# thunlp/OpenMatch

Measured on AMD Instinct MI355X. Metric: passages/sec encode (bert-base DPR bi-encoder, 128 tok -> 768-d) [+ queries/sec exact top-1000 over 8.8M x 768 in `search`], higher is better.
Workload: dtype f16; 1 GPU; bert-base DPR bi-encoder encode+search, MS MARCO 8.8M x 128-tok -> 768-d (BASELINE configs[1]); seq_len=128, global_batch=1024, index_rows=8841823, queries=6980, topk=1000, weights=random-init BertConfig() seed 0, parallelism=shard1

## Files before the change

### include/openmatch_hip.h

```cpp
#ifndef OPENMATCH_HIP_H
#define OPENMATCH_HIP_H

#include <stddef.h>
#include <stdint.h>

#ifdef __cplusplus
extern "C" {
#endif

#define OM_ABI_VERSION 6

#define OM_F32 0
#define OM_BF16 1
#define OM_F16 2

#define OM_ACT_NONE 0
#define OM_ACT_GELU_ERF 1
#define OM_ACT_RELU 2
#define OM_ACT_GELU_TANH 3
#define OM_ACT_SILU 5
#define OM_ACT_MUL_RESID 0x100
#define OM_ACT_PRE_GRAD 0x200

#define OM_ARCH_BERT 0
#define OM_ARCH_T5 1
#define OM_ARCH_MODERNBERT 2

#define OM_ARCH_CAUSAL 3

#define OM_ARCH_NOMICBERT 4

#define OM_POOL_NONE 0
#define OM_POOL_FIRST 1
#define OM_POOL_MEAN 2
#define OM_POOL_LAST 3

#define OM_SEARCH_F32 0
#define OM_SEARCH_F16_RESCORE 1

const char* om_last_error(void);
int om_abi_version(void);

int om_device_count(void);

#define OM_TIMING_GEMM_BF16 0
#define OM_TIMING_GEMM_F32 1
#define OM_TIMING_SCAN 2
void om_debug_gemm_trace(unsigned long long* buf);
void om_debug_gemm_gen(int gen);
#define OM_GEMM_FAMILY_V1 1
#define OM_GEMM_FAMILY_V2 2
#define OM_GEMM_FAMILY_V6 6
#define OM_GEMM_FAMILY_G7 7
#define OM_GEMM_FAMILY_G7_ONE_TILE 70
#define OM_GEMM_FAMILY_G7C16 71
#define OM_GEMM_FAMILY_G7R16 72
#define OM_GEMM_FAMILY_SKINNY 9
int om_debug_gemm_last(void);
int om_debug_gemm_plan(int in_dtype, const void* A, int64_t lda, const void* B, int64_t ldb, int out_dtype, void* C, int64_t ldc,
                       int64_t M, int64_t N, int64_t K, const float* bias, const void* resid, int64_t ldr, int act);
typedef struct OmDebugGemmEpilogue {
  const float* bias; const void* resid; int64_t ldr; int act;
  void* pre_act; int64_t ldp; float drop_p; uint64_t seed; const int* drop_rows;
  const float* ln_stats; const float* ln_colsum; const float* rln_stats; const float* rln_g; const float* rln_b; float* stats_out;
  const void* resid_lo; void* out_lo;
  const float* resid32; float* out32;
  const float* a_ln32; const float* a_ln_g; const float* a_ln_b; float* a_ln_stats_out; const float* rln32; const float* rln32_stats;
  int lo8; float ln_inv_h, ln_eps; int ln_rms; int reverse;
  const int* rows_dev;
} OmDebugGemmEpilogue;
int om_debug_gemm_ex(int in_dtype, const void* A, int64_t lda, const void* B, int64_t ldb, int out_dtype, void* C, int64_t ldc,
                     int64_t M, int64_t N, int64_t K, const OmDebugGemmEpilogue* ep, void* stream);
int om_debug_gemm_plan_ex(int in_dtype, const void* A, int64_t lda, const void* B, int64_t ldb, int out_dtype, void* C, int64_t ldc,
                          int64_t M, int64_t N, int64_t K, const OmDebugGemmEpilogue* ep);
int om_debug_gemm_splitk(int in_dtype, const void* A, int64_t lda, const void* B, int64_t ldb, float* C, int64_t ldc, int64_t M,
                         int64_t N, int64_t K, void* stream);
#define OM_OPT_ENCODER_FUSED_LN 0
#define OM_OPT_ENCODER_DEBUG 1
#define OM_OPT_ATTENTION_FAST 2
#define OM_OPT_SCAN_GEN7 3
#define OM_OPT_SCAN_GROWTH 4
#define OM_OPT_WGRAD_DEBUG 5
#define OM_OPT_GEMM_GROUP_M 6
#define OM_OPT_SCAN_QGROUP 7
#define OM_OPT_TRAIN_WGRAD_STREAM 8
#define OM_OPT_ATTENTION_DEBUG 9
#define OM_OPT_ENCODER_PINGPONG 10
#define OM_OPT_ENCODER_TWO_PLANE 11
#define OM_OPT_GEMM_VARIANT 12
#define OM_OPT_SEARCH_DEBUG 13
#define OM_OPT_TRAIN_WGRAD_BATCH 14
#define OM_OPT_GEMM_MAX_GRID 15
#define OM_OPT_GEMM_CONT 16
#define OM_OPT_TRAIN_TAPE_GRAD 17
#define OM_OPT_TRAIN_RES32 18
#define OM_OPT_GEMM_SKINNY_M 19
#define OM_OPT_GEMM_SKINNY_CFG 20
#define OM_OPT_FEW_ROWS_LN_FUSE 21
#define OM_OPT_ENCODER_SKIP_PAD 22
#define OM_OPT_ENCODER_CLS_TAIL 23
#define OM_OPT_ENCODER_LANES 24
#define OM_OPT_COUNT 25
int om_debug_option(int opt, int value);
int om_debug_option_value(int opt);
int om_debug_attention(const void* qkv, void* ctx, const int64_t* mask, int64_t B, int L, int H, int heads, void* stream);
int om_debug_attention_ex(int dtype, const void* qkv, void* ctx, const int64_t* mask, const float* pos_bias, int64_t B, int L, int H,
                          int heads, float scale, float drop_p, uint64_t seed, void* stream, int reverse, const int* kmax,
                          const int* cu, int w);
int om_debug_rope(int dtype, void* qkv, int64_t M, int L, int H, float theta, void* stream);
int om_debug_rope_rows(int dtype, void* qkv, int64_t rows, int L, int H, float theta, const int* row_map, void* stream);
int om_debug_swiglu_rows(int dtype, const void* in, void* out, int64_t M, int F, void* stream);
int om_debug_embed(int dtype, const int64_t* ids, const int64_t* type_ids, const float* word, const float* pos, const float* type,
                   const float* g, const float* b, void* out, int64_t M, int L, int H, int vocab, int type_vocab, float eps, void* stream);
int om_debug_attention_causal(int dtype, const void* qkv, void* ctx, const int64_t* mask, int64_t B, int L, int n_heads, int n_kv_heads,
                              float scale, void* stream);
int om_debug_rope_gqa(int dtype, void* qkv, int64_t M, int L, int n_heads, int n_kv_heads, const float* inv_freq, float scaling, void* stream);
int om_debug_attention_causal_packed(int dtype, const void* qkv, void* ctx, const int64_t* mask, const int* cu, int64_t B, int L, int n_heads,
                                     int n_kv_heads, float scale, void* stream);
int om_debug_rope_gqa_rows(int dtype, void* qkv, int64_t rows, int L, int n_heads, int n_kv_heads, const float* inv_freq, float scaling,
                           const int* row_map, void* stream);
int om_debug_attention_causal_hd(int dtype, const void* qkv, void* ctx, const int64_t* mask, int64_t B, int L, int n_heads, int n_kv_heads,
                                 int head_dim, float scale, void* stream);
int om_debug_attention_causal_hd_packed(int dtype, const void* qkv, void* ctx, const int64_t* mask, const int* cu, int64_t B, int L,
                                        int n_heads, int n_kv_heads, int head_dim, float scale, void* stream);
int om_debug_qknorm_rope(int dtype, void* qkv, int64_t M, int L, int n_heads, int n_kv_heads, int head_dim, const float* q_norm_g,
                         const float* k_norm_g, float eps, const float* inv_freq, float scaling, void* stream);
int om_debug_qknorm_rope_rows(int dtype, void* qkv, int64_t rows, int L, int n_heads, int n_kv_heads, int head_dim, const float* q_norm_g,
                              const float* k_norm_g, float eps, const float* inv_freq, float scaling, const int* row_map, void* stream);
int om_debug_attention_gqa_d256(int dtype, const void* qkv, void* ctx, const int64_t* mask, int64_t B, int L, int n_heads, int n_kv_heads,
                                float scale, int w, void* stream);
int om_debug_qknorm_rope_d256(int dtype, void* qkv, int64_t M, int L, int n_heads, int n_kv_heads, const float* q_norm_g, const float* k_norm_g,
                              float eps, const float* inv_freq, float scaling, void* stream);
int om_debug_attention_gqa_d256_packed(int dtype, const void* qkv, void* ctx, const int64_t* mask, const int* cu, int64_t B, int L, int n_heads,
                                       int n_kv_heads, float scale, int w, void* stream);
int om_debug_qknorm_rope_d256_rows(int dtype, void* qkv, int64_t rows, int L, int n_heads, int n_kv_heads, const float* q_norm_g,
                                   const float* k_norm_g, float eps, const float* inv_freq, float scaling, const int* row_map, void* stream);
int om_debug_rmsnorm_add(int dtype, const void* h, int64_t ldh, float* x, int64_t ldx, const float* g, int64_t M, int H, float eps, void* stream);
int om_debug_mask_extent(const int64_t* mask, int64_t B, int L, int* kmax, void* stream);
int om_debug_pack_rows(const int* kmax, int64_t B, int L, int64_t rows, int* cu, int* cls_rows, int* row_map, void* stream);
#define OM_ATTN_FAMILY_GENERIC 1
#define OM_ATTN_FAMILY_FWD16 2
#define OM_ATTN_FAMILY_FWD16_KMAX4 3
#define OM_ATTN_FAMILY_FWD16C 4
#define OM_ATTN_FAMILY_LONG 5
#define OM_ATTN_FAMILY_D32 6
#define OM_ATTN_FAMILY_BAND16 7
#define OM_ATTN_FAMILY_BAND32 8
int om_debug_attention_last(void);
int om_debug_attention_plan(int dtype, int64_t B, int L, int H, int heads, int has_bias, float drop_p, int has_kmax, int has_cu, int w);
#define OM_ATTN_BWD_FAMILY_BWD16 1
#define OM_ATTN_BWD_FAMILY_GENERIC 2
#define OM_ATTN_BWD_FAMILY_LONG 3
#define OM_ATTN_BWD_FAMILY_D32 4
int om_debug_attention_bwd_last(void);
int om_debug_attention_bwd_plan(int dtype, int64_t B, int L, int H, int heads, int has_bias, int has_drel, int has_cu, int packed);
int om_debug_attention_bwd_ex(int dtype, const void* qkv, const void* ctx, const void* dctx, void* dqkv, const int64_t* mask,
                              const float* pos_bias, float* drel, float* stats, int64_t B, int L, int H, int heads, float scale,
                              float drop_p, uint64_t seed, const int* cu, int packed, void* stream);
size_t om_debug_attention_bwd_stats_bytes(int64_t B, int heads);
#define OM_ENC_PATH_BERT_FUSED 1
#define OM_ENC_PATH_BERT_PENDING_LN 2
#define OM_ENC_PATH_BERT_FEW32 3
#define OM_ENC_PATH_BERT_PLAIN 4
#define OM_ENC_PATH_MODERNBERT 5
#define OM_ENC_PATH_T5_FUSED 6
#define OM_ENC_PATH_T5_PLAIN 7
struct OmEncoderConfig;
int om_debug_encoder_plan(const struct OmEncoderConfig* cfg, int gated_ffn, int has_rel_bias, int64_t B, int64_t L, int64_t packed_rows,
                          int want_hidden);
int om_debug_encoder_skip_pad(const struct OmEncoderConfig* cfg, int gated_ffn, int has_rel_bias, int64_t B, int64_t L, int want_hidden);
int om_debug_encoder_cls_tail(const struct OmEncoderConfig* cfg, int gated_ffn, int has_rel_bias, int64_t B, int64_t L, int64_t packed_rows,
                              int want_hidden);
int om_debug_encoder_lanes(const struct OmEncoderConfig* cfg, int gated_ffn, int has_rel_bias, int64_t B, int64_t L, int64_t packed_rows,
                           int want_hidden, int64_t* B0);
#define OM_ENCODER_LANE_RANGES 15
int om_debug_encoder_lane_ranges(const struct OmEncoderConfig* cfg, int gated_ffn, int has_rel_bias, int64_t B, int64_t L, int lane,
                                 int64_t* out, int cap);
int64_t om_debug_encoder_lane_forks(void);
int om_debug_gather_rows(const void* src0, void* dst0, const void* src1, void* dst1, const void* src2, void* dst2, const float* stats_src,
                         float* stats_dst, const int* rows, int64_t B, int64_t L, int64_t Mc, int H, void* stream);
int om_debug_attn_drop_keep(uint64_t seed, int64_t b, int h, int heads, int Lm, int q, int key, float p);
int om_debug_wave_sum_check(const float* in, float* out_shuffle, float* out_dpp, int64_t groups, void* stream);
#define OM_ROW_FWD_GENERIC 1
#define OM_ROW_FWD_X8 2
#define OM_ROW_LN_BWD 3
int om_debug_row_kernel_last(void);
int om_debug_layernorm(int dtype, const void* x, int64_t ldx, void* y, int64_t ldy, const float* g, const float* b, int64_t M, int H,
                       float eps, int rms, const void* x_lo, int lo8, void* stream);
int om_debug_layernorm_f32out(int dtype, const void* x, int64_t ldx, float* y, int64_t ldy, const float* g, const float* b, int64_t M,
                              int H, float eps, int rms, const void* x_lo, const int* rows, int lo8, void* stream);
int om_debug_layernorm_from_f32(int dtype, const float* x, int64_t ldx, void* y, int64_t ldy, const float* g, const float* b, int64_t M,
                                int H, float eps, int rms, void* stream);
int om_debug_layernorm_dual(int dtype, const float* x, int64_t ldx, void* y, float* y32, int64_t ldy, const float* g, const float* b,
                            int64_t M, int H, float eps, void* stream);
int om_debug_norm_bwd(int dtype, const void* dy, const void* x, const float* g, void* dx, float* dg, float* db, int64_t M, int H,
                      float eps, int rms, const void* add, void* stream);
int om_debug_ln_bwd_drop(int dtype, const void* dy, const void* x, const float* g, void* dx, void* dx_drop, float drop_p,
                         uint64_t drop_seed, float* dg, float* db, int64_t M, int H, float eps, const float* dy32, const float* x32,
                         float* partial, int* partial_blocks , const int* drop_rows, void* stream);
typedef struct OmLnSite { const float* partial; float* dg; float* db; int blocks; } OmLnSite;
int om_debug_ln_param_reduce(const OmLnSite* sites , int n, int H, void* stream);
int om_debug_embed_bwd(int dtype, const void* dy, const int64_t* ids, const int64_t* type_ids, const float* word, const float* pos,
                       const float* type, const float* g, float* dword, float* dpos, float* dtype_, float* dg, float* db, int64_t M,
                       int L, int H, int vocab, int type_vocab, float eps, const int* cu, void* stream);
int om_debug_pool(int dtype, const void* x, const int64_t* mask, float* out, int64_t B, int L, int H, int mode, const int* cu,
                  void* stream);
int om_debug_pool_bwd(int dtype, const float* dp, const int64_t* mask, void* dh, int64_t B, int L, int H, int mode, const int* cu,
                      void* stream);
int om_debug_l2norm(const float* x, float* y, int64_t M, int D, void* stream);
int om_debug_l2norm_bwd(const float* x, const float* dy, float* dx, int64_t M, int D, void* stream);
int om_debug_colsum(int dtype, const void* x, int64_t ld, int64_t M, int N, float* out, void* stream);
int om_debug_dropout(int dtype, const void* x, void* y, int64_t n, float p, uint64_t seed, const int* rows, int H, void* stream);
int om_debug_ln_fold(int dtype, const void* W, const float* gamma, const float* beta, const float* b, void* Wf, float* colsum,
                     float* bf, int N, int K, void* stream);
int om_debug_ln_stats_reduce(const float* slots, int nslots, int64_t M, float* out, void* stream);
int om_kernel_timing_enable(int enable);
int om_kernel_timing_read(int kernel_class, double* total_ms, int64_t* launches, double* flops);

int om_gemm_nt(int in_dtype, const void* A, int64_t lda, const void* B, int64_t ldb,
               int out_dtype, void* C, int64_t ldc, int64_t M, int64_t N, int64_t K,
               const float* bias, const void* resid, int64_t ldr, int act, void* stream);

int om_gemm_tn_acc(int in_dtype, const void* A, int64_t lda, const void* B, int64_t ldb,
                   float* C, int64_t ldc, float* bias, int64_t M, int64_t N, int64_t K, void* stream);

typedef struct OmTnProblem {
  const void* A; const void* B; float* C; float* bias;
  int64_t lda, ldb, ldc, N, K;
} OmTnProblem;
int om_gemm_tn_acc_batch(int in_dtype, const OmTnProblem* problems, int n, int64_t M, void* stream);

typedef struct OmLayerWeights {
  const void* qkv_w;
  const float* qkv_b;
  const void* o_w;
  const float* o_b;
  const float* ln1_g;
  const float* ln1_b;
  const void* ffn1_w;
  const float* ffn1_b;
  const void* ffn1g_w;
  const void* ffn2_w;
  const float* ffn2_b;
  const float* ln2_g;
  const float* ln2_b;
} OmLayerWeights;

typedef struct OmEncoderConfig {
  int arch;
  int dtype;
  int hidden;
  int n_layers;
  int n_heads;
  int head_dim;
  int ffn;
  int vocab;
  int max_pos;
  int type_vocab;
  int act;
  float ln_eps;
  int rel_buckets;
  int rel_max_dist;
  int pooling;
  int head_in;
  int head_out;
  int normalize;
  float rope_theta_global;
  float rope_theta_local;
  int half_window;
  uint64_t sliding_layers;
} OmEncoderConfig;

typedef struct OmEncoderWeights {
  const float* word_emb;
  const float* pos_emb;
  const float* type_emb;
  const float* emb_ln_g;
  const float* emb_ln_b;
  const OmLayerWeights* layers_host;
  const float* final_ln_g;
  const float* rel_bias;
  const float* head_w;
  const void* folded;
  const float* final_ln_b;
} OmEncoderWeights;

size_t om_encoder_fold_bytes(const OmEncoderConfig* cfg);
int om_encoder_fold_weights(const OmEncoderConfig* cfg, const OmEncoderWeights* w, void* folded, size_t bytes, void* stream);

size_t om_encoder_workspace_bytes(const OmEncoderConfig* cfg, int64_t B, int64_t L);

int om_t5_relative_bucket(int relative_position, int num_buckets, int max_distance);

int om_encoder_forward(const OmEncoderConfig* cfg, const OmEncoderWeights* w,
                       const int64_t* input_ids, const int64_t* attention_mask,
                       const int64_t* token_type_ids, int64_t B, int64_t L,
                       void* out_hidden, float* out_reps, void* workspace,
                       size_t workspace_bytes, void* stream);

int om_encoder_packed_supported(const OmEncoderConfig* cfg, int gated_ffn, int64_t B, int64_t L, int64_t packed_rows);
size_t om_encoder_workspace_bytes_packed(const OmEncoderConfig* cfg, int64_t B, int64_t L, int64_t packed_rows);
int om_encoder_forward_packed(const OmEncoderConfig* cfg, const OmEncoderWeights* w,
                              const int64_t* input_ids, const int64_t* attention_mask,
                              const int64_t* token_type_ids, int64_t B, int64_t L, int64_t packed_rows,
                              float* out_reps, void* workspace, size_t workspace_bytes, void* stream);

typedef struct OmCausalConfig {
  OmEncoderConfig base;
  int n_kv_heads;
  float rope_attention_scaling;
  float inv_freq[32];
} OmCausalConfig;
size_t om_causal_encoder_workspace_bytes(const OmCausalConfig* cfg, int64_t B, int64_t L);
int om_causal_encoder_forward(const OmCausalConfig* cfg, const OmEncoderWeights* w, const int64_t* input_ids,
                              const int64_t* attention_mask, int64_t B, int64_t L, void* out_hidden, float* out_reps,
                              void* workspace, size_t workspace_bytes, void* stream);
int om_causal_encoder_packed_supported(const OmCausalConfig* cfg, int64_t B, int64_t L, int64_t packed_rows);
size_t om_causal_encoder_workspace_bytes_packed(const OmCausalConfig* cfg, int64_t B, int64_t L, int64_t packed_rows);
int om_causal_encoder_forward_packed(const OmCausalConfig* cfg, const OmEncoderWeights* w, const int64_t* input_ids,
                                     const int64_t* attention_mask, int64_t B, int64_t L, int64_t packed_rows, float* out_reps,
                                     void* workspace, size_t workspace_bytes, void* stream);

typedef struct OmCausalConfig2 {
  OmCausalConfig base;
  int qk_norm;
  int reserved;
  float inv_freq[64];
} OmCausalConfig2;
typedef struct OmCausalQkNorm {
  const float* q_norm_g;
  const float* k_norm_g;
} OmCausalQkNorm;
size_t om_causal2_encoder_workspace_bytes(const OmCausalConfig2* cfg, int64_t B, int64_t L);
int om_causal2_encoder_forward(const OmCausalConfig2* cfg, const OmEncoderWeights* w, const OmCausalQkNorm* qk_norm_host,
                               const int64_t* input_ids, const int64_t* attention_mask, int64_t B, int64_t L, void* out_hidden,
                               float* out_reps, void* workspace, size_t workspace_bytes, void* stream);
int om_causal2_encoder_packed_supported(const OmCausalConfig2* cfg, int64_t B, int64_t L, int64_t packed_rows);
size_t om_causal2_encoder_workspace_bytes_packed(const OmCausalConfig2* cfg, int64_t B, int64_t L, int64_t packed_rows);
int om_causal2_encoder_forward_packed(const OmCausalConfig2* cfg, const OmEncoderWeights* w, const OmCausalQkNorm* qk_norm_host,
                                      const int64_t* input_ids, const int64_t* attention_mask, int64_t B, int64_t L, int64_t packed_rows,
                                      float* out_reps, void* workspace, size_t workspace_bytes, void* stream);

#define OM_ARCH_GEMMA3 5
typedef struct OmGemma3Config {
  OmCausalConfig base;
  float attn_scale;
  int half_window;
  uint64_t sliding_layers;
  float full_scaling;
  float sliding_scaling;
  float attn_logit_softcapping;
  int bidirectional;
  float full_inv_freq[128];
  float sliding_inv_freq[128];
} OmGemma3Config;
typedef struct OmGemma3Norms {
  const float* q_norm_g;
  const float* k_norm_g;
  const float* post_attention_norm_g;
  const float* post_feedforward_norm_g;
} OmGemma3Norms;
size_t om_gemma3_encoder_workspace_bytes(const OmGemma3Config* cfg, int64_t B, int64_t L);
int om_gemma3_encoder_forward(const OmGemma3Config* cfg, const OmEncoderWeights* w, const OmGemma3Norms* norms_host, const int64_t* input_ids,
                              const int64_t* attention_mask, int64_t B, int64_t L, void* out_hidden, float* out_reps, void* workspace,
                              size_t workspace_bytes, void* stream);
int om_gemma3_encoder_packed_supported(const OmGemma3Config* cfg, int64_t B, int64_t L, int64_t packed_rows);
size_t om_gemma3_encoder_workspace_bytes_packed(const OmGemma3Config* cfg, int64_t B, int64_t L, int64_t packed_rows);
int om_gemma3_encoder_forward_packed(const OmGemma3Config* cfg, const OmEncoderWeights* w, const OmGemma3Norms* norms_host,
                                     const int64_t* input_ids, const int64_t* attention_mask, int64_t B, int64_t L, int64_t packed_rows,
                                     float* out_reps, void* workspace, size_t workspace_bytes, void* stream);

typedef struct OmT5DecoderLayer {
  const void* sa_v_w;
  const void* sa_o_w;
  const float* sa_ln_g;
  const void* ca_q_w;
  const void* ca_kv_w;
  const void* ca_o_w;
  const float* ca_ln_g;
  const void* ffn1_w;
  const void* ffn1g_w;
  const void* ffn2_w;
  const float* ffn_ln_g;
} OmT5DecoderLayer;
typedef struct OmT5DecoderWeights {
  const float* start_emb;
  const float* final_ln_g;
  const OmT5DecoderLayer* layers_host;
  int n_layers;
} OmT5DecoderWeights;
size_t om_t5_decoder_workspace_bytes(const OmEncoderConfig* cfg, int64_t B, int64_t L);
int om_t5_decoder_step(const OmEncoderConfig* cfg, const OmT5DecoderWeights* w, const void* enc_hidden,
                       const int64_t* attention_mask, int64_t B, int64_t L, float* out_hidden,
                       void* workspace, size_t workspace_bytes, void* stream);

typedef struct OmT5DecoderLayerGrads {
  float* sa_v_w;  float* sa_o_w; float* sa_ln_g;
  float* ca_q_w;  float* ca_kv_w; float* ca_o_w; float* ca_ln_g;
  float* ffn1_w;  float* ffn1g_w; float* ffn2_w; float* ffn_ln_g;
} OmT5DecoderLayerGrads;
typedef struct OmT5DecoderGrads {
  float* start_emb;
  float* final_ln_g;
  const OmT5DecoderLayerGrads* layers_host;
} OmT5DecoderGrads;
size_t om_t5_decoder_tape_bytes(const OmEncoderConfig* cfg, int n_layers, int64_t B, int64_t L);
size_t om_t5_decoder_train_workspace_bytes(const OmEncoderConfig* cfg, int n_layers, int64_t B, int64_t L);
int om_t5_decoder_train_forward(const OmEncoderConfig* cfg, const OmT5DecoderWeights* w, const void* enc_hidden,
                                const int64_t* attention_mask, int64_t B, int64_t L, float dropout, uint64_t seed,
                                void* tape, size_t tape_bytes, float* out_hidden, void* workspace,
                                size_t workspace_bytes, void* stream);
int om_t5_decoder_train_backward(const OmEncoderConfig* cfg, const OmT5DecoderWeights* w, const void* enc_hidden,
                                 const int64_t* attention_mask, int64_t B, int64_t L, float dropout, uint64_t seed,
                                 const void* tape, const float* d_out, const OmT5DecoderGrads* grads,
                                 void* d_enc_hidden, void* workspace, size_t workspace_bytes, void* stream);

int om_linear_f32_backward(const float* dy, const float* x, const float* w, float* dw, float* dx, int B, int D, int K,
                           void* stream);

typedef struct OmLayerGrads {
  float* qkv_w;  float* qkv_b;  float* o_w;    float* o_b;   float* ln1_g; float* ln1_b;
  float* ffn1_w; float* ffn1_b; float* ffn2_w; float* ffn2_b; float* ln2_g; float* ln2_b;
  float* ffn1g_w;
} OmLayerGrads;

typedef struct OmEncoderGrads {
  float* word_emb; float* pos_emb; float* type_emb; float* emb_ln_g; float* emb_ln_b;
  const OmLayerGrads* layers_host;
  float* head_w;
  float* final_ln_g;
  float* rel_bias;
} OmEncoderGrads;

size_t om_encoder_tape_bytes(const OmEncoderConfig* cfg, int64_t B, int64_t L);
size_t om_encoder_train_workspace_bytes(const OmEncoderConfig* cfg, int64_t B, int64_t L);

int om_encoder_train_forward(const OmEncoderConfig* cfg, const OmEncoderWeights* w,
                             const int64_t* input_ids, const int64_t* attention_mask,
                             const int64_t* token_type_ids, int64_t B, int64_t L,
                             float hidden_dropout, float attn_dropout, uint64_t seed, void* tape,
                             size_t tape_bytes, float* out_reps, void* workspace,
                             size_t workspace_bytes, void* stream);

int om_encoder_train_backward(const OmEncoderConfig* cfg, const OmEncoderWeights* w,
                              const int64_t* input_ids, const int64_t* attention_mask,
                              const int64_t* token_type_ids, int64_t B, int64_t L,
                              float hidden_dropout, float attn_dropout, uint64_t seed,
                              const void* tape, const float* d_reps, const OmEncoderGrads* grads,
                              void* workspace, size_t workspace_bytes, void* stream);

int om_encoder_train_packed_supported(const OmEncoderConfig* cfg, int64_t B, int64_t L, int64_t packed_rows);
size_t om_encoder_tape_bytes_packed(const OmEncoderConfig* cfg, int64_t B, int64_t L, int64_t packed_rows);
size_t om_encoder_train_workspace_bytes_packed(const OmEncoderConfig* cfg, int64_t B, int64_t L, int64_t packed_rows);
int om_encoder_train_forward_packed(const OmEncoderConfig* cfg, const OmEncoderWeights* w,
                                    const int64_t* input_ids, const int64_t* attention_mask,
                                    const int64_t* token_type_ids, int64_t B, int64_t L, int64_t packed_rows,
                                    float hidden_dropout, float attn_dropout, uint64_t seed,
                                    void* tape, size_t tape_bytes, float* out_reps,
                                    void* workspace, size_t workspace_bytes, void* stream);
int om_encoder_train_backward_packed(const OmEncoderConfig* cfg, const OmEncoderWeights* w,
                                     const int64_t* input_ids, const int64_t* attention_mask,
                                     const int64_t* token_type_ids, int64_t B, int64_t L, int64_t packed_rows,
                                     float hidden_dropout, float attn_dropout, uint64_t seed,
                                     const void* tape, const float* d_reps, const OmEncoderGrads* grads,
                                     void* workspace, size_t workspace_bytes, void* stream);

int om_encoder_train_forward_hidden(const OmEncoderConfig* cfg, const OmEncoderWeights* w,
                                    const int64_t* input_ids, const int64_t* attention_mask,
                                    const int64_t* token_type_ids, int64_t B, int64_t L,
                                    float hidden_dropout, float attn_dropout, uint64_t seed, void* tape,
                                    size_t tape_bytes, void* out_hidden, void* workspace,
                                    size_t workspace_bytes, void* stream);
int om_encoder_train_backward_hidden(const OmEncoderConfig* cfg, const OmEncoderWeights* w,
                                     const int64_t* input_ids, const int64_t* attention_mask,
                                     const int64_t* token_type_ids, int64_t B, int64_t L,
                                     float hidden_dropout, float attn_dropout, uint64_t seed,
                                     const void* tape, const void* d_hidden, const OmEncoderGrads* grads,
                                     void* workspace, size_t workspace_bytes, void* stream);

int om_encoder_train_set_layer_events(void* const* events, int n);

#define OM_ADAM_CHUNK 16384
typedef struct OmAdamTensor {
  float* p; const float* g; float* m; float* v;
  void* shadow0; void* shadow1;
  int64_t n;
  float weight_decay;
  int shadow0_dtype, shadow1_dtype, reserved;
} OmAdamTensor;
int om_grad_sqnorm(const OmAdamTensor* tensors, const int32_t* chunks, int n_chunks, float* partial, float* out_sq, void* stream);
int om_adamw_step(const OmAdamTensor* tensors, const int32_t* chunks, int n_chunks, float lr, float beta1, float beta2, float eps,
                  int64_t step, const float* gnorm_sq, float max_norm, float grad_scale, int skip_nonfinite,
                  const float* scale_state ,
                  void* stream);
int om_loss_scale_update(const float* gnorm_sq, float* state4, int growth_interval, void* stream);


int om_index_to_f16(const float* rows_f32, int64_t N, int d, void* rows_f16, float* stats,
                    void* stream);

size_t om_sim_topk_workspace_bytes(int64_t n_queries, int d, int k);

int om_sim_topk(int mode, const float* queries, int64_t n_queries, const float* index_f32,
                const void* index_f16, const float* stats, int64_t N, int d, int k,
                int64_t id_offset, float* out_scores, int64_t* out_ids, void* workspace,
                size_t workspace_bytes, void* stream);

void om_sim_topk_info(int64_t out[8]);

#define OM_SCAN_FAMILY_GENERIC 1
#define OM_SCAN_FAMILY_WIDE 2
#define OM_SCAN_FAMILY_STREAM32 3
#define OM_SCAN_FAMILY_STREAM16 4
int om_debug_scan_plan(int half, int64_t nq, int d, int out[4]);
int om_debug_sim_stream(const void* rows16, int64_t nrows, uint32_t row_base, const void* queries16, int64_t nq, int d, const float* thr,
                        uint64_t* keys, unsigned* cnt, int grid, void* stream);

int om_topk_merge(const float* part_scores, const int64_t* part_ids, int W, int64_t n_queries,
                  int k_in, int k_out, float* out_scores, int64_t* out_ids, void* stream);

int om_contrastive_fwd_bwd(const float* q, const float* p, int Qg, int Pg, int d, int n_psg,
                           float loss_scale, int q_row0, int q_rows, int p_row0, int p_rows,
                           float* loss, float* scores, float* d_q, float* d_p, float* workspace,
                           void* stream);

int om_contrastive_fwd_bwd_ex(const float* q, const float* p, int Qg, int Pg, int d, const int64_t* target, int n_psg,
                              int reduction, const float* row_grad, float loss_scale, int q_row0, int q_rows,
                              int p_row0, int p_rows, float* loss, float* scores, float* d_q, float* d_p,
                              float* workspace, void* stream);

#define OM_COMM_ID_BYTES 128
int om_comm_unique_id(void* id128);
int om_comm_init(const void* id128, int world, int rank, void** comm);
int om_comm_destroy(void* comm);
int om_comm_count(void* comm, int* count);
int om_allgather_rows(void* comm, const void* send, void* recv, int64_t rows, int64_t row_bytes, void* stream);
int om_allreduce_grads(void* comm, float* buf, int64_t n, int average, void* stream);
int om_exchange_topk(void* comm, int world, const float* D, const int64_t* I, int64_t q_block, int k, float* recvD,
                     int64_t* recvI, void* stream);

#ifdef __cplusplus
}
#endif
#endif
```

### openmatch_amd/csrc/abi.cpp

```cpp
#include "common.h"

static thread_local std::string g_last_error;
void om_set_error(const std::string& msg) { g_last_error = msg; }

extern "C" const char* om_last_error(void) { return g_last_error.c_str(); }
extern "C" int om_abi_version(void) { return OM_ABI_VERSION; }
extern "C" int om_device_count(void) {
  int n = 0;
  hipError_t e = hipGetDeviceCount(&n);
  if (e != hipSuccess) {
    om_set_error(std::string("hipGetDeviceCount: ") + hipGetErrorString(e));
    return -1;
  }
  return n;
}

#include <mutex>
#include <vector>
namespace {
struct Span { hipEvent_t a, b; };
struct ClassStat { std::vector<Span> spans; double flops = 0; size_t used = 0; };
bool g_timing = false;
ClassStat g_stat[3];
std::mutex g_mu;
}
bool om_timing_on() { return g_timing; }
void om_timing_begin(int c, hipStream_t s) {
  std::lock_guard<std::mutex> lk(g_mu);
  ClassStat& st = g_stat[c];
  if (st.used == st.spans.size()) {
    Span sp;
    (void)hipEventCreate(&sp.a);
    (void)hipEventCreate(&sp.b);
    st.spans.push_back(sp);
  }
  (void)hipEventRecord(st.spans[st.used].a, s);
}
void om_timing_end(int c, hipStream_t s, double flops) {
  std::lock_guard<std::mutex> lk(g_mu);
  ClassStat& st = g_stat[c];
  (void)hipEventRecord(st.spans[st.used].b, s);
  st.used++;
  st.flops += flops;
}
extern "C" int om_kernel_timing_enable(int enable) { g_timing = enable != 0; return 0; }
extern "C" int om_kernel_timing_read(int c, double* total_ms, int64_t* launches, double* flops) {
  if (c < 0 || c > 2) { om_set_error("om_kernel_timing_read: bad class"); return 1; }
  std::lock_guard<std::mutex> lk(g_mu);
  ClassStat& st = g_stat[c];
  double ms = 0;
  for (size_t i = 0; i < st.used; ++i) {
    hipError_t e = hipEventSynchronize(st.spans[i].b);
    float t = 0;
    if (e == hipSuccess) e = hipEventElapsedTime(&t, st.spans[i].a, st.spans[i].b);
    if (e != hipSuccess) { om_set_error(std::string("om_kernel_timing_read: ") + hipGetErrorString(e)); return 1; }
    ms += t;
  }
  if (total_ms) *total_ms = ms;
  if (launches) *launches = (int64_t)st.used;
  if (flops) *flops = st.flops;
  st.used = 0; st.flops = 0;
  return 0;
}

#include <atomic>
#include <map>
#include <tuple>
namespace {
std::atomic<int> g_opt[OM_OPT_COUNT];
std::atomic<bool> g_opt_init{false};
std::mutex g_opt_mu;
void opt_init() {
  std::lock_guard<std::mutex> lk(g_opt_mu);
  if (g_opt_init.load()) return;
  const char* e = getenv("OM_ENCODER_FUSED_LN");
  g_opt[OM_OPT_ENCODER_FUSED_LN] = e ? atoi(e) : 1;
  g_opt[OM_OPT_ENCODER_DEBUG] = getenv("OM_ENCODER_DEBUG") ? 1 : 0;
  e = getenv("OM_ATTENTION_FAST");
  g_opt[OM_OPT_ATTENTION_FAST] = e ? atoi(e) : 1;
  e = getenv("OM_SCAN_GEN7");
  g_opt[OM_OPT_SCAN_GEN7] = e ? atoi(e) : 1;
  e = getenv("OM_SCAN_GROWTH");
  g_opt[OM_OPT_SCAN_GROWTH] = e ? atoi(e) : 60;
  g_opt[OM_OPT_WGRAD_DEBUG] = 0;
  g_opt[OM_OPT_ATTENTION_DEBUG] = 0;
  e = getenv("OM_ENCODER_PINGPONG");
  g_opt[OM_OPT_ENCODER_PINGPONG] = e ? atoi(e) : 1;
  e = getenv("OM_TRAIN_WGRAD_STREAM");
  g_opt[OM_OPT_TRAIN_WGRAD_STREAM] = e ? atoi(e) : 1;
  e = getenv("OM_SCAN_QGROUP");
  g_opt[OM_OPT_SCAN_QGROUP] = e ? atoi(e) : 8;
  e = getenv("OM_GEMM_GROUP_M");
  g_opt[OM_OPT_GEMM_GROUP_M] = e ? atoi(e) : 8;
  e = getenv("OM_ENCODER_TWO_PLANE");
  g_opt[OM_OPT_ENCODER_TWO_PLANE] = e ? atoi(e) : 3;
  e = getenv("OM_GEMM_VARIANT");
  g_opt[OM_OPT_GEMM_VARIANT] = e ? atoi(e) : 0;
  e = getenv("OM_SEARCH_DEBUG");
  g_opt[OM_OPT_SEARCH_DEBUG] = e ? (atoi(e) ? atoi(e) : 1) : 0;
  e = getenv("OM_TRAIN_WGRAD_BATCH");
  g_opt[OM_OPT_TRAIN_WGRAD_BATCH] = e ? atoi(e) : 4;
  e = getenv("OM_GEMM_MAX_GRID");
  g_opt[OM_OPT_GEMM_MAX_GRID] = e ? atoi(e) : 0;
  e = getenv("OM_TRAIN_TAPE_GRAD");
  g_opt[OM_OPT_TRAIN_TAPE_GRAD] = e ? atoi(e) : 1;
  e = getenv("OM_TRAIN_RES32");
  g_opt[OM_OPT_TRAIN_RES32] = e ? atoi(e) : 1;
  e = getenv("OM_GEMM_CONT");
  g_opt[OM_OPT_GEMM_CONT] = e ? atoi(e) : 495;
  e = getenv("OM_GEMM_SKINNY_M");
  g_opt[OM_OPT_GEMM_SKINNY_M] = e ? atoi(e) : 1024;
  e = getenv("OM_FEW_ROWS_LN_FUSE");
  g_opt[OM_OPT_FEW_ROWS_LN_FUSE] = e ? atoi(e) : 64;
  e = getenv("OM_ENCODER_SKIP_PAD");
  g_opt[OM_OPT_ENCODER_SKIP_PAD] = e ? atoi(e) : 1;
  e = getenv("OM_ENCODER_CLS_TAIL");
  g_opt[OM_OPT_ENCODER_CLS_TAIL] = e ? atoi(e) : 1;
  e = getenv("OM_ENCODER_LANES");
  g_opt[OM_OPT_ENCODER_LANES] = e ? atoi(e) : 65536;
  g_opt_init.store(true);
}
}
bool om_option_is_set(int opt) {
  if (opt == OM_OPT_SCAN_GROWTH) return getenv("OM_SCAN_GROWTH") != nullptr;
  return false;
}
int om_option(int opt) {
  if (!g_opt_init.load(std::memory_order_acquire)) opt_init();
  return g_opt[opt].load(std::memory_order_relaxed);
}
extern "C" int om_debug_option(int opt, int value) {
  if (opt < 0 || opt >= OM_OPT_COUNT) { om_set_error("om_debug_option: unknown option"); return 1; }
  if (!g_opt_init.load(std::memory_order_acquire)) opt_init();
  g_opt[opt].store(value);
  return 0;
}
extern "C" int om_debug_option_value(int opt) {
  if (opt < 0 || opt >= OM_OPT_COUNT) { om_set_error("om_debug_option_value: unknown option"); return -1; }
  return om_option(opt);
}

int om_t5_lut_device(int L, int buckets, int max_dist, const int** out) {
  static std::mutex mu;
  static std::map<std::tuple<int, int, int, int>, int*> cache;
  int dev = 0;
  OM_HIP(hipGetDevice(&dev));
  std::lock_guard<std::mutex> lk(mu);
  auto key = std::make_tuple(dev, L, buckets, max_dist);
  auto it = cache.find(key);
  if (it == cache.end()) {
    std::vector<int> lut(2 * L);
    for (int rel = -(L - 1); rel <= L - 1; ++rel) lut[rel + (L - 1)] = om_t5_relative_bucket(rel, buckets, max_dist);
    int* d = nullptr;
    OM_HIP(hipMalloc(&d, (size_t)(2 * L) * sizeof(int)));
    OM_HIP(hipMemcpy(d, lut.data(), (size_t)(2 * L - 1) * sizeof(int), hipMemcpyHostToDevice));
    it = cache.emplace(key, d).first;
  }
  *out = it->second;
  return 0;
}
```

### openmatch_amd/csrc/attention.hip

```cpp
#include <type_traits>

#include "attn_chunked.h"
#include "attn_plan.h"

static thread_local int g_attn_last = 0;
extern "C" int om_debug_attention_last(void) { return g_attn_last; }

template <typename T, int KT>
__global__ __launch_bounds__(64 * KT) void attention_kernel(
    const T* __restrict__ qkv, T* __restrict__ ctx, const int64_t* __restrict__ mask,
    const float* __restrict__ pos_bias, int L, int H, int heads, float scale, float drop_p,
    uint64_t seed) {
  typedef AttnGeom<T> G;
  typedef typename MmaOps<T>::frag_t frag_t;
  constexpr int LP = KT * 32 + 4;
  extern __shared__ __attribute__((aligned(16))) char smem[];
  char* sK = smem;
  T* sVt = (T*)(smem + KT * 32 * G::ROWB);
  float* sM = (float*)(smem + KT * 32 * G::ROWB + 64 * LP * (int)sizeof(T));

  const int h = blockIdx.x % heads;
  const int64_t b = blockIdx.x / heads;
  const int tid = threadIdx.x, nthr = blockDim.x;
  const int64_t ld = 3 * (int64_t)H;
  const T* base = qkv + b * L * ld + h * 64;

  for (int idx = tid; idx < KT * 32 * G::CPR; idx += nthr) {
    const int row = idx / G::CPR, c = idx % G::CPR;
    uint4 kv = make_uint4(0, 0, 0, 0), vv = make_uint4(0, 0, 0, 0);
    if (row < L) {
      kv = *(const uint4*)(base + (int64_t)row * ld + H + c * G::EPC);
      vv = *(const uint4*)(base + (int64_t)row * ld + 2 * H + c * G::EPC);
    }
    *(uint4*)(sK + row * G::ROWB + ((c ^ G::key(row)) << 4)) = kv;
    const T* ve = (const T*)&vv;
#pragma unroll
    for (int e = 0; e < G::EPC; ++e) sVt[(c * G::EPC + e) * LP + row] = ve[e];
  }
  for (int k = tid; k < KT * 32; k += nthr)
    sM[k] = k < L ? (mask[b * L + k] != 0 ? 0.f : kFinfoMin) : -INFINITY;
  __syncthreads();

  const int wave = tid >> 6, lane = tid & 63, half = lane >> 5, l31 = lane & 31;
  const int q0 = wave * 32;
  if (q0 >= L) return;
  const int qrow = (q0 + l31) < L ? (q0 + l31) : (L - 1);

  frag_t qf[G::NKK];
#pragma unroll
  for (int kk = 0; kk < G::NKK; ++kk)
    qf[kk] = *(const frag_t*)(base + (int64_t)qrow * ld + (kk * 2 + half) * G::EPC);

  f32x16_t s[KT];
#pragma unroll
  for (int t = 0; t < KT; ++t) {
#pragma unroll
    for (int r = 0; r < 16; ++r) s[t][r] = 0.f;
    const int row = t * 32 + l31;
    const char* krow = sK + row * G::ROWB;
    const int key = G::key(row);
#pragma unroll
    for (int kk = 0; kk < G::NKK; ++kk) {
      const frag_t a = *(const frag_t*)(krow + (((kk * 2 + half) ^ key) << 4));
      MmaOps<T>::mma(a, qf[kk], s[t]);
    }
  }

  float mx = -INFINITY;
#pragma unroll
  for (int t = 0; t < KT; ++t)
#pragma unroll
    for (int g = 0; g < 4; ++g) {
      const int k0 = t * 32 + 8 * g + 4 * half;
      const f32x4_t mb = *(const f32x4_t*)(sM + k0);
#pragma unroll
      for (int e = 0; e < 4; ++e) {
        float v = s[t][4 * g + e] * scale;
        if (pos_bias) {
          const int kc = (k0 + e) < L ? (k0 + e) : (L - 1);
          v += pos_bias[((int64_t)h * L + qrow) * L + kc];
        }
        v += mb[e];
        s[t][4 * g + e] = v;
        mx = fmaxf(mx, v);
      }
    }
  mx = fmaxf(mx, __shfl_xor(mx, 32, 64));
  float sum = 0.f;
#pragma unroll
  for (int t = 0; t < KT; ++t)
#pragma unroll
    for (int r = 0; r < 16; ++r) {
      const float e = G::exp_(s[t][r] - mx);
      s[t][r] = e;
      sum += e;
    }
  sum += __shfl_xor(sum, 32, 64);
  const float inv = 1.0f / sum;
#pragma unroll
  for (int t = 0; t < KT; ++t)
#pragma unroll
    for (int r = 0; r < 16; ++r) s[t][r] *= inv;
  if (drop_p > 0.f) {
    const AttnDrop dr(drop_p);
#pragma unroll
    for (int t = 0; t < KT; ++t)
#pragma unroll
      for (int g = 0; g < 4; ++g) {
        const uint64_t bits = attn_drop_bits(seed, b, h, heads, L, q0 + l31, (t * 32 + 8 * g + 4 * half) >> 2);
#pragma unroll
        for (int e = 0; e < 4; ++e) s[t][4 * g + e] = attn_drop_keep(bits, e, dr.thresh) ? s[t][4 * g + e] * dr.keep_scale : 0.f;
      }
  }

  f32x16_t o[2];
#pragma unroll
  for (int dt = 0; dt < 2; ++dt)
#pragma unroll
    for (int r = 0; r < 16; ++r) o[dt][r] = 0.f;
#pragma unroll
  for (int t = 0; t < KT; ++t) SlabMma<T>::run(s[t], sVt + l31 * LP + t * 32 + 4 * half, LP, o);

  __syncthreads();
  T* so = (T*)(sK + (size_t)q0 * G::ROWB);
#pragma unroll
  for (int dt = 0; dt < 2; ++dt)
#pragma unroll
    for (int r = 0; r < 16; ++r) {
      const int q = (r & 3) + 8 * (r >> 2) + 4 * half;
      ElemOps<T>::store(so + q * 64 + dt * 32 + l31, o[dt][r]);
    }
  T* out = ctx + (b * L + q0) * H + h * 64;
  constexpr int VPR = G::ROWB / 16;
#pragma unroll
  for (int it = 0; it < 32 * VPR / 64; ++it) {
    const int idx = it * 64 + lane, row = idx / VPR, c = idx % VPR;
    const uint4 v = *(const uint4*)((const char*)so + row * G::ROWB + c * 16);
    if (q0 + row < L) *(uint4*)((char*)(out + (int64_t)row * H) + c * 16) = v;
  }
}

template <typename T, int KT, bool BIAS, bool DROP, int DBG, int KTV>
__device__ __forceinline__ void attention_fwd16_body(
    const T* __restrict__ qkv, T* __restrict__ ctx, const int64_t* __restrict__ mask,
    const float* __restrict__ pos_bias, int L, int H, int heads, float scale, float drop_p, uint64_t seed, int rev,
    int64_t row0, int Lm) {
  typedef typename MmaOps<T>::frag_t frag_t;
  extern __shared__ __attribute__((aligned(16))) char smem[];
  char* const sK = smem;
  char* const sV = smem + KT * 32 * 128;
  float* const sM = (float*)(smem + 2 * KT * 32 * 128);
  const int h = blockIdx.x % heads;
  const int64_t b = rev ? (int64_t)(gridDim.x / heads) - 1 - blockIdx.x / heads : blockIdx.x / heads;
  const int tid = threadIdx.x, lane = tid & 63, half = lane >> 5, l31 = lane & 31;
  const int wave = __builtin_amdgcn_readfirstlane(tid >> 6);
  const int64_t ld2 = 6 * (int64_t)H;
  const char* const base = (const char*)(qkv + row0 * 3 * (int64_t)H + h * 64);
  if (!(DBG & 1))
#pragma unroll
  for (int i = 0; i < 4; ++i) {
    if (KTV < KT && i * KT + wave >= KTV * 4) continue;
    const int r = (i * KT + wave) * 8 + (lane >> 3);
    const int rr = r < L ? r : L - 1;
    const uint32_t off = (uint32_t)(rr * ld2) + (((lane & 7) ^ ((r >> 1) & 7)) << 4);
    const uint32_t offv = (uint32_t)(rr * ld2) + (((lane & 7) ^ (((r >> 1) & 1) << 2)) << 4);
    const uint32_t dst = (uint32_t)((i * KT + wave) * 1024);
    g7_dma(base + 2 * H, off, g7_lds_addr(sK) + dst);
    g7_dma(base + 4 * H, offv, g7_lds_addr(sV) + dst);
  }
  const float LOG2E = 1.4426950408889634f;
  for (int k = tid; k < KT * 32; k += 64 * KT)
    sM[k] = k < L ? (mask[b * Lm + k] != 0 ? 0.f : -1e30f) : -INFINITY;

  const int q0 = wave * 32;
  const int qrow = (q0 + l31) < L ? (q0 + l31) : (L - 1);
  frag_t qf[4];
#pragma unroll
  for (int kk = 0; kk < 4; ++kk) qf[kk] = *(const frag_t*)(base + (int64_t)qrow * ld2 + (kk * 2 + half) * 16);
  asm volatile("s_waitcnt vmcnt(0)" ::: "memory");
  __syncthreads();
  if (q0 >= L) return;

  constexpr int KTC = (DBG & 2) ? 0 : KTV;
  const int key = (l31 >> 1) & 7;
  f32x16_t s[KTV];
#pragma unroll
  for (int t = 0; t < KTC; ++t) {
#pragma unroll
    for (int r = 0; r < 16; ++r) s[t][r] = 0.f;
    const char* krow = sK + (t * 32 + l31) * 128;
#pragma unroll
    for (int kk = 0; kk < 4; ++kk) {
      const frag_t a = *(const frag_t*)(krow + (((kk * 2 + half) ^ key) << 4));
      MmaOps<T>::mma(a, qf[kk], s[t]);
    }
    __builtin_amdgcn_sched_barrier(0);
  }
  const float c2 = scale * LOG2E;
  float mx = -INFINITY;
#pragma unroll
  for (int t = 0; t < KTC; ++t)
#pragma unroll
    for (int g = 0; g < 4; ++g) {
      const int k0 = t * 32 + 8 * g + 4 * half;
      const f32x4_t mb = *(const f32x4_t*)(sM + k0);
      f32x4_t pb = {0.f, 0.f, 0.f, 0.f};
      if (BIAS) {
        const float* pr = pos_bias + ((int64_t)h * Lm + qrow) * Lm;
#pragma unroll
        for (int e = 0; e < 4; ++e) pb[e] = pr[(k0 + e) < Lm ? (k0 + e) : (Lm - 1)] * LOG2E;
      }
#pragma unroll
      for (int e = 0; e < 4; ++e) {
        const float v = fmaf(s[t][4 * g + e], c2, mb[e]) + pb[e];
        s[t][4 * g + e] = v;
        mx = fmaxf(mx, v);
      }
      __builtin_amdgcn_sched_barrier(0);
    }
  mx = fmaxf(mx, __shfl_xor(mx, 32, 64));
  float sum = 0.f;
#pragma unroll
  for (int t = 0; t < KTC; ++t)
#pragma unroll
    for (int r = 0; r < 16; ++r) {
      const float e = __builtin_amdgcn_exp2f(s[t][r] - mx);
      s[t][r] = e;
      sum += e;
    }
  sum += __shfl_xor(sum, 32, 64);
  float inv = 1.0f / sum;
  if (DROP) {
    const AttnDrop dr(drop_p);
#pragma unroll
    for (int t = 0; t < KTC; ++t)
  #pragma unroll
      for (int g = 0; g < 4; ++g) {
        const uint64_t bits = attn_drop_bits(seed, b, h, heads, Lm, q0 + l31, (t * 32 + 8 * g + 4 * half) >> 2);
#pragma unroll
        for (int e = 0; e < 4; ++e) s[t][4 * g + e] = attn_drop_keep(bits, e, dr.thresh) ? s[t][4 * g + e] : 0.f;
        __builtin_amdgcn_sched_barrier(0);
      }
    inv *= dr.keep_scale;
  }

  const int i16 = lane & 15;
  const char* const vt0 = sV + (4 * half + (i16 >> 2)) * 128 + 32 * ((lane >> 4) & 1) + 8 * (i16 & 3);
  const int vsw = (i16 >> 3) & 1;
  f32x16_t o[2];
#pragma unroll
  for (int dt = 0; dt < 2; ++dt)
#pragma unroll
    for (int r = 0; r < 16; ++r) o[dt][r] = 0.f;
#pragma unroll
  for (int t = 0; t < KTC; ++t) {
    uint4 pa[2];
#pragma unroll
    for (int u = 0; u < 2; ++u)
      pa[u] = make_uint4(Half16<T>::pack2(s[t][8 * u + 0], s[t][8 * u + 1]), Half16<T>::pack2(s[t][8 * u + 2], s[t][8 * u + 3]),
                         Half16<T>::pack2(s[t][8 * u + 4], s[t][8 * u + 5]), Half16<T>::pack2(s[t][8 * u + 6], s[t][8 * u + 7]));
#pragma unroll
    for (int u = 0; u < 2; ++u) {
#pragma unroll
      for (int dt = 0; dt < 2; ++dt) {
        const char* p = vt0 + (t * 32 + 16 * u) * 128 + ((dt ^ vsw) << 6);
        const frag_t vf = vfrag_of<frag_t>(vtrd(p), vtrd(p + 8 * 128));
        MmaOps<T>::mma(vf, __builtin_bit_cast(frag_t, pa[u]), o[dt]);
      }
    }
    __builtin_amdgcn_sched_barrier(0);
  }
  if (DBG & 2) {
#pragma unroll
    for (int kk = 0; kk < 4; ++kk) o[0][kk] = (float)qf[kk][0];
  }
  __syncthreads();
  char* const so = sK + q0 * 128;
#pragma unroll
  for (int dt = 0; dt < 2; ++dt)
#pragma unroll
    for (int gp = 0; gp < 2; ++gp) {
      uint32_t a0 = Half16<T>::pack2(o[dt][8 * gp + 0] * inv, o[dt][8 * gp + 1] * inv), a1 = Half16<T>::pack2(o[dt][8 * gp + 2] * inv, o[dt][8 * gp + 3] * inv);
      uint32_t b0 = Half16<T>::pack2(o[dt][8 * gp + 4] * inv, o[dt][8 * gp + 5] * inv), b1 = Half16<T>::pack2(o[dt][8 * gp + 6] * inv, o[dt][8 * gp + 7] * inv);
      auto r0 = __builtin_amdgcn_permlane32_swap(a0, b0, false, false);
      auto r1 = __builtin_amdgcn_permlane32_swap(a1, b1, false, false);
      *(uint4*)(so + l31 * 128 + (((4 * dt + 2 * gp + half) ^ (l31 & 7)) << 4)) = make_uint4(r0[0], r1[0], r0[1], r1[1]);
    }
  char* const out = (char*)(ctx + (row0 + q0) * (int64_t)H + h * 64);
#pragma unroll
  for (int it = 0; it < 4; ++it) {
    const int row = it * 8 + (lane >> 3), c = lane & 7;
    const uint4 v = *(const uint4*)(so + row * 128 + ((c ^ (row & 7)) << 4));
    if (!(DBG & 4) || v.x == 0x12345u) { if (q0 + row < L) *(uint4*)(out + (int64_t)row * H * 2 + c * 16) = v; }
  }
}

template <typename T, int KT, bool BIAS, bool DROP, int DBG = 0>
__global__ __launch_bounds__(64 * KT, KT <= 4 ? ((BIAS || DROP) ? 3 : 4) : 2) void attention_fwd16_kernel(
    const T* __restrict__ qkv, T* __restrict__ ctx, const int64_t* __restrict__ mask,
    const float* __restrict__ pos_bias, int L, int H, int heads, float scale, float drop_p, uint64_t seed, int rev,
    const int* __restrict__ kmax, const int* __restrict__ cu) {
#define OM_ATTN_BODY(V) attention_fwd16_body<T, KT, BIAS, DROP, DBG, V>(qkv, ctx, mask, pos_bias, Lb, H, heads, scale, drop_p, seed, rev, row0, L)
  const int64_t b = rev ? (int64_t)(gridDim.x / heads) - 1 - blockIdx.x / heads : blockIdx.x / heads;
  int64_t row0 = b * L;
  int Lb = L;
  if (cu) {
    const int c0 = __builtin_amdgcn_readfirstlane(cu[b]), c1 = __builtin_amdgcn_readfirstlane(cu[b + 1]);
    row0 = c0; Lb = c1 - c0;
    if (Lb <= 0) return;
  }
  if (KT == 4 && !BIAS && !DROP && (kmax || cu)) {
    const int kt = ((cu ? Lb : __builtin_amdgcn_readfirstlane(kmax[b])) + 31) >> 5;
    if (kt <= 1) { OM_ATTN_BODY(1); return; }
    if (kt == 2) { OM_ATTN_BODY(2); return; }
    if (kt == 3) { OM_ATTN_BODY(3); return; }
  }
  OM_ATTN_BODY(KT);
#undef OM_ATTN_BODY
}

template <typename T, int KT, bool BIAS, bool DROP>
static int launch_attn16(const void* qkv, void* ctx, const int64_t* mask, const float* pos_bias, int64_t B, int L, int H,
                         int heads, float scale, float drop_p, uint64_t seed, hipStream_t s, int rev, const int* kmax, const int* cu) {
  const int lds = 2 * KT * 32 * 128 + KT * 32 * 4;
  if (attn_lds_once<attention_fwd16_kernel<T, KT, BIAS, DROP>>(lds)) return 1;
#ifdef OM_PROBE_KERNELS
  const int dbg = (sizeof(T) == 2 && std::is_same<T, bf16_t>::value && KT == 4 && !BIAS && !DROP) ? om_option(OM_OPT_ATTENTION_DEBUG) : 0;
#else
  const int dbg = 0;
#endif
  if (dbg) {
#ifdef OM_PROBE_KERNELS
#define OM_ATTN_DBG(D)                                                                                                        \
  case D:                                                                                                                     \
    hipLaunchKernelGGL((attention_fwd16_kernel<bf16_t, 4, false, false, D>), dim3((unsigned)(heads * B)), dim3(256), lds, s,          \
                       (const bf16_t*)qkv, (bf16_t*)ctx, mask, pos_bias, L, H, heads, scale, drop_p, seed, rev, kmax, cu);    \
    break;
    switch (dbg) { OM_ATTN_DBG(1) OM_ATTN_DBG(2) OM_ATTN_DBG(3) OM_ATTN_DBG(4) OM_ATTN_DBG(5) OM_ATTN_DBG(6) OM_ATTN_DBG(7) default: break; }
#undef OM_ATTN_DBG
#endif
    OM_LAUNCH_CHECK();
    return 0;
  }
  hipLaunchKernelGGL((attention_fwd16_kernel<T, KT, BIAS, DROP>), dim3((unsigned)(heads * B)), dim3(64 * KT), lds, s, (const T*)qkv,
                     (T*)ctx, mask, pos_bias, L, H, heads, scale, drop_p, seed, rev, kmax, cu);
  OM_LAUNCH_CHECK();
  return 0;
}
template <typename T, bool BIAS, bool DROP>
__global__ __launch_bounds__(256, 2) void attention_fwd16c_kernel(
    const T* __restrict__ qkv, T* __restrict__ ctx, const int64_t* __restrict__ mask,
    const float* __restrict__ pos_bias, int Lm, int H, int heads, float scale, float drop_p, uint64_t seed, const int* __restrict__ cu) {
  const int h = blockIdx.x % heads;
  const int64_t b = blockIdx.x / heads;
  int64_t row0 = b * Lm;
  int L = Lm;
  if (cu) {
    const int c0 = __builtin_amdgcn_readfirstlane(cu[b]), c1 = __builtin_amdgcn_readfirstlane(cu[b + 1]);
    row0 = c0; L = c1 - c0;
  }
  const int qb = blockIdx.y * 128;
  if (qb >= L) return;
  attn_chunked16<T, AttnFull, BIAS, DROP>(attn_rows_fused(qkv, ctx, row0, H, h), AttnFull{}, mask + b * Lm, L, L, qb, scale, AttnFullArgs{pos_bias, drop_p, seed, b, h, heads, Lm});
}

template <typename T, bool BIAS, bool DROP>
static int launch_attn16c(const void* qkv, void* ctx, const int64_t* mask, const float* pos_bias, int64_t B, int L, int H,
                           int heads, float scale, float drop_p, uint64_t seed, hipStream_t s, const int* cu) {
  const int lds = 2 * 128 * 128 + 128 * 4;
  hipLaunchKernelGGL((attention_fwd16c_kernel<T, BIAS, DROP>), dim3((unsigned)(heads * B), (unsigned)((L + 127) / 128)), dim3(256), lds, s,
                     (const T*)qkv, (T*)ctx, mask, pos_bias, L, H, heads, scale, drop_p, seed, cu);
  OM_LAUNCH_CHECK();
  return 0;
}
template <typename T>
__global__ __launch_bounds__(256) void attention_long_kernel(
    const T* __restrict__ qkv, T* __restrict__ ctx, const int64_t* __restrict__ mask,
    const float* __restrict__ pos_bias, int Lm, int H, int heads, float scale, float drop_p, uint64_t seed, const int* __restrict__ cu) {
  const int h = blockIdx.x % heads;
  const int64_t b = blockIdx.x / heads;
  const int qb = blockIdx.y * 128;
  int64_t row0 = b * Lm;
  int L = Lm;
  if (cu) { row0 = cu[b]; L = cu[b + 1] - cu[b]; }
  if (qb >= L) return;
  attn_chunked_qreg<T, AttnFull>(attn_rows_fused(qkv, ctx, row0, H, h), AttnFull{}, mask + b * Lm, L, L, qb, scale, AttnFullArgs{pos_bias, drop_p, seed, b, h, heads, Lm});
}

template <typename T>
static int launch_attn_long(const void* qkv, void* ctx, const int64_t* mask, const float* pos_bias, int64_t B, int L, int H,
                            int heads, float scale, float drop_p, uint64_t seed, hipStream_t s, const int* cu) {
  const int lds = 128 * AttnGeom<T>::ROWB + 64 * 132 * (int)sizeof(T) + 128 * 4 + 128 * 4;
  if (attn_lds_once<attention_long_kernel<T>>(lds)) return 1;
  hipLaunchKernelGGL((attention_long_kernel<T>), dim3((unsigned)(heads * B), (unsigned)((L + 127) / 128)), dim3(256), lds, s,
                     (const T*)qkv, (T*)ctx, mask, pos_bias, L, H, heads, scale, drop_p, seed, cu);
  OM_LAUNCH_CHECK();
  return 0;
}

template <typename T, int KT>
static int launch_attn(const void* qkv, void* ctx, const int64_t* mask, const float* pos_bias,
                       int64_t B, int L, int H, int heads, float scale, float drop_p, uint64_t seed,
                       hipStream_t s) {
  constexpr int LP = KT * 32 + 4;
  const int lds = KT * 32 * AttnGeom<T>::ROWB + 64 * LP * (int)sizeof(T) + KT * 32 * 4;
  if (attn_lds_once<attention_kernel<T, KT>>(lds)) return 1;
  const int waves = (L + 31) / 32;
  hipLaunchKernelGGL((attention_kernel<T, KT>), dim3((unsigned)(heads * B)),
                     dim3(64 * waves), lds, s, (const T*)qkv, (T*)ctx, mask, pos_bias, L, H, heads,
                     scale, drop_p, seed);
  OM_LAUNCH_CHECK();
  return 0;
}

__global__ void mask_extent_kernel(const int64_t* __restrict__ mask, int64_t B, int L, int* __restrict__ kmax) {
  const int64_t b = (int64_t)blockIdx.x * (blockDim.x >> 6) + (threadIdx.x >> 6);
  if (b >= B) return;
  const int lane = threadIdx.x & 63;
  int last = 0;
  for (int k = lane; k < L; k += 64) if (mask[b * L + k] != 0) last = k + 1;
#pragma unroll
  for (int o = 32; o > 0; o >>= 1) last = max(last, __shfl_xor(last, o, 64));
  if (lane == 0) kmax[b] = last ? last : L;
}
__global__ __launch_bounds__(1024) void pack_rows_kernel(const int* __restrict__ kmax, int64_t B, int L, int64_t rows, int* __restrict__ cu,
                                                          int* __restrict__ cls_rows, int* __restrict__ row_map) {
  __shared__ int part[1024];
  const int tid = threadIdx.x;
  const int64_t per = (B + 1023) / 1024, lo = tid * per, hi = lo + per < B ? lo + per : B;
  int sum = 0;
  for (int64_t i = lo; i < hi; ++i) sum += kmax[i];
  part[tid] = sum;
  __syncthreads();
  for (int off = 1; off < 1024; off <<= 1) {
    const int v = tid >= off ? part[tid - off] : 0;
    __syncthreads();
    part[tid] += v;
    __syncthreads();
  }
  const int total = part[1023];
  const int cap = (int)rows;
  if (blockIdx.x == 0) {
    int run = part[tid] - sum;
    for (int64_t i = lo; i < hi; ++i) {
      cu[i] = run < cap ? run : cap;
      cls_rows[i] = run < cap ? run : cap - 1;
      run += kmax[i];
    }
    if (tid == 1023) { cu[B] = total < cap ? total : cap; cu[B + 1] = total; }
  }
  for (int64_t t = (int64_t)blockIdx.x * 1024 + tid; t < rows; t += (int64_t)gridDim.x * 1024) {
    int v = -1;
    if (t < total) {
      int a = 0, b = 1023;
      while (a < b) { const int m = (a + b) >> 1; if (part[m] > (int)t) b = m; else a = m + 1; }
      int64_t i = a * per;
      int run = a ? part[a - 1] : 0;
      for (int n = kmax[i]; run + n <= (int)t; n = kmax[++i]) run += n;
      v = (int)(i * L + ((int)t - run));
    }
    row_map[t] = v;
  }
}
int omk_pack_rows(const int* kmax, int64_t B, int L, int64_t rows, int* cu, int* cls_rows, int* row_map, hipStream_t s) {
  if (B <= 0) return 0;
  if (rows > 0x7fffffff || B * (int64_t)L > 0x7fffffff) OM_FAIL("packed rows: token counts below 2^31");
  const int64_t slices = (rows + 1023) / 1024;
  hipLaunchKernelGGL(pack_rows_kernel, dim3((unsigned)(slices < 1 ? 1 : slices > 1024 ? 1024 : slices)), dim3(1024), 0, s, kmax, B, L, rows, cu, cls_rows,
                     row_map);
  OM_LAUNCH_CHECK();
  return 0;
}

int omk_mask_extent(const int64_t* mask, int64_t B, int L, int* kmax, hipStream_t s) {
  if (B <= 0) return 0;
  hipLaunchKernelGGL(mask_extent_kernel, dim3((unsigned)((B + 3) / 4)), dim3(256), 0, s, mask, B, L, kmax);
  OM_LAUNCH_CHECK();
  return 0;
}

int omk_attention(int dtype, const void* qkv, void* ctx, const int64_t* mask, const float* pos_bias, int64_t B, int L, int H, int heads,
                  float scale, float drop_p, uint64_t seed, hipStream_t s, int reverse, const int* kmax, const int* cu, int w) {
  g_attn_last = 0;
  const AttnPlan p = attn_plan_fwd(dtype, B, L, H, heads, pos_bias != nullptr, drop_p, kmax != nullptr, cu != nullptr, w, attn_switches());
  if (p.error) OM_FAIL(p.error);
  g_attn_last = p.family | (p.kt << 8);
  switch (p.family) {
    case 0: return 0;
    case OM_ATTN_FAMILY_D32: return omk_attention_d32(p, dtype, qkv, ctx, mask, pos_bias, B, L, H, heads, scale, drop_p, seed, s, reverse, kmax, cu);
    case OM_ATTN_FAMILY_BAND16: case OM_ATTN_FAMILY_BAND32: return omk_attention_band(dtype, qkv, ctx, mask, B, L, H, heads, scale, w, kmax, s);
    case OM_ATTN_FAMILY_FWD16: case OM_ATTN_FAMILY_FWD16_KMAX4:
      return attn_with_type16(dtype, [&](auto t) {
        return attn_with_kt<1, 2, 4, 6, 8>(p.kt, [&](auto kt) {
          return attn_with_flags(p.bias, p.drop, [&](auto bias, auto drop) {
            return launch_attn16<decltype(t), kt(), bias(), drop()>(qkv, ctx, mask, pos_bias, B, L, H, heads, scale, drop_p, seed, s, reverse, kmax, cu);
          });
        });
      });
    case OM_ATTN_FAMILY_FWD16C:
      return attn_with_type16(dtype, [&](auto t) {
        return attn_with_flags(p.bias, p.drop, [&](auto bias, auto drop) {
          return launch_attn16c<decltype(t), bias(), drop()>(qkv, ctx, mask, pos_bias, B, L, H, heads, scale, drop_p, seed, s, cu);
        });
      });
    case OM_ATTN_FAMILY_LONG:
      return attn_with_type(dtype, [&](auto t) { return launch_attn_long<decltype(t)>(qkv, ctx, mask, pos_bias, B, L, H, heads, scale, drop_p, seed, s, cu); });
    default:
      if (dtype == OM_BF16)
        return attn_with_kt<1, 2, 4, 6, 8>(p.kt, [&](auto kt) { return launch_attn<bf16_t, kt()>(qkv, ctx, mask, pos_bias, B, L, H, heads, scale, drop_p, seed, s); });
      return attn_with_kt<1, 2, 4, 6, 8>(p.kt, [&](auto kt) { return launch_attn<float, kt()>(qkv, ctx, mask, pos_bias, B, L, H, heads, scale, drop_p, seed, s); });
  }
}

extern "C" int om_debug_attention_plan(int dtype, int64_t B, int L, int H, int heads, int has_bias, float drop_p, int has_kmax, int has_cu, int w) {
  const AttnPlan p = attn_plan_fwd(dtype, B, L, H, heads, has_bias != 0, drop_p, has_kmax != 0, has_cu != 0, w, attn_switches());
  if (p.error) { om_set_error(std::string(__func__) + ": " + p.error); return -1; }
  return p.family | (p.kt << 8);
}

extern "C" int om_debug_attention_ex(int dtype, const void* qkv, void* ctx, const int64_t* mask, const float* pos_bias, int64_t B, int L, int H,
                                     int heads, float scale, float drop_p, uint64_t seed, void* stream, int reverse, const int* kmax,
                                     const int* cu, int w) {
  g_attn_last = 0;
  if (!qkv || !ctx || !mask) OM_FAIL("null argument");
  if (dtype != OM_F32 && dtype != OM_BF16 && dtype != OM_F16) OM_FAIL("attention: dtype must be OM_F32, OM_BF16 or OM_F16");
  if (w > 0 && (pos_bias || drop_p > 0.f || cu || reverse)) OM_FAIL("banded attention: no position bias, dropout, packed rows or reverse walk");
  return omk_attention(dtype, qkv, ctx, mask, pos_bias, B, L, H, heads, scale, drop_p, seed, (hipStream_t)stream, reverse, kmax, cu, w);
}
extern "C" int om_debug_attention(const void* qkv, void* ctx, const int64_t* mask, int64_t B, int L, int H, int heads, void* stream) {
  return om_debug_attention_ex(OM_BF16, qkv, ctx, mask, nullptr, B, L, H, heads, 0.125f, 0.f, 0, stream, 0, nullptr, nullptr, 0);
}
extern "C" int om_debug_rope(int dtype, void* qkv, int64_t M, int L, int H, float theta, void* stream) {
  if (!qkv) OM_FAIL("null argument");
  if (dtype != OM_F32 && dtype != OM_BF16 && dtype != OM_F16) OM_FAIL("rotary positions: dtype must be OM_F32, OM_BF16 or OM_F16");
  return omk_rope(dtype, qkv, M, L, H, theta, (hipStream_t)stream);
}
extern "C" int om_debug_rope_rows(int dtype, void* qkv, int64_t rows, int L, int H, float theta, const int* row_map, void* stream) {
  if (!qkv || !row_map) OM_FAIL("null argument");
  if (dtype != OM_F32 && dtype != OM_BF16 && dtype != OM_F16) OM_FAIL("rotary positions: dtype must be OM_F32, OM_BF16 or OM_F16");
  return omk_rope(dtype, qkv, rows, L, H, theta, (hipStream_t)stream, row_map);
}
extern "C" int om_debug_mask_extent(const int64_t* mask, int64_t B, int L, int* kmax, void* stream) {
  if (!mask || !kmax) OM_FAIL("null argument");
  if (L < 1) OM_FAIL("mask extent: L must be at least 1");
  return omk_mask_extent(mask, B, L, kmax, (hipStream_t)stream);
}
extern "C" int om_debug_pack_rows(const int* kmax, int64_t B, int L, int64_t rows, int* cu, int* cls_rows, int* row_map, void* stream) {
  if (!kmax || !cu || !cls_rows || !row_map) OM_FAIL("null argument");
  if (rows < 1) OM_FAIL("packed rows: rows must be at least 1");
  return omk_pack_rows(kmax, B, L, rows, cu, cls_rows, row_map, (hipStream_t)stream);
}
extern "C" int om_debug_attn_drop_keep(uint64_t seed, int64_t b, int h, int heads, int Lm, int q, int key, float p) {
  return attn_drop_keep1(seed, b, h, heads, Lm, q, key, AttnDrop(p).thresh) ? 1 : 0;
}
```

### openmatch_amd/csrc/encoder.hip

```cpp
#include <math.h>

#include <stdlib.h>

#include <algorithm>
#include <atomic>
#include <map>
#include <mutex>
#include <utility>
#include <vector>

#include "encoder_plan.h"

namespace {
struct FoldSlot { size_t w, cs, bf; };
struct FoldLayout { size_t per_layer, total; FoldSlot qkv, ffn1; };
FoldLayout fold_layout(const OmEncoderConfig* c) {
  const size_t H = c->hidden, F = enc_ffn1_cols(c);
  size_t off = 0;
  auto take = [&](size_t bytes) { size_t o = off; off = align_up(off + bytes, 256); return o; };
  FoldLayout L;
  L.qkv.w = take(3 * H * H * 2); L.qkv.cs = take(3 * H * 4); L.qkv.bf = take(3 * H * 4);
  L.ffn1.w = take(F * H * 2); L.ffn1.cs = take(F * 4); L.ffn1.bf = take(F * 4);
  L.per_layer = off;
  L.total = off * (size_t)c->n_layers;
  return L;
}
bool fold_applies(const OmEncoderConfig* c) {
  return c->arch != OM_ARCH_MODERNBERT && (c->dtype == OM_BF16 || c->dtype == OM_F16) && c->n_layers > 0 && c->hidden % 256 == 0 && c->ffn % 256 == 0;
}
}

extern "C" size_t om_encoder_fold_bytes(const OmEncoderConfig* cfg) {
  if (!cfg || !fold_applies(cfg)) return 0;
  return fold_layout(cfg).total;
}

extern "C" int om_encoder_fold_weights(const OmEncoderConfig* c, const OmEncoderWeights* w, void* blob, size_t bytes, void* stream) {
  if (!c || !w || !blob) OM_FAIL("null argument");
  if (!fold_applies(c)) OM_FAIL("nothing to fold for this configuration (om_encoder_fold_bytes is 0)");
  const FoldLayout L = fold_layout(c);
  if (bytes < L.total || ((uintptr_t)blob & 255)) OM_FAIL("fold buffer too small or not 256-byte aligned");
  const OmLayerWeights* Ls = w->layers_host;
  if (!Ls) OM_FAIL("layers_host is null");
  hipStream_t s = (hipStream_t)stream;
  const int H = c->hidden, F = enc_ffn1_cols(c);
  const bool bert = enc_bert_family(c);
  for (int l = 0; l < c->n_layers; ++l) {
    char* base = (char*)blob + (size_t)l * L.per_layer;
    const OmLayerWeights& lw = Ls[l];
    if (l > 0) {
      const float* g = bert ? Ls[l - 1].ln2_g : lw.ln1_g;
      const float* beta = bert ? Ls[l - 1].ln2_b : nullptr;
      if (omk_ln_fold(c->dtype, lw.qkv_w, g, beta, bert ? lw.qkv_b : nullptr, base + L.qkv.w, (float*)(base + L.qkv.cs),
                      (float*)(base + L.qkv.bf), 3 * H, H, s)) return 1;
    }
    if (!lw.ffn1g_w) {
      const float* g = bert ? lw.ln1_g : lw.ln2_g;
      const float* beta = bert ? lw.ln1_b : nullptr;
      if (omk_ln_fold(c->dtype, lw.ffn1_w, g, beta, bert ? lw.ffn1_b : nullptr, base + L.ffn1.w, (float*)(base + L.ffn1.cs),
                      (float*)(base + L.ffn1.bf), F, H, s)) return 1;
    }
  }
  return 0;
}

static int folded_weights(const OmEncoderConfig* c, const OmEncoderWeights* w, int layer, bool ffn1, const void* W, const float* g,
                          const float* beta, const float* b, int N, int K, void* scratch_w, float* scratch_cs, float* scratch_bf,
                          hipStream_t s, const void** Wf, const float** cs, const float** bf) {
  if (w->folded) {
    const FoldLayout L = fold_layout(c);
    const char* base = (const char*)w->folded + (size_t)layer * L.per_layer;
    const FoldSlot& sl = ffn1 ? L.ffn1 : L.qkv;
    *Wf = base + sl.w; *cs = (const float*)(base + sl.cs); *bf = (const float*)(base + sl.bf);
    return 0;
  }
  if (omk_ln_fold(c->dtype, W, g, beta, b, scratch_w, scratch_cs, scratch_bf, N, K, s)) return 1;
  *Wf = scratch_w; *cs = scratch_cs; *bf = scratch_bf;
  return 0;
}

struct EncWs {
  char *x, *y, *x1, *qkv, *ctx, *ff, *ff2;
  float *pooled, *headout, *posbias;
  float* final32;
  int* lut;
  int* kmax;
  int *cu, *cls_rows, *row_map;
  char* wfold;
  float *colsum, *bfold, *stats1, *stats2, *slots;
  char *y_lo, *x1_lo;
  float *r32a, *r32b, *y32;
  size_t total;
};

static EncWs carve(const OmEncoderConfig* c, const EncPlan& p, int64_t B, int64_t L, int64_t packed_rows, char* base) {
  const bool half = c->dtype == OM_BF16 || c->dtype == OM_F16;
  const size_t es = half ? 2 : 4;
  const size_t Mreal = (size_t)p.M, M = (size_t)p.Mp, H = c->hidden, F = c->ffn, F1 = enc_ffn1_cols(c);
  const bool bertf = enc_bert_family(c);
  size_t off = 0;
  auto take = [&](size_t bytes) { size_t o = off; off = align_up(off + bytes, 256); return base + o; };
  EncWs w;
  w.x = take(M * H * es);
  w.y = take(M * H * es);
  w.x1 = take(M * H * es);
  w.qkv = take(M * 3 * H * es);
  w.ctx = take(M * H * es);
  w.ff = take(M * F1 * es);
  w.ff2 = take(c->arch == OM_ARCH_T5 || c->arch == OM_ARCH_MODERNBERT || c->arch == OM_ARCH_NOMICBERT ? M * F * es : 0);
  w.pooled = (float*)take((size_t)B * H * 4);
  w.headout = (float*)take((size_t)B * (c->head_out > 0 ? c->head_out : 1) * 4);
  const bool rel = c->arch == OM_ARCH_T5 || (c->arch == OM_ARCH_BERT && c->rel_buckets > 0);
  w.posbias = (float*)take(rel ? (size_t)c->n_heads * L * L * 4 : 0);
  w.lut = (int*)take(rel ? (size_t)(2 * L) * 4 : 0);
  w.kmax = (int*)take((size_t)B * 4);
  w.cu = (int*)take(packed_rows > 0 ? (size_t)(B + 2) * 4 : 0);
  w.cls_rows = (int*)take(packed_rows > 0 ? (size_t)B * 4 : 0);
  w.row_map = (int*)take(packed_rows > 0 ? (size_t)packed_rows * 4 : 0);
  w.final32 = (float*)take(half && c->pooling != OM_POOL_NONE ? (c->pooling == OM_POOL_FIRST ? (size_t)B : Mreal) * H * 4 : 0);
  const bool fuse = half && c->arch != OM_ARCH_MODERNBERT;
  const size_t wide = std::max((size_t)3 * H, F1);
  w.wfold = take(fuse ? wide * H * es : 0);
  w.colsum = (float*)take(fuse ? wide * 4 : 0);
  w.bfold = (float*)take(fuse ? wide * 4 : 0);
  w.stats1 = (float*)take(fuse ? (size_t)2 * c->n_layers * M * 8 : 0);
  w.stats2 = w.stats1 ? w.stats1 + (size_t)c->n_layers * M * 2 : nullptr;
  w.slots = (float*)take(fuse ? (size_t)2 * ((H + 255) / 256) * M * 8 : 0);
  const bool two = fuse && bertf;
  w.y_lo = take(two ? M * H * es : 0);
  w.x1_lo = take(two ? M * H * es : 0);
  w.r32a = (float*)take(p.alloc_few32 ? Mreal * H * 4 : 0);
  w.r32b = (float*)take(p.alloc_few32 ? Mreal * H * 4 : 0);
  w.y32 = (float*)take(p.alloc_few32 ? Mreal * H * 4 : 0);
  w.total = off;
  return w;
}

static size_t workspace_bytes(const OmEncoderConfig* c, int64_t B, int64_t L, int64_t packed_rows) {
  const EncPlan p = encoder_plan_checked(EncPlanIn{c, B, L, packed_rows, false, false, false, false}, encoder_switches());
  return carve(c, p, B, L, packed_rows, nullptr).total;
}

extern "C" size_t om_encoder_workspace_bytes(const OmEncoderConfig* cfg, int64_t B, int64_t L) {
  if (!cfg || B <= 0 || L <= 0) return 0;
  return workspace_bytes(cfg, B, L, 0);
}

extern "C" size_t om_encoder_workspace_bytes_packed(const OmEncoderConfig* cfg, int64_t B, int64_t L, int64_t packed_rows) {
  if (!cfg || B <= 0 || L <= 0 || packed_rows <= 0) return 0;
  return workspace_bytes(cfg, B, L, packed_rows);
}

extern "C" int om_encoder_packed_supported(const OmEncoderConfig* c, int gated_ffn, int64_t B, int64_t L, int64_t packed_rows) {
  return encoder_packed_ok(c, gated_ffn != 0, B, L, packed_rows, encoder_switches()) ? 1 : 0;
}

extern "C" int om_debug_encoder_plan(const OmEncoderConfig* c, int gated_ffn, int has_rel_bias, int64_t B, int64_t L, int64_t packed_rows,
                                     int want_hidden) {
  if (!c) {
    om_set_error("om_debug_encoder_plan: null argument");
    return -1;
  }
  const EncPlan p = encoder_plan(EncPlanIn{c, B, L, packed_rows, want_hidden != 0, gated_ffn != 0, has_rel_bias != 0, c->type_vocab > 0},
                                 encoder_switches());
  if (p.error) {
    om_set_error(std::string("om_debug_encoder_plan: ") + p.error);
    return -1;
  }
  return p.path | (int)p.few_rows << 8 | (int)p.two << 9 | p.lo8 << 10;
}

extern "C" int om_debug_encoder_skip_pad(const OmEncoderConfig* c, int gated_ffn, int has_rel_bias, int64_t B, int64_t L, int want_hidden) {
  if (!c) {
    om_set_error("om_debug_encoder_skip_pad: null argument");
    return -1;
  }
  const EncPlanIn in = {c, B, L, 0, want_hidden != 0, gated_ffn != 0, has_rel_bias != 0, c->type_vocab > 0};
  const EncSwitches sw = encoder_switches();
  return encoder_skip_pad(in, encoder_plan(in, sw), sw) ? 1 : 0;
}

extern "C" int om_debug_encoder_cls_tail(const OmEncoderConfig* c, int gated_ffn, int has_rel_bias, int64_t B, int64_t L, int64_t packed_rows,
                                         int want_hidden) {
  if (!c) {
    om_set_error("om_debug_encoder_cls_tail: null argument");
    return -1;
  }
  const EncPlanIn in = {c, B, L, packed_rows, want_hidden != 0, gated_ffn != 0, has_rel_bias != 0, c->type_vocab > 0};
  const EncSwitches sw = encoder_switches();
  return encoder_cls_tail(in, encoder_plan(in, sw), sw) ? 1 : 0;
}

extern "C" int om_t5_relative_bucket(int relative_position, int num_buckets, int max_distance) {
  int nb = num_buckets / 2;
  int bucket = relative_position > 0 ? nb : 0;
  const int n = relative_position < 0 ? -relative_position : relative_position;
  const int max_exact = nb / 2;
  if (n < max_exact) return bucket + n;
  const double v = log((double)n / max_exact) / log((double)max_distance / max_exact) * (nb - max_exact);
  int large = max_exact + (int)v;
  if (large > nb - 1) large = nb - 1;
  return bucket + large;
}

static int check_cfg(const OmEncoderConfig* c) {
  if (const char* why = encoder_cfg_error(c)) OM_FAIL(why);
  return 0;
}

struct EncCall {
  const OmEncoderConfig* c;
  const OmEncoderWeights* w;
  const int64_t* mask;
  int64_t B, L;
  const EncPlan& p;
  const EncWs& ws;
  const float* posbias;
  const int* cu;
  const int* row_map;
  void* out_hidden;
  hipStream_t s;
  const int* rows_dev;
  int64_t cls_mc;
  std::vector<int>* families;
  int64_t whole_mg, whole_mc;
};

struct EncStream {
  const void* x;
  const void* x_lo;
  int lo8;
  const float *g, *b;
  int rms;
  void* spare;
  char* hidden;
  const float* rows32;
  bool cls_compact;
};

#define GEMM(A_, lda_, W_, ldw_, C_, ldc_, N_, K_, bias_, res_, ldr_, act_)                        \
  do {                                                                                             \
    if (om_gemm_nt(dt, A_, lda_, W_, ldw_, dt, C_, ldc_, Mg, N_, K_, bias_, res_, ldr_, act_, s)) \
      return 1;                                                                                    \
  } while (0)
#define RUN(expr) do { if (expr) return 1; } while (0)
#define ENC_LOCALS                                                                                                   \
  const OmEncoderConfig* c = k.c; const EncWs& ws = k.ws; const OmLayerWeights* Ls = k.w->layers_host; hipStream_t s = k.s;     \
  const int dt = c->dtype, H = c->hidden, F = c->ffn, nh = c->n_heads;                                              \
  const int64_t B = k.B, L = k.L, M = k.p.M, Mg = k.p.Mg
#define NOMIC_LOCALS                                                                                                 \
  const bool nomic = c->arch == OM_ARCH_NOMICBERT;                                                                   \
  const int F1 = enc_ffn1_cols(c), act1 = nomic ? OM_ACT_NONE : c->act;                                             \
  const void* const ffa = nomic ? ws.ff2 : ws.ff
#define NOMIC_ROPE() do { if (nomic) RUN(omk_rope(dt, ws.qkv, M, (int)L, H, c->rope_theta_global, s, k.row_map)); } while (0)
#define NOMIC_SWIGLU(rows_) do { if (nomic) RUN(omk_swiglu_rows(dt, ws.ff, ws.ff2, rows_, F, s)); } while (0)

static int bert_fused(const EncCall& k, EncStream* out) {
  ENC_LOCALS;
  NOMIC_LOCALS;
  const float scale = 1.0f / sqrtf((float)c->head_dim);
  const float inv_h = 1.0f / (float)H;
  const bool two = k.p.two;
  const int lo8 = k.p.lo8;
  const int nslots = 2 * (H / 256);
  const bool pingpong = k.p.pingpong;
  int walk = 1;
  const bool probe = k.families != nullptr;
  auto gemm = [&](const void* A, int64_t lda, const void* W, int64_t ldw, void* C, int64_t ldc, int64_t rows, int64_t N, int64_t K,
                  const GemmEpilogue& ep) {
    const int64_t as = rows == Mg ? k.whole_mg : k.whole_mc;
    if (!probe) return omk_gemm(dt, A, lda, W, ldw, dt, C, ldc, rows, N, K, ep, s, as);
    k.families->push_back(omk_gemm_family(dt, A, lda, W, ldw, dt, C, ldc, rows, N, K, ep, as));
    return 0;
  };
#define LAUNCH(expr) do { if (!probe) RUN(expr); } while (0)
  const int64_t Mc = k.cls_mc;
  const size_t cplane = (size_t)Mc * H * 2;
  char* const cbase = ws.qkv;
  float* const cst2p = (float*)(cbase + 7 * cplane);
  float* const cst1 = cst2p + 2 * Mc;
  if (Mc > 0 && ((char*)(cst1 + 2 * Mc) > ws.qkv + (size_t)Mg * 3 * H * 2 || Mc > Mg || c->n_layers < 2 || lo8))
    OM_FAIL("[CLS] tail: the compact buffers do not fit the qkv area");
#define OM_WALK() (pingpong ? (walk ^= 1, walk ^ 1) : 0)
  for (int l = 0; l < c->n_layers; ++l) {
    const OmLayerWeights& lw = Ls[l];
    const bool last = l == c->n_layers - 1, tail = last && Mc > 0;
    float* st1 = tail ? cst1 : ws.stats1 + (size_t)l * Mg * 2;
    float* st2 = ws.stats2 + (size_t)l * Mg * 2;
    const float* st2p = l ? ws.stats2 + (size_t)(l - 1) * Mg * 2 : nullptr;
    const int64_t Mr = tail ? Mc : Mg;
    const int* const rdev = tail ? nullptr : k.rows_dev;
    const char *ctx = ws.ctx, *xin = ws.x1, *xin_lo = ws.x1_lo;
    char *y = ws.y, *y_lo = ws.y_lo, *xout = ws.x1, *xout_lo = ws.x1_lo;
    GemmEpilogue e = {};
    if (l == 0) {
      e.bias = lw.qkv_b; e.reverse = OM_WALK(); e.rows_dev = k.rows_dev;
      RUN(gemm(ws.x, H, lw.qkv_w, H, ws.qkv, 3 * H, Mg, 3 * H, H, e));
    } else {
      const OmLayerWeights& pw = Ls[l - 1];
      const void* wf; const float *cs, *bfp;
      RUN(folded_weights(c, k.w, l, false, lw.qkv_w, pw.ln2_g, pw.ln2_b, lw.qkv_b, 3 * H, H, ws.wfold, ws.colsum, ws.bfold, s, &wf, &cs, &bfp));
      e.bias = bfp; e.ln_stats = st2p; e.ln_colsum = cs; e.ln_inv_h = inv_h; e.ln_eps = c->ln_eps; e.reverse = OM_WALK(); e.rows_dev = k.rows_dev;
      RUN(gemm(ws.x1, H, wf, H, ws.qkv, 3 * H, Mg, 3 * H, H, e));
    }
    if (!probe) NOMIC_ROPE();
    const int attn_walk = OM_WALK();
    LAUNCH(omk_attention(dt, ws.qkv, ws.ctx, k.mask, k.posbias, B, (int)L, H, nh, scale, 0.f, 0, s, attn_walk, ws.kmax, k.cu));
    if (tail) {
      const GatherPlane planes[3] = {{ws.ctx, cbase}, {ws.x1, cbase + cplane}, {two ? ws.x1_lo : nullptr, cbase + 2 * cplane}};
      LAUNCH(omk_gather_rows(planes, st2p, cst2p, k.cu ? ws.cls_rows : nullptr, B, L, Mc, H, s));
      ctx = cbase; xin = cbase + cplane; xin_lo = cbase + 2 * cplane; st2p = cst2p;
      y = cbase + 3 * cplane; y_lo = cbase + 4 * cplane; xout = cbase + 5 * cplane; xout_lo = cbase + 6 * cplane;
    }
    e = GemmEpilogue{};
    e.bias = lw.o_b; e.ldr = H; e.stats_out = ws.slots; e.ln_inv_h = inv_h; e.ln_eps = c->ln_eps;
    if (two) { e.out_lo = y_lo; e.lo8 = lo8; }
    if (l == 0) {
      e.resid = ws.x;
    } else {
      const OmLayerWeights& pw = Ls[l - 1];
      e.resid = xin; e.rln_stats = st2p; e.rln_g = pw.ln2_g; e.rln_b = pw.ln2_b;
      if (two) e.resid_lo = xin_lo;
    }
    e.reverse = OM_WALK(); e.rows_dev = rdev;
    RUN(gemm(ctx, H, lw.o_w, H, y, H, Mr, H, H, e));
    LAUNCH(omk_ln_stats_reduce(ws.slots, nslots, Mr, st1, s));
    const void* wf1; const float *cs1, *bf1;
    RUN(folded_weights(c, k.w, l, true, lw.ffn1_w, lw.ln1_g, lw.ln1_b, lw.ffn1_b, F1, H, ws.wfold, ws.colsum, ws.bfold, s, &wf1, &cs1, &bf1));
    e = GemmEpilogue{};
    e.bias = bf1; e.act = act1; e.ln_stats = st1; e.ln_colsum = cs1; e.ln_inv_h = inv_h; e.ln_eps = c->ln_eps;
    e.reverse = OM_WALK(); e.rows_dev = rdev;
    RUN(gemm(y, H, wf1, H, ws.ff, F1, Mr, F1, H, e));
    if (!probe) NOMIC_SWIGLU(Mr);
    e = GemmEpilogue{};
    e.bias = lw.ffn2_b; e.resid = y; e.ldr = H; e.rln_stats = st1; e.rln_g = lw.ln1_g; e.rln_b = lw.ln1_b;
    e.stats_out = ws.slots; e.ln_inv_h = inv_h; e.ln_eps = c->ln_eps;
    if (two) { e.resid_lo = y_lo; e.out_lo = xout_lo; e.lo8 = lo8; }
    e.reverse = OM_WALK(); e.rows_dev = rdev;
    RUN(gemm(ffa, F, lw.ffn2_w, F, xout, H, Mr, H, F, e));
    if (!last) LAUNCH(omk_ln_stats_reduce(ws.slots, nslots, Mg, st2, s));
  }
#undef LAUNCH
#undef OM_WALK
  const OmLayerWeights& lastw = Ls[c->n_layers - 1];
  *out = EncStream{ws.x1, two ? ws.x1_lo : nullptr, lo8, lastw.ln2_g, lastw.ln2_b, 0, ws.x};
  if (Mc > 0) { out->x = cbase + 5 * cplane; out->x_lo = two ? cbase + 6 * cplane : nullptr; out->cls_compact = true; }
  return 0;
}

static int bert_pending_ln(const EncCall& k, EncStream* out) {
  ENC_LOCALS;
  NOMIC_LOCALS;
  const float scale = 1.0f / sqrtf((float)c->head_dim);
  float* const y_a = ws.y32;
  float* const y_b = ws.r32b;
  for (int l = 0; l < c->n_layers; ++l) {
    const OmLayerWeights& lw = Ls[l];
    float* const st1 = ws.stats1 + (size_t)l * M * 2;
    float* const st2p = l ? ws.stats2 + (size_t)(l - 1) * M * 2 : nullptr;
    GemmEpilogue e = {};
    e.bias = lw.qkv_b; e.ln_eps = c->ln_eps;
    if (l) { e.a_ln32 = y_b; e.a_ln_g = Ls[l - 1].ln2_g; e.a_ln_b = Ls[l - 1].ln2_b; e.a_ln_stats_out = st2p; }
    RUN(omk_gemm(dt, ws.x, H, lw.qkv_w, H, dt, ws.qkv, 3 * H, Mg, 3 * H, H, e, s));
    NOMIC_ROPE();
    RUN(omk_attention(dt, ws.qkv, ws.ctx, k.mask, k.posbias, B, (int)L, H, nh, scale, 0.f, 0, s, 0, ws.kmax));
    e = GemmEpilogue{};
    e.bias = lw.o_b; e.ldr = H; e.out32 = y_a; e.ln_eps = c->ln_eps;
    if (l) { e.rln32 = y_b; e.rln32_stats = st2p; e.rln_g = Ls[l - 1].ln2_g; e.rln_b = Ls[l - 1].ln2_b; }
    else e.resid32 = ws.r32a;
    RUN(omk_gemm(dt, ws.ctx, H, lw.o_w, H, dt, ws.y, H, Mg, H, H, e, s));
    e = GemmEpilogue{};
    e.bias = lw.ffn1_b; e.act = act1; e.ln_eps = c->ln_eps;
    e.a_ln32 = y_a; e.a_ln_g = lw.ln1_g; e.a_ln_b = lw.ln1_b; e.a_ln_stats_out = st1;
    RUN(omk_gemm(dt, ws.x1, H, lw.ffn1_w, H, dt, ws.ff, F1, Mg, F1, H, e, s));
    NOMIC_SWIGLU(Mg);
    e = GemmEpilogue{};
    e.bias = lw.ffn2_b; e.ldr = H; e.out32 = y_b; e.ln_eps = c->ln_eps;
    e.rln32 = y_a; e.rln32_stats = st1; e.rln_g = lw.ln1_g; e.rln_b = lw.ln1_b;
    RUN(omk_gemm(dt, ffa, F, lw.ffn2_w, F, dt, ws.y, H, Mg, H, F, e, s));
  }
  const OmLayerWeights& last = Ls[c->n_layers - 1];
  void* dst = k.out_hidden ? k.out_hidden : (void*)ws.x;
  RUN(omk_layernorm_dual(dt, y_b, H, dst, ws.r32a, H, last.ln2_g, last.ln2_b, M, H, c->ln_eps, s));
  *out = EncStream{};
  out->hidden = (char*)dst; out->rows32 = ws.r32a;
  return 0;
}

static int bert_few32(const EncCall& k, EncStream* out) {
  ENC_LOCALS;
  NOMIC_LOCALS;
  const float scale = 1.0f / sqrtf((float)c->head_dim);
  void* dst = ws.x;
  for (int l = 0; l < c->n_layers; ++l) {
    const OmLayerWeights& lw = Ls[l];
    GEMM(ws.x, H, lw.qkv_w, H, ws.qkv, 3 * H, 3 * H, H, lw.qkv_b, nullptr, 0, OM_ACT_NONE);
    NOMIC_ROPE();
    RUN(omk_attention(dt, ws.qkv, ws.ctx, k.mask, k.posbias, B, (int)L, H, nh, scale, 0.f, 0, s, 0, ws.kmax));
    GemmEpilogue e = {};
    e.bias = lw.o_b; e.resid32 = ws.r32a; e.ldr = H; e.out32 = ws.y32;
    RUN(omk_gemm(dt, ws.ctx, H, lw.o_w, H, dt, ws.y, H, Mg, H, H, e, s));
    RUN(omk_layernorm_dual(dt, ws.y32, H, ws.x1, ws.r32b, H, lw.ln1_g, lw.ln1_b, M, H, c->ln_eps, s));
    GEMM(ws.x1, H, lw.ffn1_w, H, ws.ff, F1, F1, H, lw.ffn1_b, nullptr, 0, act1);
    NOMIC_SWIGLU(Mg);
    e = GemmEpilogue{};
    e.bias = lw.ffn2_b; e.resid32 = ws.r32b; e.ldr = H; e.out32 = ws.y32;
    RUN(omk_gemm(dt, ffa, F, lw.ffn2_w, F, dt, ws.y, H, Mg, H, F, e, s));
    if (l == c->n_layers - 1 && k.out_hidden) dst = k.out_hidden;
    RUN(omk_layernorm_dual(dt, ws.y32, H, dst, ws.r32a, H, lw.ln2_g, lw.ln2_b, M, H, c->ln_eps, s));
  }
  *out = EncStream{};
  out->hidden = (char*)dst; out->rows32 = ws.r32a;
  return 0;
}

static int bert_plain(const EncCall& k, EncStream* out) {
  ENC_LOCALS;
  NOMIC_LOCALS;
  const float scale = 1.0f / sqrtf((float)c->head_dim);
  for (int l = 0; l < c->n_layers; ++l) {
    const OmLayerWeights& lw = Ls[l];
    if (l) RUN(omk_layernorm(dt, ws.y, H, ws.x, H, Ls[l - 1].ln2_g, Ls[l - 1].ln2_b, M, H, c->ln_eps, 0, s));
    GEMM(ws.x, H, lw.qkv_w, H, ws.qkv, 3 * H, 3 * H, H, lw.qkv_b, nullptr, 0, OM_ACT_NONE);
    NOMIC_ROPE();
    RUN(omk_attention(dt, ws.qkv, ws.ctx, k.mask, k.posbias, B, (int)L, H, nh, scale, 0.f, 0, s, 0, ws.kmax));
    GEMM(ws.ctx, H, lw.o_w, H, ws.y, H, H, H, lw.o_b, ws.x, H, OM_ACT_NONE);
    RUN(omk_layernorm(dt, ws.y, H, ws.x1, H, lw.ln1_g, lw.ln1_b, M, H, c->ln_eps, 0, s));
    GEMM(ws.x1, H, lw.ffn1_w, H, ws.ff, F1, F1, H, lw.ffn1_b, nullptr, 0, act1);
    NOMIC_SWIGLU(Mg);
    GEMM(ffa, F, lw.ffn2_w, F, ws.y, H, H, F, lw.ffn2_b, ws.x1, H, OM_ACT_NONE);
  }
  *out = EncStream{};
  if (c->n_layers > 0) *out = EncStream{ws.y, nullptr, 0, Ls[c->n_layers - 1].ln2_g, Ls[c->n_layers - 1].ln2_b, 0, ws.x};
  else out->hidden = ws.x;
  return 0;
}

static int modernbert(const EncCall& k, EncStream* out) {
  ENC_LOCALS;
  const float scale = 1.0f / sqrtf((float)c->head_dim);
  for (int l = 0; l < c->n_layers; ++l) {
    const OmLayerWeights& lw = Ls[l];
    if (!lw.ffn1g_w) OM_FAIL("ModernBERT layers need the gate half of Wi (ffn1g_w)");
    const void* a_in = ws.x;
    if (lw.ln1_g) {
      RUN(omk_layernorm(dt, ws.x, H, ws.y, H, lw.ln1_g, lw.ln1_b, M, H, c->ln_eps, 0, s));
      a_in = ws.y;
    }
    GEMM(a_in, H, lw.qkv_w, H, ws.qkv, 3 * H, 3 * H, H, lw.qkv_b, nullptr, 0, OM_ACT_NONE);
    const bool sliding = ((c->sliding_layers >> l) & 1) != 0;
    RUN(omk_rope(dt, ws.qkv, M, (int)L, H, sliding ? c->rope_theta_local : c->rope_theta_global, s));
    RUN(omk_attention(dt, ws.qkv, ws.ctx, k.mask, nullptr, B, (int)L, H, nh, scale, 0.f, 0, s, 0, ws.kmax, nullptr, sliding ? c->half_window : 0));
    GEMM(ws.ctx, H, lw.o_w, H, ws.x, H, H, H, lw.o_b, ws.x, H, OM_ACT_NONE);
    RUN(omk_layernorm(dt, ws.x, H, ws.y, H, lw.ln2_g, lw.ln2_b, M, H, c->ln_eps, 0, s));
    GEMM(ws.y, H, lw.ffn1g_w, H, ws.ff2, F, F, H, nullptr, nullptr, 0, OM_ACT_NONE);
    GEMM(ws.y, H, lw.ffn1_w, H, ws.ff, F, F, H, lw.ffn1_b, ws.ff2, F, c->act | OM_ACT_MUL_RESID);
    GEMM(ws.ff, F, lw.ffn2_w, F, ws.x, H, H, F, lw.ffn2_b, ws.x, H, OM_ACT_NONE);
  }
  *out = EncStream{ws.x, nullptr, 0, k.w->final_ln_g, k.w->final_ln_b, 0, ws.y};
  return 0;
}

static int t5_fused(const EncCall& k, EncStream* out) {
  ENC_LOCALS;
  const float inv_h = 1.0f / (float)H;
  const int nslots = 2 * (H / 256);
  auto folded = [&](int layer_, bool ffn1_, const void* A_, const void* W_, const float* g_, const float* stats_, void* C_, int N_, int act_,
                    const void* res_, int64_t ldr_) -> int {
    const void* wf; const float *cs, *bfp;
    if (folded_weights(c, k.w, layer_, ffn1_, W_, g_, nullptr, nullptr, N_, H, ws.wfold, ws.colsum, ws.bfold, s, &wf, &cs, &bfp)) return 1;
    (void)cs; (void)bfp;
    GemmEpilogue e = {};
    e.act = act_; e.resid = res_; e.ldr = ldr_;
    e.ln_stats = stats_; e.ln_rms = 1; e.ln_inv_h = inv_h; e.ln_eps = c->ln_eps; e.rows_dev = k.rows_dev;
    return omk_gemm(dt, A_, H, wf, H, dt, C_, N_, Mg, N_, H, e, s);
  };
  for (int l = 0; l < c->n_layers; ++l) {
    const OmLayerWeights& lw = Ls[l];
    float* st1 = ws.stats1 + (size_t)l * Mg * 2;
    float* st2 = ws.stats2 + (size_t)l * Mg * 2;
    if (l == 0) {
      RUN(omk_layernorm(dt, ws.x, H, ws.y, H, lw.ln1_g, nullptr, M, H, c->ln_eps, 1, s));
      GemmEpilogue e0 = {};
      e0.rows_dev = k.rows_dev;
      RUN(omk_gemm(dt, ws.y, H, lw.qkv_w, H, dt, ws.qkv, 3 * H, Mg, 3 * H, H, e0, s));
    } else {
      RUN(folded(l, false, ws.x, lw.qkv_w, lw.ln1_g, ws.stats2 + (size_t)(l - 1) * Mg * 2, ws.qkv, 3 * H, OM_ACT_NONE, nullptr, 0));
    }
    RUN(omk_attention(dt, ws.qkv, ws.ctx, k.mask, k.posbias, B, (int)L, H, nh, 1.0f, 0.f, 0, s, 0, ws.kmax, k.cu));
    GemmEpilogue e = {};
    e.resid = ws.x; e.ldr = H; e.stats_out = ws.slots; e.ln_inv_h = inv_h; e.ln_eps = c->ln_eps; e.rows_dev = k.rows_dev;
    RUN(omk_gemm(dt, ws.ctx, H, lw.o_w, H, dt, ws.x, H, Mg, H, H, e, s));
    RUN(omk_ln_stats_reduce(ws.slots, nslots, Mg, st1, s));
    RUN(folded(l, true, ws.x, lw.ffn1_w, lw.ln2_g, st1, ws.ff, F, c->act, nullptr, 0));
    e = GemmEpilogue{};
    e.resid = ws.x; e.ldr = H; e.stats_out = ws.slots; e.ln_inv_h = inv_h; e.ln_eps = c->ln_eps; e.rows_dev = k.rows_dev;
    RUN(omk_gemm(dt, ws.ff, F, lw.ffn2_w, F, dt, ws.x, H, Mg, H, F, e, s));
    RUN(omk_ln_stats_reduce(ws.slots, nslots, Mg, st2, s));
  }
  *out = EncStream{ws.x, nullptr, 0, k.w->final_ln_g, nullptr, 1, ws.y};
  return 0;
}

static int t5_plain(const EncCall& k, EncStream* out) {
  ENC_LOCALS;
  for (int l = 0; l < c->n_layers; ++l) {
    const OmLayerWeights& lw = Ls[l];
    RUN(omk_layernorm(dt, ws.x, H, ws.y, H, lw.ln1_g, nullptr, M, H, c->ln_eps, 1, s));
    GEMM(ws.y, H, lw.qkv_w, H, ws.qkv, 3 * H, 3 * H, H, nullptr, nullptr, 0, OM_ACT_NONE);
    RUN(omk_attention(dt, ws.qkv, ws.ctx, k.mask, k.posbias, B, (int)L, H, nh, 1.0f, 0.f, 0, s, 0, ws.kmax));
    GEMM(ws.ctx, H, lw.o_w, H, ws.x, H, H, H, nullptr, ws.x, H, OM_ACT_NONE);
    RUN(omk_layernorm(dt, ws.x, H, ws.y, H, lw.ln2_g, nullptr, M, H, c->ln_eps, 1, s));
    if (lw.ffn1g_w) {
      GEMM(ws.y, H, lw.ffn1g_w, H, ws.ff2, F, F, H, nullptr, nullptr, 0, OM_ACT_NONE);
      GEMM(ws.y, H, lw.ffn1_w, H, ws.ff, F, F, H, nullptr, ws.ff2, F, c->act | OM_ACT_MUL_RESID);
    } else {
      GEMM(ws.y, H, lw.ffn1_w, H, ws.ff, F, F, H, nullptr, nullptr, 0, c->act);
    }
    GEMM(ws.ff, F, lw.ffn2_w, F, ws.x, H, H, F, nullptr, ws.x, H, OM_ACT_NONE);
  }
  *out = EncStream{ws.x, nullptr, 0, k.w->final_ln_g, nullptr, 1, ws.y};
  return 0;
}

static int final_norm(const EncCall& k, const EncStream& n, char** hidden, const float** rows32, int64_t* n32) {
  const OmEncoderConfig* c = k.c; const EncWs& ws = k.ws; hipStream_t s = k.s;
  const int dt = c->dtype, H = c->hidden;
  const int64_t B = k.B, L = k.L, M = k.p.M;
  const bool pooled32 = dt != OM_F32 && c->pooling != OM_POOL_NONE;
  *hidden = n.hidden; *rows32 = ws.final32; *n32 = 0;
  if (!n.x) {
    if (n.rows32 && c->pooling != OM_POOL_NONE) { *rows32 = n.rows32; *n32 = M; }
    return 0;
  }
  if (k.out_hidden || !pooled32) {
    void* dst = k.out_hidden ? k.out_hidden : n.spare;
    RUN(omk_layernorm(dt, n.x, H, dst, H, n.g, n.b, M, H, c->ln_eps, n.rms, s, n.x_lo, n.lo8));
    *hidden = (char*)dst;
  }
  if (pooled32 && c->pooling == OM_POOL_FIRST) {
    const int* rows = k.cu && !n.cls_compact ? ws.cls_rows : nullptr;
    RUN(omk_layernorm_f32out(dt, n.x, rows || n.cls_compact ? H : L * H, ws.final32, H, n.g, n.b, B, H, c->ln_eps, n.rms, s, n.x_lo, rows, n.lo8));
    *n32 = B;
  } else if (pooled32) {
    RUN(omk_layernorm_f32out(dt, n.x, H, ws.final32, H, n.g, n.b, M, H, c->ln_eps, n.rms, s, n.x_lo, nullptr, n.lo8));
    *n32 = M;
  }
  return 0;
}

int omk_pooled_tail(const OmEncoderConfig* c, const OmEncoderWeights* w, const float* pooled, float* out_reps, int64_t B, const int* cu,
                    int64_t packed_rows, hipStream_t s) {
  int D = c->hidden;
  if (c->head_in > 0 && w->head_w) {
    D = c->head_out;
    RUN(om_gemm_nt(OM_F32, pooled, c->hidden, w->head_w, c->head_in, OM_F32, out_reps, D, B, D, c->head_in, nullptr, nullptr, 0, OM_ACT_NONE, s));
  }
  if (c->normalize) RUN(omk_l2norm(out_reps, out_reps, B, D, s));
  if (cu) RUN(omk_pack_overflow_poison(cu, B, packed_rows, out_reps, B * (int64_t)D, s));
  return 0;
}

static int skip_pad_buffer(hipStream_t s, size_t ints, int** out) {
  struct Buf { int* p = nullptr; size_t n = 0; bool captured = false; };
  static std::mutex mu;
  static std::map<std::pair<int, hipStream_t>, Buf> bufs;
  *out = nullptr;
  int dev = 0;
  OM_HIP(hipGetDevice(&dev));
  hipStreamCaptureStatus st = hipStreamCaptureStatusNone;
  if (hipStreamIsCapturing(s, &st) != hipSuccess) {
    (void)hipGetLastError();
    return 0;
  }
  const bool capturing = st != hipStreamCaptureStatusNone;
  std::lock_guard<std::mutex> lk(mu);
  Buf& b = bufs[std::make_pair(dev, s)];
  if (b.n < ints) {
    if (capturing) return 0;
    if (b.p && !b.captured) { OM_HIP(hipDeviceSynchronize()); OM_HIP(hipFree(b.p)); }
    b = Buf{};
    OM_HIP(hipMalloc(&b.p, ints * sizeof(int)));
    b.n = ints;
  }
  b.captured |= capturing;
  *out = b.p;
  return 0;
}

struct EncChain {
  const OmEncoderConfig* c;
  const OmEncoderWeights* w;
  const int64_t *input_ids, *attention_mask, *token_type_ids;
  void* out_hidden;
  float* out_reps;
  EncPlanIn in;
  EncPlan plan;
  EncSwitches sw;
  EncWs ws;
  hipStream_t s;
  int* side;
  int64_t whole_mg, whole_mc;
};

static EncWs lane_view(const OmEncoderConfig* c, const EncWs& w, const EncPlan& lane, int h, int64_t B0, int64_t L) {
  const size_t H = c->hidden, F = c->ffn, F1 = enc_ffn1_cols(c), es = 2;
  const size_t row0 = h ? (size_t)(B0 * L) : 0, seq0 = h ? (size_t)B0 : 0;
  EncWs v = {};
  v.x = w.x + row0 * H * es; v.y = w.y + row0 * H * es; v.x1 = w.x1 + row0 * H * es;
  v.qkv = w.qkv + row0 * 3 * H * es;
  v.ctx = w.ctx + row0 * H * es;
  v.ff = w.ff + row0 * F1 * es;
  v.ff2 = c->arch == OM_ARCH_NOMICBERT ? w.ff2 + row0 * F * es : w.ff2;
  v.y_lo = w.y_lo + row0 * H * es; v.x1_lo = w.x1_lo + row0 * H * es;
  v.pooled = w.pooled + seq0 * H;
  v.headout = w.headout + seq0 * (size_t)(c->head_out > 0 ? c->head_out : 1);
  v.kmax = w.kmax + seq0;
  v.final32 = w.final32 + (c->pooling == OM_POOL_FIRST ? seq0 : row0) * H;
  v.stats1 = w.stats1 + 4 * (size_t)c->n_layers * row0;
  v.stats2 = v.stats1 + (size_t)c->n_layers * (size_t)lane.Mg * 2;
  v.slots = w.slots + 4 * ((H + 255) / 256) * row0;
  v.total = w.total;
  return v;
}

static void lane_ranges(const OmEncoderConfig* c, const EncWs& v, const EncPlan& lane, int64_t Bh, const char* base, int64_t* out) {
  const size_t H = c->hidden, F = c->ffn, F1 = enc_ffn1_cols(c), es = 2, M = (size_t)lane.Mp, B = (size_t)Bh;
  const bool nomic = c->arch == OM_ARCH_NOMICBERT;
  const std::pair<const void*, size_t> f[OM_ENCODER_LANE_RANGES] = {
      {v.x, M * H * es}, {v.y, M * H * es}, {v.x1, M * H * es}, {v.qkv, M * 3 * H * es}, {v.ctx, M * H * es}, {v.ff, M * F1 * es},
      {v.ff2, nomic ? M * F * es : 0}, {v.pooled, B * H * 4}, {v.headout, B * (size_t)(c->head_out > 0 ? c->head_out : 1) * 4}, {v.kmax, B * 4},
      {v.final32, (c->pooling == OM_POOL_FIRST ? B : (size_t)lane.M) * H * 4}, {v.stats1, (size_t)2 * c->n_layers * M * 8},
      {v.slots, (size_t)2 * ((H + 255) / 256) * M * 8}, {v.y_lo, M * H * es}, {v.x1_lo, M * H * es}};
  for (int i = 0; i < OM_ENCODER_LANE_RANGES; ++i) {
    out[2 * i] = (int64_t)((const char*)f[i].first - base);
    out[2 * i + 1] = (int64_t)f[i].second;
  }
}

extern "C" int om_debug_encoder_lanes(const OmEncoderConfig* c, int gated_ffn, int has_rel_bias, int64_t B, int64_t L, int64_t packed_rows,
                                      int want_hidden, int64_t* B0) {
  if (!c) {
    om_set_error("om_debug_encoder_lanes: null argument");
    return -1;
  }
  const EncPlanIn in = {c, B, L, packed_rows, want_hidden != 0, gated_ffn != 0, has_rel_bias != 0, c->type_vocab > 0};
  const EncSwitches sw = encoder_switches();
  return encoder_lanes(in, encoder_plan(in, sw), sw, B0) ? 1 : 0;
}

extern "C" int om_debug_encoder_lane_ranges(const OmEncoderConfig* c, int gated_ffn, int has_rel_bias, int64_t B, int64_t L, int lane,
                                            int64_t* out, int cap) {
  if (!c || !out || cap < 2 * OM_ENCODER_LANE_RANGES || (lane != 0 && lane != 1)) {
    om_set_error("om_debug_encoder_lane_ranges: null argument, a lane other than 0 | 1, or room for fewer than 15 pairs");
    return -1;
  }
  EncPlanIn in = {c, B, L, 0, false, gated_ffn != 0, has_rel_bias != 0, c->type_vocab > 0};
  const EncSwitches sw = encoder_switches();
  const EncPlan whole = encoder_plan(in, sw);
  int64_t B0 = 0;
  if (!encoder_lanes(in, whole, sw, &B0)) {
    om_set_error("om_debug_encoder_lane_ranges: this call does not fork (om_debug_encoder_lanes)");
    return -1;
  }
  static char origin[1];
  const EncWs ws = carve(c, whole, B, L, 0, origin);
  in.B = lane ? B - B0 : B0;
  const EncPlan lp = encoder_plan_checked(in, sw);
  lane_ranges(c, lane_view(c, ws, lp, lane, B0, L), lp, in.B, origin, out);
  return OM_ENCODER_LANE_RANGES;
}

static std::atomic<int64_t> g_lane_forks{0};
extern "C" int64_t om_debug_encoder_lane_forks(void) { return g_lane_forks.load(); }

struct LaneStream { hipStream_t side = nullptr; hipEvent_t fork = nullptr, join = nullptr; };
static int lane_stream(hipStream_t s, LaneStream* out) {
  static std::mutex mu;
  static std::map<std::pair<int, hipStream_t>, LaneStream> lanes;
  int dev = 0;
  OM_HIP(hipGetDevice(&dev));
  std::lock_guard<std::mutex> lk(mu);
  LaneStream& l = lanes[std::make_pair(dev, s)];
  if (!l.side) {
    LaneStream n;
    OM_HIP(hipStreamCreateWithFlags(&n.side, hipStreamNonBlocking));
    OM_HIP(hipEventCreateWithFlags(&n.fork, hipEventDisableTiming));
    OM_HIP(hipEventCreateWithFlags(&n.join, hipEventDisableTiming));
    l = n;
  }
  *out = l;
  return 0;
}

static int encoder_chain(const EncChain& q, std::vector<int>* families);

static int encoder_fork(const EncChain& whole, int* forked) {
  *forked = 0;
  const OmEncoderConfig* c = whole.c;
  const int64_t B = whole.in.B, L = whole.in.L;
  int64_t B0 = 0;
  if (!whole.w->folded || om_timing_on() || !encoder_lanes(whole.in, whole.plan, whole.sw, &B0)) return 0;
  hipStreamCaptureStatus st = hipStreamCaptureStatusNone;
  if (hipStreamIsCapturing(whole.s, &st) != hipSuccess) {
    (void)hipGetLastError();
    return 0;
  }
  if (st != hipStreamCaptureStatusNone) return 0;
  LaneStream ls;
  RUN(lane_stream(whole.s, &ls));
  const bool skip = encoder_skip_pad(whole.in, whole.plan, whole.sw);
  int64_t whole_mc = 0;
  if (!encoder_cls_tail(whole.in, whole.plan, whole.sw, &whole_mc)) whole_mc = 0;
  const int64_t D =c->head_in > 0 && whole.w->head_w ? c->head_out : c->hidden;
  EncChain lane[2] = {whole, whole};
  for (int h = 0; h < 2; ++h) {
    EncChain& q = lane[h];
    const int64_t seq0 = h ? B0 : 0;
    q.in.B = h ? B - B0 : B0;
    q.plan = encoder_plan_checked(q.in, q.sw);
    q.ws = lane_view(c, whole.ws, q.plan, h, B0, L);
    q.input_ids += seq0 * L; q.attention_mask += seq0 * L;
    if (q.token_type_ids) q.token_type_ids += seq0 * L;
    q.out_reps += seq0 * D;
    if (h) q.s = ls.side;
    q.whole_mg = whole.plan.Mg; q.whole_mc = whole_mc;
    q.side = nullptr;
    if (skip) {
      RUN(skip_pad_buffer(q.s, (size_t)(q.plan.Mp + 2 * q.in.B + 2), &q.side));
      if (!q.side) return 0;
    }
  }
  if (lane[0].plan.Mp != B0 * L || lane[0].plan.Mp + lane[1].plan.Mp != whole.plan.Mp) return 0;
  EncChain ask = whole;
  ask.side = lane[0].side;
  std::vector<int> fam_whole, fam_lane[2];
  if (encoder_chain(ask, &fam_whole) || encoder_chain(lane[0], &fam_lane[0]) || encoder_chain(lane[1], &fam_lane[1])) return 0;
  if (fam_lane[0] != fam_whole || fam_lane[1] != fam_whole || std::find_if(fam_whole.begin(), fam_whole.end(), [](int f) { return f <= 0; }) != fam_whole.end())
    return 0;

  OM_HIP(hipEventRecord(ls.fork, whole.s));
  OM_HIP(hipStreamWaitEvent(ls.side, ls.fork, 0));
  *forked = 1;
  g_lane_forks.fetch_add(1);
  int rc = encoder_chain(lane[0], nullptr);
  if (!rc) rc = encoder_chain(lane[1], nullptr);
  hipError_t e = hipEventRecord(ls.join, ls.side);
  if (e == hipSuccess) e = hipStreamWaitEvent(whole.s, ls.join, 0);
  if (e != hipSuccess) {
    (void)hipStreamSynchronize(ls.side);
    if (!rc) OM_FAIL(std::string("encoder lanes: join failed: ") + hipGetErrorString(e));
  }
  return rc;
}

static int encoder_forward_impl(const OmEncoderConfig* c, const OmEncoderWeights* w,
                                const int64_t* input_ids, const int64_t* attention_mask,
                                const int64_t* token_type_ids, int64_t B, int64_t L,
                                void* out_hidden, float* out_reps, void* workspace,
                                size_t workspace_bytes, void* stream, int64_t packed_rows) {
  if (!c || !w || !input_ids || !attention_mask) OM_FAIL("null argument");
  if (check_cfg(c)) return 1;
  if (B <= 0) return 0;
  const OmLayerWeights* Ls = w->layers_host;
  if (!Ls) OM_FAIL("layers_host is null");
  const EncPlanIn plan_in = {c, B, L, packed_rows, out_hidden != nullptr, c->n_layers > 0 && Ls[0].ffn1g_w != nullptr, w->rel_bias != nullptr,
                             w->type_emb != nullptr};
  const EncSwitches sw = encoder_switches();
  const EncPlan plan = encoder_plan_checked(plan_in, sw);
  if (om_option(OM_OPT_ENCODER_DEBUG) && plan.path && enc_bert_family(c))
    fprintf(stderr, "om_encoder_forward: M=%ld fused_ln=%d packed=%d few_rows=%d pending_ln=%d L=%ld head_dim=%d rel_bias=%d\n", (long)plan.M,
            (int)(plan.path == OM_ENC_PATH_BERT_FUSED), (int)(packed_rows > 0), (int)plan.few_rows, (int)(plan.path == OM_ENC_PATH_BERT_PENDING_LN), (long)L,
            c->head_dim, (int)plan.rel_bias);
  if (om_option(OM_OPT_ENCODER_DEBUG) && plan.path && c->arch == OM_ARCH_T5)
    fprintf(stderr, "om_encoder_forward (t5): M=%ld fused_norm=%d packed=%d\n", (long)plan.M, (int)(plan.path == OM_ENC_PATH_T5_FUSED), (int)(packed_rows > 0));
  if (plan.error) OM_FAIL(plan.error);
  if (c->arch == OM_ARCH_T5 && !w->final_ln_g) OM_FAIL("T5 needs rel_bias and final_ln_g");
  if (c->arch == OM_ARCH_MODERNBERT && (!w->emb_ln_g || !w->final_ln_g)) OM_FAIL("ModernBERT needs emb_ln_g and final_ln_g");
  if (c->arch == OM_ARCH_NOMICBERT && (!w->type_emb || w->pos_emb || w->rel_bias)) OM_FAIL("NomicBERT needs type_emb and takes no pos_emb or rel_bias");
  if (!workspace || ((uintptr_t)workspace & 255)) OM_FAIL("workspace must be 256-byte aligned");
  EncChain whole = {c, w, input_ids, attention_mask, token_type_ids, out_hidden, out_reps, plan_in, plan, sw,
                    carve(c, plan, B, L, packed_rows, (char*)workspace), (hipStream_t)stream, nullptr, 0, 0};
  if (whole.ws.total > workspace_bytes) OM_FAIL("workspace too small");
  if (c->pooling != OM_POOL_NONE && !out_reps) OM_FAIL("out_reps required when pooling is set");
  int forked = 0;
  RUN(encoder_fork(whole, &forked));
  if (forked) return 0;
  if (encoder_skip_pad(plan_in, plan, sw)) RUN(skip_pad_buffer(whole.s, (size_t)(plan.Mp + 2 * B + 2), &whole.side));
  return encoder_chain(whole, nullptr);
}

static int encoder_chain(const EncChain& q, std::vector<int>* families) {
  const OmEncoderConfig* c = q.c; const OmEncoderWeights* w = q.w;
  const int64_t *input_ids = q.input_ids, *attention_mask = q.attention_mask, *token_type_ids = q.token_type_ids;
  void* const out_hidden = q.out_hidden; float* const out_reps = q.out_reps;
  const EncPlanIn& plan_in = q.in; const EncPlan& plan = q.plan; const EncSwitches sw = q.sw;
  const int64_t B = q.in.B, L = q.in.L, packed_rows = q.in.packed_rows;
  const bool bert = enc_bert_family(c);
  EncWs ws = q.ws;
  hipStream_t s = q.s;
  const int dt = c->dtype, H = c->hidden;
  const int64_t M = plan.M;
  int64_t pack_bound = packed_rows;
  const bool skip = q.side != nullptr;
  if (skip) {
    pack_bound = plan.Mp;
    ws.cu = q.side; ws.cls_rows = q.side + (B + 2); ws.row_map = ws.cls_rows + B;
  }
  const bool packed = pack_bound > 0;
  int64_t cls_mc = 0;
  if (!encoder_cls_tail(plan_in, plan, sw, &cls_mc)) cls_mc = 0;
  const int* const row_map = packed ? ws.row_map : nullptr;
  if (families) {
    if (plan.path != OM_ENC_PATH_BERT_FUSED) OM_FAIL("encoder lanes: the fused BERT path only");
    const EncCall k = {c, w, attention_mask, B, L, plan, ws, nullptr, packed ? ws.cu : nullptr, row_map, out_hidden, s, skip ? ws.cu + B : nullptr,
                       cls_mc, families, q.whole_mg, q.whole_mc};
    EncStream unused = {};
    RUN(bert_fused(k, &unused));
    if (c->head_in > 0 && w->head_w)
      families->push_back(omk_gemm_family(OM_F32, ws.pooled, c->hidden, w->head_w, c->head_in, OM_F32, out_reps, c->head_out, B, c->head_out,
                                          c->head_in, GemmEpilogue{}));
    return 0;
  }

  RUN(omk_mask_extent(attention_mask, B, (int)L, ws.kmax, s));
  if (packed) RUN(omk_pack_rows(ws.kmax, B, (int)L, pack_bound, ws.cu, ws.cls_rows, ws.row_map, s));
  if (plan.rel_bias) {
    const int* lut = nullptr;
    RUN(om_t5_lut_device((int)L, c->rel_buckets, c->rel_max_dist, &lut));
    RUN(omk_t5_bias(w->rel_bias, lut, ws.posbias, (int)L, c->n_heads, s));
  }
  const bool few32 = plan.path == OM_ENC_PATH_BERT_FEW32 || plan.path == OM_ENC_PATH_BERT_PENDING_LN;
  if (bert)
    RUN(omk_embed(dt, input_ids, token_type_ids, w->word_emb, w->pos_emb, w->type_emb, w->emb_ln_g, w->emb_ln_b, ws.x, M, (int)L, H,
                  c->vocab, c->type_vocab, c->ln_eps, 1, s, row_map, few32 ? ws.r32a : nullptr));
  else if (c->arch == OM_ARCH_MODERNBERT)
    RUN(omk_embed(dt, input_ids, nullptr, w->word_emb, nullptr, nullptr, w->emb_ln_g, w->emb_ln_b, ws.x, M, (int)L, H, c->vocab, 1, c->ln_eps, 1, s));
  else
    RUN(omk_embed(dt, input_ids, nullptr, w->word_emb, nullptr, nullptr, nullptr, nullptr, ws.x, M, (int)L, H, c->vocab, 1, c->ln_eps, 0, s, row_map));

  const EncCall k = {c, w, attention_mask, B, L, plan, ws, plan.rel_bias ? ws.posbias : nullptr, packed ? ws.cu : nullptr, row_map, out_hidden, s,
                     skip ? ws.cu + B : nullptr, cls_mc, nullptr, q.whole_mg, q.whole_mc};
  EncStream stream_out = {};
  switch (plan.path) {
    case OM_ENC_PATH_BERT_FUSED: RUN(bert_fused(k, &stream_out)); break;
    case OM_ENC_PATH_BERT_PENDING_LN: RUN(bert_pending_ln(k, &stream_out)); break;
    case OM_ENC_PATH_BERT_FEW32: RUN(bert_few32(k, &stream_out)); break;
    case OM_ENC_PATH_BERT_PLAIN: RUN(bert_plain(k, &stream_out)); break;
    case OM_ENC_PATH_MODERNBERT: RUN(modernbert(k, &stream_out)); break;
    case OM_ENC_PATH_T5_FUSED: RUN(t5_fused(k, &stream_out)); break;
    case OM_ENC_PATH_T5_PLAIN: RUN(t5_plain(k, &stream_out)); break;
    default: OM_FAIL("no path planned");
  }
  char* final_hidden;
  const float* f32_rows;
  int64_t final32_rows;
  RUN(final_norm(k, stream_out, &final_hidden, &f32_rows, &final32_rows));

  if (c->pooling != OM_POOL_NONE) {
    float* pooled = c->head_in > 0 && w->head_w ? ws.pooled : out_reps;
    if (final32_rows == B && c->pooling == OM_POOL_FIRST && (f32_rows == ws.final32 || L == 1))
      OM_HIP(hipMemcpyAsync(pooled, f32_rows, (size_t)B * H * 4, hipMemcpyDeviceToDevice, s));
    else if (final32_rows == M)
      RUN(omk_pool(OM_F32, f32_rows, attention_mask, pooled, B, (int)L, H, c->pooling, s, k.cu));
    else
      RUN(omk_pool(dt, final_hidden, attention_mask, pooled, B, (int)L, H, c->pooling, s));
    RUN(omk_pooled_tail(c, w, pooled, out_reps, B, k.cu, pack_bound, s));
  }
  return 0;
}
#undef NOMIC_SWIGLU
#undef NOMIC_ROPE
#undef NOMIC_LOCALS
#undef ENC_LOCALS
#undef GEMM
#undef RUN

extern "C" int om_encoder_forward(const OmEncoderConfig* c, const OmEncoderWeights* w,
                                  const int64_t* input_ids, const int64_t* attention_mask,
                                  const int64_t* token_type_ids, int64_t B, int64_t L,
                                  void* out_hidden, float* out_reps, void* workspace,
                                  size_t workspace_bytes, void* stream) {
  return encoder_forward_impl(c, w, input_ids, attention_mask, token_type_ids, B, L, out_hidden, out_reps, workspace, workspace_bytes, stream, 0);
}

extern "C" int om_encoder_forward_packed(const OmEncoderConfig* c, const OmEncoderWeights* w,
                                         const int64_t* input_ids, const int64_t* attention_mask,
                                         const int64_t* token_type_ids, int64_t B, int64_t L, int64_t packed_rows,
                                         float* out_reps, void* workspace, size_t workspace_bytes, void* stream) {
  if (packed_rows <= 0) OM_FAIL("packed_rows must be positive");
  return encoder_forward_impl(c, w, input_ids, attention_mask, token_type_ids, B, L, nullptr, out_reps, workspace, workspace_bytes, stream, packed_rows);
}
```

### openmatch_amd/csrc/encoder_plan.h

```cpp
#pragma once
#include <algorithm>

#include "kernels.h"

bool omk_gemm_skinny_ok(int in_dtype, int out_dtype, int64_t M, int64_t N, int64_t K, const GemmEpilogue& ep, int max_m);

struct EncSwitches {
  int fused_ln;
  int two_plane;
  int pingpong;
  int skinny_m;
  int few_ln_fuse;
  int attention_fast;
  int skip_pad;
  int cls_tail;
  int lanes;
};

static EncSwitches encoder_switches() {
  return EncSwitches{om_option(OM_OPT_ENCODER_FUSED_LN), om_option(OM_OPT_ENCODER_TWO_PLANE), om_option(OM_OPT_ENCODER_PINGPONG),
                     om_option(OM_OPT_GEMM_SKINNY_M), om_option(OM_OPT_FEW_ROWS_LN_FUSE), om_option(OM_OPT_ATTENTION_FAST),
                     om_option(OM_OPT_ENCODER_SKIP_PAD), om_option(OM_OPT_ENCODER_CLS_TAIL), om_option(OM_OPT_ENCODER_LANES)};
}

struct EncPlanIn {
  const OmEncoderConfig* c;
  int64_t B, L, packed_rows;
  bool want_hidden;
  bool gated_ffn, has_rel_bias, has_type_emb;
};

struct EncPlan {
  int path;
  const char* error;
  int64_t M;
  int64_t Mp;
  int64_t Mg;
  bool few_rows;
  bool two;
  int lo8;
  bool pingpong;
  bool rel_bias;
  bool alloc_few32;
};

static const char* encoder_cfg_error(const OmEncoderConfig* c) {
  if (c->dtype != OM_F32 && c->dtype != OM_BF16 && c->dtype != OM_F16) return "dtype must be OM_F32, OM_BF16 or OM_F16";
  if (c->dtype == OM_F16 && c->arch == OM_ARCH_BERT && c->act != OM_ACT_GELU_ERF) return "float16 mode: erf-GELU BERT-family encoders only";
  if (c->dtype == OM_F16 && c->arch == OM_ARCH_T5 && c->act != OM_ACT_RELU && c->act != OM_ACT_GELU_TANH)
    return "float16 mode: T5 feed-forwards with ReLU or tanh-GELU only";
  if (c->arch != OM_ARCH_BERT && c->arch != OM_ARCH_T5 && c->arch != OM_ARCH_MODERNBERT && c->arch != OM_ARCH_NOMICBERT) return "unknown arch";
  if (c->arch == OM_ARCH_NOMICBERT) {
    if (c->head_dim != 64 || c->n_heads * 64 != c->hidden) return "NomicBERT: only head_dim 64 with n_heads*64 == hidden is supported";
    if (c->act != OM_ACT_SILU) return "NomicBERT: hidden_act must be \"silu\"";
    if (!(c->rope_theta_global > 0.f)) return "NomicBERT: a positive rope theta";
    if (c->rel_buckets != 0) return "NomicBERT: no relative position bias (rel_buckets must be 0)";
    if (c->hidden % 64 || c->ffn % 64 || c->ffn < 64) return "NomicBERT: hidden and ffn must be multiples of 64";
  }
  if (c->arch == OM_ARCH_MODERNBERT) {
    if (c->head_dim != 64 || c->n_heads * 64 != c->hidden) return "ModernBERT: only head_dim 64 with n_heads*64 == hidden is supported";
    if (c->act != OM_ACT_GELU_ERF) return "ModernBERT: hidden_activation must be \"gelu\" (erf)";
    if (c->n_layers > 64) return "ModernBERT: at most 64 layers";
    if (!(c->rope_theta_global > 0.f) || !(c->rope_theta_local > 0.f) || c->half_window < 0)
      return "ModernBERT: positive rope thetas and a non-negative half window";
  }
  if (c->arch == OM_ARCH_T5 && (c->head_dim != 64 || c->n_heads * 64 != c->hidden))
    return "T5 encoders: only d_kv 64 with n_heads*64 == d_model is supported";
  if ((c->head_dim != 32 && c->head_dim != 64) || c->n_heads * c->head_dim != c->hidden)
    return "head_dim must be 32 or 64 with n_heads*head_dim == hidden";
  if (c->arch == OM_ARCH_BERT && c->rel_buckets != 0 && (c->rel_buckets < 4 || c->rel_buckets % 2 || c->rel_max_dist <= c->rel_buckets / 4))
    return "relative position bias: an even number of buckets >= 4 and a maximum distance beyond the exact buckets";
  const int es = c->dtype == OM_F32 ? 4 : 2;
  if ((c->hidden * es) % 128 || (c->ffn * es) % 128) return "hidden/ffn rows must be multiples of 128 bytes";
  if (c->head_in > 0 && ((c->head_in * 4) % 128 || c->head_in != c->hidden)) return "head_in must equal hidden";
  return nullptr;
}

static inline bool enc_bert_family(const OmEncoderConfig* c) { return c->arch == OM_ARCH_BERT || c->arch == OM_ARCH_NOMICBERT; }
static inline int enc_ffn1_cols(const OmEncoderConfig* c) { return c->arch == OM_ARCH_NOMICBERT ? 2 * c->ffn : c->ffn; }

static bool enc_ln_fusable(int dt, int64_t rows, int H, int F, int F1) {
  return omk_gemm_ln_fusable(dt, rows, H, H) && omk_gemm_ln_fusable(dt, rows, F1, H) && omk_gemm_ln_fusable(dt, rows, 3 * H, H) &&
         omk_gemm_ln_fusable(dt, rows, H, F);
}

static bool enc_pending_ln_ok(int dt, int64_t M, int H, int F, int F1, int act, int max_m) {
  static const float one = 1.f;
  GemmEpilogue a = {}, r = {};
  a.a_ln32 = &one; a.a_ln_g = &one; a.a_ln_b = &one;
  r.rln32 = &one; r.rln32_stats = &one; r.rln_g = &one; r.rln_b = &one; r.out32 = const_cast<float*>(&one);
  GemmEpilogue f = a;
  f.act = act;
  return omk_gemm_skinny_ok(dt, dt, M, 3 * (int64_t)H, H, a, max_m) && omk_gemm_skinny_ok(dt, dt, M, F1, H, f, max_m) &&
         omk_gemm_skinny_ok(dt, dt, M, H, H, r, max_m) && omk_gemm_skinny_ok(dt, dt, M, H, F, r, max_m);
}

static EncPlan encoder_plan_checked(const EncPlanIn& in, const EncSwitches sw) {
  const OmEncoderConfig* c = in.c;
  EncPlan p = {};
  auto run = [&](int path) { p.path = path; return p; };
  auto refuse = [&](const char* why) { p.error = why; return p; };
  const int dt = c->dtype, H = c->hidden, F = c->ffn, F1 = enc_ffn1_cols(c);
  const bool half = dt == OM_BF16 || dt == OM_F16, packed = in.packed_rows > 0, bert = enc_bert_family(c), nomic = c->arch == OM_ARCH_NOMICBERT;
  p.M = packed ? in.packed_rows : in.B * in.L;
  p.Mp = half && p.M >= 512 ? (p.M + 255) / 256 * 256 : p.M;
  p.alloc_few32 = half && bert && !packed && p.M <= (int64_t)std::max(0, sw.skinny_m);
  if (in.B <= 0) return p;
  if (in.L < 1 || in.L > 1024) return refuse("sequence length must be in [1,1024]");
  if (packed) {
    if (dt == OM_F32 || in.want_hidden || c->pooling == OM_POOL_NONE || c->n_layers < 1)
      return refuse("packed rows: 16-bit inference that returns representations only");
    if (in.packed_rows % 256 || in.packed_rows < 512 || in.packed_rows > in.B * in.L + 255)
      return refuse("packed_rows: a multiple of 256 in [512, B * L + 255]");
  }
  p.few_rows = !packed && half && p.M <= (int64_t)sw.skinny_m && !(dt == OM_BF16 && bert && p.M >= 512 && (sw.two_plane & 1) != 0);
  p.Mg = p.few_rows ? p.M : p.Mp;
  const bool fusable = sw.fused_ln != 0 && !p.few_rows && c->n_layers > 0 && H % 8 == 0 && enc_ln_fusable(dt, p.Mg, H, F, F1);
  if (c->arch == OM_ARCH_MODERNBERT) {
    if (packed) return refuse("packed rows: not for ModernBERT (om_encoder_packed_supported is 0)");
    return run(OM_ENC_PATH_MODERNBERT);
  }
  if (!bert) {
    if (!in.has_rel_bias) return refuse("T5 needs rel_bias and final_ln_g");
    p.rel_bias = true;
    p.path = fusable && !in.gated_ffn ? OM_ENC_PATH_T5_FUSED : OM_ENC_PATH_T5_PLAIN;
    if (packed && p.path != OM_ENC_PATH_T5_FUSED) return refuse("packed rows need the fused 16-bit path (T5: widths of 256, no gated feed-forward)");
    return p;
  }
  if (in.L > c->max_pos) return refuse(nomic ? "NomicBERT: sequence longer than max_pos (max_position_embeddings)" : "sequence longer than the position table");
  if (in.has_rel_bias != (c->rel_buckets > 0)) return refuse("relative position bias: rel_bias and rel_buckets must be set together");
  if (in.has_type_emb && c->type_vocab <= 0) return refuse("token types: a type_emb table needs type_vocab > 0");
  p.rel_bias = in.has_rel_bias;
  const bool plane = (sw.two_plane & (dt == OM_BF16 ? 1 : 2)) != 0;
  if (fusable && (c->act == OM_ACT_GELU_ERF || nomic)) {
    p.two = plane;
    p.lo8 = plane && dt == OM_F16 && (sw.two_plane & 4) ? 1 : 0;
    p.pingpong = sw.pingpong != 0;
    return run(OM_ENC_PATH_BERT_FUSED);
  }
  const bool few32 = p.few_rows && c->n_layers > 0 && plane;
  p.path = !few32 ? OM_ENC_PATH_BERT_PLAIN
           : p.M <= (int64_t)sw.few_ln_fuse && enc_pending_ln_ok(dt, p.Mg, H, F, F1, nomic ? OM_ACT_NONE : c->act, sw.skinny_m) ? OM_ENC_PATH_BERT_PENDING_LN
                                                                                                       : OM_ENC_PATH_BERT_FEW32;
  if (packed) return refuse("packed rows need the fused 16-bit path (hidden, ffn multiples of 256; erf-GELU)");
  return p;
}

static EncPlan encoder_plan(const EncPlanIn& in, const EncSwitches sw) {
  if (const char* why = encoder_cfg_error(in.c)) {
    EncPlan p = {};
    p.error = why;
    return p;
  }
  return encoder_plan_checked(in, sw);
}

static bool encoder_packed_ok(const OmEncoderConfig* c, bool gated_ffn, int64_t B, int64_t L, int64_t packed_rows, const EncSwitches sw) {
  if (!c || B <= 0 || packed_rows <= 0) return false;
  if ((c->dtype != OM_BF16 && c->dtype != OM_F16) || (!enc_bert_family(c) && c->arch != OM_ARCH_T5)) return false;
  if (B * L <= (int64_t)sw.skinny_m) return false;
  if (c->dtype == OM_BF16 && !sw.attention_fast) return false;
  if (c->arch == OM_ARCH_T5 && c->dtype == OM_F16 && c->act != OM_ACT_RELU) return false;
  OmEncoderConfig q = *c;
  q.pooling = OM_POOL_FIRST;
  q.max_pos = 1024;
  const bool rel = c->arch == OM_ARCH_T5 || c->rel_buckets > 0;
  const EncPlan p = encoder_plan_checked(EncPlanIn{&q, B, L, packed_rows, false, gated_ffn, rel, false}, sw);
  return p.path && !p.error;
}

static bool encoder_skip_pad(const EncPlanIn& in, const EncPlan& p, const EncSwitches sw) {
  if (!sw.skip_pad || in.packed_rows != 0 || in.want_hidden || in.c->pooling == OM_POOL_NONE) return false;
  if (p.error || (p.path != OM_ENC_PATH_BERT_FUSED && p.path != OM_ENC_PATH_T5_FUSED)) return false;
  return encoder_packed_ok(in.c, in.gated_ffn, in.B, in.L, p.Mp, sw);
}

static bool encoder_cls_tail(const EncPlanIn& in, const EncPlan& p, const EncSwitches sw, int64_t* Mc = nullptr) {
  if (!sw.cls_tail || p.error || p.path != OM_ENC_PATH_BERT_FUSED || p.lo8) return false;
  if (in.c->pooling != OM_POOL_FIRST || in.want_hidden || in.c->n_layers < 2 || in.B < 512) return false;
  const int64_t mc = (in.B + 255) / 256 * 256;
  if (4 * mc > p.Mp) return false;
  if (Mc) *Mc = mc;
  return true;
}

static const int64_t ENC_LANE_ROWS_END = 131072;
static bool encoder_lanes(const EncPlanIn& in, const EncPlan& p, const EncSwitches sw, int64_t* B0 = nullptr) {
  if (sw.lanes <= 0 || in.packed_rows != 0 || in.want_hidden || in.has_rel_bias || in.c->pooling == OM_POOL_NONE) return false;
  if (p.error || p.path != OM_ENC_PATH_BERT_FUSED || p.rel_bias || in.B < 2 || in.L < 1) return false;
  int64_t step = 256;
  for (int64_t l = in.L; step > 1 && l % 2 == 0; l /= 2) step /= 2;
  const int64_t b0 = in.B / 2 / step * step;
  if (b0 <= 0 || b0 * in.L < (int64_t)sw.lanes || (in.B - b0) * in.L < (int64_t)sw.lanes) return false;
  if ((in.B - b0) * in.L >= ENC_LANE_ROWS_END) return false;
  const bool skip = encoder_skip_pad(in, p, sw), tail = encoder_cls_tail(in, p, sw);
  for (const int64_t bh : {b0, in.B - b0}) {
    EncPlanIn li = in;
    li.B = bh;
    const EncPlan lp = encoder_plan_checked(li, sw);
    if (lp.error || lp.path != p.path || lp.two != p.two || lp.lo8 != p.lo8 || lp.pingpong != p.pingpong) return false;
    if (encoder_skip_pad(li, lp, sw) != skip || encoder_cls_tail(li, lp, sw) != tail) return false;
  }
  if (B0) *B0 = b0;
  return true;
}
```

### openmatch_amd/csrc/kernels.h

```cpp
#pragma once
#include "common.h"

int omk_ln_fold(int dtype , const void* W, const float* gamma, const float* beta, const float* b, void* Wf,
                float* colsum, float* bf, int N, int K, hipStream_t s);
int omk_layernorm(int dtype, const void* x, int64_t ldx, void* y, int64_t ldy, const float* g,
                  const float* b, int64_t M, int H, float eps, int rms, hipStream_t s,
                  const void* x_lo = nullptr ,
                  int lo8 = 0 );
int omk_layernorm_dual(int dtype, const float* x, int64_t ldx, void* y, float* y32, int64_t ldy, const float* g, const float* b,
                       int64_t M, int H, float eps, hipStream_t s);
int omk_layernorm_f32out(int dtype, const void* x, int64_t ldx, float* y, int64_t ldy, const float* g, const float* b,
                         int64_t M, int H, float eps, int rms, hipStream_t s, const void* x_lo = nullptr,
                         const int* rows = nullptr ,
                         int lo8 = 0 );
int omk_layernorm_from_f32(int dtype, const float* x, int64_t ldx, void* y, int64_t ldy, const float* g, const float* b, int64_t M, int H,
                           float eps, int rms, hipStream_t s);
int omk_embed(int dtype, const int64_t* ids, const int64_t* type_ids, const float* word,
              const float* pos, const float* type, const float* g, const float* b, void* out,
              int64_t M, int L, int H, int vocab, int type_vocab, float eps, int bert,
              hipStream_t s, const int* row_map = nullptr ,
              float* out32 = nullptr );
int omk_pool(int dtype, const void* x, const int64_t* mask, float* out, int64_t B, int L, int H,
             int mode, hipStream_t s, const int* cu = nullptr );
int omk_l2norm(const float* x, float* y, int64_t M, int D, hipStream_t s);
int omk_swiglu_rows(int dtype, const void* in, void* out, int64_t M, int F, hipStream_t s);
void omk_row_note(int word);
int omk_t5_bias(const float* table, const int* lut, float* out, int L, int heads, hipStream_t s);

int omk_attention(int dtype, const void* qkv, void* ctx, const int64_t* mask,
                  const float* pos_bias, int64_t B, int L, int H, int heads, float scale,
                  float drop_p, uint64_t seed, hipStream_t s, int reverse = 0 ,
                  const int* kmax = nullptr ,
                  const int* cu = nullptr ,
                  int w = 0 );
struct AttnPlan;
int omk_attention_d32(const AttnPlan& p, int dtype, const void* qkv, void* ctx, const int64_t* mask, const float* pos_bias, int64_t B, int L,
                      int H, int heads, float scale, float drop_p, uint64_t seed, hipStream_t s, int reverse, const int* kmax, const int* cu);
int omk_rope(int dtype, void* qkv, int64_t M, int L, int H, float theta, hipStream_t s,
             const int* row_map = nullptr );
int omk_attention_band(int dtype, const void* qkv, void* ctx, const int64_t* mask, int64_t B, int L, int H, int heads, float scale,
                       int w, const int* kmax, hipStream_t s);
int omk_rope_gqa(int dtype, void* qkv, int64_t M, int L, int heads, int kv_heads, const float* inv_freq_host, float scaling, hipStream_t s,
                 const int* row_map = nullptr );
int omk_attention_causal(int dtype, const void* qkv, void* ctx, const int64_t* mask, int64_t B, int L, int heads, int kv_heads, float scale,
                         const int* kmax, hipStream_t s);
int omk_attention_causal_packed(int dtype, const void* qkv, void* ctx, const int64_t* mask, int64_t B, int L, int heads, int kv_heads, float scale,
                                const int* cu, hipStream_t s);
int omk_attention_causal_d128(int dtype, const void* qkv, void* ctx, const int64_t* mask, int64_t B, int L, int heads, int kv_heads, float scale,
                              const int* kmax, hipStream_t s);
int omk_attention_causal_d128_packed(int dtype, const void* qkv, void* ctx, const int64_t* mask, int64_t B, int L, int heads, int kv_heads,
                                     float scale, const int* cu, hipStream_t s);
int omk_qknorm_rope(int dtype, void* qkv, int64_t M, int L, int heads, int kv_heads, int head_dim, const float* q_norm_g, const float* k_norm_g,
                    float eps, const float* inv_freq_host, float scaling, hipStream_t s, const int* row_map = nullptr,
                    int gemma = 0 );
int omk_attention_gqa_d256(int dtype, const void* qkv, void* ctx, const int64_t* mask, int64_t B, int L, int heads, int kv_heads, float scale, int w,
                           const int* kmax, hipStream_t s);
int omk_attention_gqa_d256_packed(int dtype, const void* qkv, void* ctx, const int64_t* mask, int64_t B, int L, int heads, int kv_heads, float scale,
                                  int w, const int* cu, hipStream_t s);
int omk_rmsnorm_add(int dtype, const void* h, int64_t ldh, float* x, int64_t ldx, const float* g, int64_t M, int H, float eps, hipStream_t s);
int omk_rope_table(const float* inv_freq, int n, float scaling, const float2** out);
int omk_causal_debug_kmax(int64_t B, int** out);
int omk_pack_rows(const int* kmax, int64_t B, int L, int64_t rows, int* cu, int* cls_rows, int* row_map, hipStream_t s);
int omk_pack_overflow_poison(const int* cu, int64_t B, int64_t rows, float* out, int64_t n, hipStream_t s);
int omk_mask_extent(const int64_t* mask, int64_t B, int L, int* kmax, hipStream_t s);
int omk_pooled_tail(const OmEncoderConfig* c, const OmEncoderWeights* w, const float* pooled, float* out_reps, int64_t B, const int* cu,
                    int64_t packed_rows, hipStream_t s);

#define OM_ACT_GELU_ERF_GRAD 4
struct GemmEpilogue {
  const float* bias;
  const void* resid;
  int64_t ldr;
  int act;
  void* pre_act;
  int64_t ldp;
  float drop_p;
  uint64_t seed;
  const int* drop_rows;
  unsigned long long* trace;
  const float* ln_stats;
  const float* ln_colsum;
  const float* rln_stats;
  const float* rln_g;
  const float* rln_b;
  float* stats_out;
  const void* resid_lo;
  void* out_lo;
  const float* resid32;
  float* out32;
  const float* a_ln32;
  const float* a_ln_g;
  const float* a_ln_b;
  float* a_ln_stats_out;
  const float* rln32;
  const float* rln32_stats;
  int lo8;
  float ln_inv_h, ln_eps;
  int ln_rms;
  int reverse;
  const int* rows_dev;
};
__host__ __device__ inline size_t omk_lo8_offset(int64_t m, int64_t n, int64_t N) {
  const int64_t tile = (m >> 8) * (N >> 8) + (n >> 8);
  const int wave = (int)(((m >> 7) & 1) * 2 + ((n >> 7) & 1));
  const int r = (int)(m & 127), c = (int)(n & 127);
  const int P = 2 * (r >> 5) + (c >> 6);
  const int G = 2 * ((r >> 4) & 1) + ((c >> 5) & 1);
  const int lane = ((c >> 2) & 3) * 16 + (r & 15);
  return ((size_t)((tile * 4 + wave) * 8 + P)) * 2048 + (size_t)((G >> 1) * 1024 + lane * 16 + (G & 1) * 8 + ((c >> 4) & 1) * 4 + (c & 3));
}
int omk_ln_stats_reduce(const float* slots, int nslots, int64_t M, float* out, hipStream_t s);
struct GatherPlane { const void* src; void* dst; };
int omk_gather_rows(const GatherPlane (&planes)[3], const float* stats_src, float* stats_dst, const int* rows, int64_t B, int64_t L, int64_t Mc,
                    int H, hipStream_t s);
struct GemmPlan { int family; const char* error; int act ; bool resid, train ; int lnf ; };
inline int gemm_lnf(const GemmEpilogue& ep, bool f16) {
  return ep.ln_stats ? 1 : ((ep.rln_stats || ep.stats_out) ? (ep.out_lo ? (ep.lo8 && f16 ? 4 : 3) : 2) : 0);
}
inline bool gemm_whole_tiles(int64_t M, int64_t N, int64_t K) { return M % 256 == 0 && N % 256 == 0 && (K * 2) % 128 == 0; }
bool omk_gemm_ln_fusable(int dtype, int64_t M, int64_t N, int64_t K);
unsigned long long* omk_debug_trace();
bool omk_gemm_tn_ok(int dtype, int64_t M, int64_t N, int64_t K, int64_t lda, int64_t ldb);
int omk_gemm_tn(int dtype, const void* A, int64_t lda, const void* B, int64_t ldb, float* C, int64_t ldc, float* bias,
                int64_t M, int64_t N, int64_t K, hipStream_t s);
bool omk_gemm_tn_batch_ok(int dtype, int64_t M, int64_t N, int64_t K, int64_t lda, int64_t ldb);
int omk_gemm_tn_batch(int dtype, const OmTnProblem* probs, int n, int64_t M, hipStream_t s);
bool omk_gemm_wide6_b16_has(int in_dtype, int out_dtype, int act, bool train, bool resid);
int omk_gemm_wide6_b16(int in_dtype, const void* A, int64_t lda, const void* B, int64_t ldb, int out_dtype,
                       void* C, int64_t ldc, int64_t M, int64_t N, int64_t K, const GemmEpilogue& ep, hipStream_t s);
bool omk_gemm_wide6_f32_has(int in_dtype, int out_dtype, int act, bool train, bool resid);
int omk_gemm_wide6_f32(int in_dtype, const void* A, int64_t lda, const void* B, int64_t ldb, int out_dtype,
                       void* C, int64_t ldc, int64_t M, int64_t N, int64_t K, const GemmEpilogue& ep, hipStream_t s);
int omk_gemm(int in_dtype, const void* A, int64_t lda, const void* B, int64_t ldb, int out_dtype,
             void* C, int64_t ldc, int64_t M, int64_t N, int64_t K, const GemmEpilogue& ep,
             hipStream_t s, int64_t plan_m = 0);
int omk_gemm_family(int in_dtype, const void* A, int64_t lda, const void* B, int64_t ldb, int out_dtype, const void* C, int64_t ldc, int64_t M,
                    int64_t N, int64_t K, const GemmEpilogue& ep, int64_t plan_m = 0);
void omk_gemm_note(int family);

int omk_gemm_splitk(int in_dtype, const void* A, int64_t lda, const void* B, int64_t ldb, float* C,
                    int64_t ldc, int64_t M, int64_t N, int64_t K, hipStream_t s);

__host__ __device__ inline uint64_t om_hash64(uint64_t seed, uint64_t idx) {
  uint64_t x = idx * 0x9E3779B97F4A7C15ull + seed;
  x ^= x >> 32; x *= 0xD6E8FEB86659FD93ull;
  x ^= x >> 32; x *= 0xD6E8FEB86659FD93ull;
  x ^= x >> 32;
  return x;
}
struct DropCfg {
  uint32_t thresh;
  float keep_scale;
  __host__ __device__ explicit DropCfg(float p) {
    thresh = p > 0.f ? (uint32_t)(p * 65536.0f + 0.5f) : 0u;
    if (thresh > 65535u) thresh = 65535u;
    keep_scale = 65536.0f / (float)(65536u - thresh);
  }
};
__host__ __device__ inline uint64_t dropout_bits(uint64_t seed, uint64_t group) { return om_hash64(seed, group); }
__host__ __device__ inline bool dropout_field(uint64_t bits, int e, uint32_t thresh) {
  return ((uint32_t)(bits >> (16 * e)) & 0xffffu) >= thresh;
}
__host__ __device__ inline bool dropout_keep(uint64_t seed, uint64_t idx, uint32_t thresh) {
  return dropout_field(dropout_bits(seed, idx >> 2), (int)(idx & 3), thresh);
}
```

### openmatch_amd/native.py

```python
import ctypes as C
import os

import torch

_HERE = os.path.dirname(os.path.abspath(__file__))
LIB_PATH = os.path.join(_HERE, "csrc", "libopenmatch_hip.so")

OM_F32, OM_BF16, OM_F16 = 0, 1, 2
ACT_NONE, ACT_GELU_ERF, ACT_RELU, ACT_GELU_TANH = 0, 1, 2, 3
ACT_SILU = 5
ACT_MUL_RESID = 0x100
ACT_GELU_ERF_GRAD, ACT_PRE_GRAD = 4, 0x200
ARCH_BERT, ARCH_T5, ARCH_MODERNBERT, ARCH_CAUSAL, ARCH_NOMICBERT, ARCH_GEMMA3 = 0, 1, 2, 3, 4, 5
POOL_NONE, POOL_FIRST, POOL_MEAN, POOL_LAST = 0, 1, 2, 3
OPT_TRAIN_WGRAD_BATCH, OPT_GEMM_MAX_GRID, OPT_GEMM_CONT = 14, 15, 16
OPT_GEMM_GROUP_M, OPT_GEMM_VARIANT, OPT_GEMM_SKINNY_M = 6, 12, 19
GEMM_FAMILY = {"v1": 1, "v2": 2, "v6": 6, "g7": 7, "g7_one_tile": 70, "7c16": 71, "7r16": 72, "skinny": 9}
ATTN_FAMILY = {"generic": 1, "fwd16": 2, "fwd16_kmax4": 3, "fwd16c": 4, "long": 5, "d32": 6, "band16": 7, "band32": 8}
ATTN_BWD_FAMILY = {"bwd16": 1, "generic": 2, "long": 3, "d32": 4}
ENC_PATH = {"bert_fused": 1, "bert_pending_ln": 2, "bert_few32": 3, "bert_plain": 4, "modernbert": 5, "t5_fused": 6, "t5_plain": 7}
SCAN_FAMILY = {"dense": 0, "generic": 1, "wide": 2, "stream32": 3, "stream16": 4}
SCAN_FAMILY_NAME = {v: k for k, v in SCAN_FAMILY.items()}
OPT_SCAN_GEN7 = 3
OPT_ATTENTION_FAST = 2
SEARCH_F32, SEARCH_F16_RESCORE = 0, 1
ABI_VERSION = 6

c_void_p, c_int, c_int64, c_float, c_size_t = C.c_void_p, C.c_int, C.c_int64, C.c_float, C.c_size_t


class OmLayerWeights(C.Structure):
    _fields_ = [(n, c_void_p) for n in (
        "qkv_w", "qkv_b", "o_w", "o_b", "ln1_g", "ln1_b", "ffn1_w", "ffn1_b", "ffn1g_w",
        "ffn2_w", "ffn2_b", "ln2_g", "ln2_b")]


class OmEncoderConfig(C.Structure):
    _fields_ = [("arch", c_int), ("dtype", c_int), ("hidden", c_int), ("n_layers", c_int),
                ("n_heads", c_int), ("head_dim", c_int), ("ffn", c_int), ("vocab", c_int),
                ("max_pos", c_int), ("type_vocab", c_int), ("act", c_int), ("ln_eps", c_float),
                ("rel_buckets", c_int), ("rel_max_dist", c_int), ("pooling", c_int),
                ("head_in", c_int), ("head_out", c_int), ("normalize", c_int),
                ("rope_theta_global", c_float), ("rope_theta_local", c_float), ("half_window", c_int),
                ("sliding_layers", C.c_uint64)]


class OmCausalConfig(C.Structure):
    _fields_ = [("base", OmEncoderConfig), ("n_kv_heads", c_int), ("rope_attention_scaling", c_float), ("inv_freq", c_float * 32)]


class OmCausalConfig2(C.Structure):
    _fields_ = [("base", OmCausalConfig), ("qk_norm", c_int), ("reserved", c_int), ("inv_freq", c_float * 64)]


class OmCausalQkNorm(C.Structure):
    _fields_ = [("q_norm_g", c_void_p), ("k_norm_g", c_void_p)]


class OmGemma3Config(C.Structure):
    _fields_ = [("base", OmCausalConfig), ("attn_scale", c_float), ("half_window", c_int), ("sliding_layers", C.c_uint64),
                ("full_scaling", c_float), ("sliding_scaling", c_float), ("attn_logit_softcapping", c_float), ("bidirectional", c_int),
                ("full_inv_freq", c_float * 128), ("sliding_inv_freq", c_float * 128)]


class OmGemma3Norms(C.Structure):
    _fields_ = [(n, c_void_p) for n in ("q_norm_g", "k_norm_g", "post_attention_norm_g", "post_feedforward_norm_g")]


class OmEncoderWeights(C.Structure):
    _fields_ = [("word_emb", c_void_p), ("pos_emb", c_void_p), ("type_emb", c_void_p),
                ("emb_ln_g", c_void_p), ("emb_ln_b", c_void_p),
                ("layers_host", C.POINTER(OmLayerWeights)), ("final_ln_g", c_void_p),
                ("rel_bias", c_void_p), ("head_w", c_void_p), ("folded", c_void_p), ("final_ln_b", c_void_p)]


class OmTnProblem(C.Structure):
    _fields_ = [("A", c_void_p), ("B", c_void_p), ("C", c_void_p), ("bias", c_void_p),
                ("lda", c_int64), ("ldb", c_int64), ("ldc", c_int64), ("N", c_int64), ("K", c_int64)]


class OmT5DecoderLayer(C.Structure):
    _fields_ = [(n, c_void_p) for n in (
        "sa_v_w", "sa_o_w", "sa_ln_g", "ca_q_w", "ca_kv_w", "ca_o_w", "ca_ln_g", "ffn1_w", "ffn1g_w", "ffn2_w", "ffn_ln_g")]


class OmT5DecoderWeights(C.Structure):
    _fields_ = [("start_emb", c_void_p), ("final_ln_g", c_void_p),
                ("layers_host", C.POINTER(OmT5DecoderLayer)), ("n_layers", c_int)]


class OmT5DecoderLayerGrads(C.Structure):
    _fields_ = [(n, c_void_p) for n in (
        "sa_v_w", "sa_o_w", "sa_ln_g", "ca_q_w", "ca_kv_w", "ca_o_w", "ca_ln_g", "ffn1_w", "ffn1g_w", "ffn2_w", "ffn_ln_g")]


class OmT5DecoderGrads(C.Structure):
    _fields_ = [("start_emb", c_void_p), ("final_ln_g", c_void_p), ("layers_host", C.POINTER(OmT5DecoderLayerGrads))]


class OmAdamTensor(C.Structure):
    _fields_ = [("p", c_void_p), ("g", c_void_p), ("m", c_void_p), ("v", c_void_p), ("shadow0", c_void_p), ("shadow1", c_void_p),
                ("n", c_int64), ("weight_decay", c_float), ("shadow0_dtype", c_int), ("shadow1_dtype", c_int), ("reserved", c_int)]


class OmDebugGemmEpilogue(C.Structure):
    _fields_ = [("bias", c_void_p), ("resid", c_void_p), ("ldr", c_int64), ("act", c_int),
                ("pre_act", c_void_p), ("ldp", c_int64), ("drop_p", c_float), ("seed", C.c_uint64), ("drop_rows", c_void_p),
                ("ln_stats", c_void_p), ("ln_colsum", c_void_p), ("rln_stats", c_void_p), ("rln_g", c_void_p), ("rln_b", c_void_p),
                ("stats_out", c_void_p), ("resid_lo", c_void_p), ("out_lo", c_void_p), ("resid32", c_void_p), ("out32", c_void_p),
                ("a_ln32", c_void_p), ("a_ln_g", c_void_p), ("a_ln_b", c_void_p), ("a_ln_stats_out", c_void_p), ("rln32", c_void_p),
                ("rln32_stats", c_void_p), ("lo8", c_int), ("ln_inv_h", c_float), ("ln_eps", c_float), ("ln_rms", c_int),
                ("reverse", c_int), ("rows_dev", c_void_p)]


class OmLnSite(C.Structure):
    _fields_ = [("partial", c_void_p), ("dg", c_void_p), ("db", c_void_p), ("blocks", c_int)]


ROW_KERNEL = {"fwd_generic": 1, "fwd_x8": 2, "ln_bwd": 3}
OPT_TRAIN_WGRAD_STREAM = 8
ADAM_CHUNK = 16384


class OmLayerGrads(C.Structure):
    _fields_ = [(n, c_void_p) for n in (
        "qkv_w", "qkv_b", "o_w", "o_b", "ln1_g", "ln1_b", "ffn1_w", "ffn1_b", "ffn2_w", "ffn2_b",
        "ln2_g", "ln2_b", "ffn1g_w")]


class OmEncoderGrads(C.Structure):
    _fields_ = [("word_emb", c_void_p), ("pos_emb", c_void_p), ("type_emb", c_void_p),
                ("emb_ln_g", c_void_p), ("emb_ln_b", c_void_p),
                ("layers_host", C.POINTER(OmLayerGrads)), ("head_w", c_void_p),
                ("final_ln_g", c_void_p), ("rel_bias", c_void_p)]


_SIGNATURES = {
    "om_last_error": (C.c_char_p, []),
    "om_abi_version": (c_int, []),
    "om_device_count": (c_int, []),
    "om_debug_gemm_trace": (None, [c_void_p]),
    "om_debug_gemm_gen": (None, [c_int]),
    "om_debug_option": (c_int, [c_int, c_int]),
    "om_debug_option_value": (c_int, [c_int]),
    "om_debug_gemm_last": (c_int, []),
    "om_debug_gemm_plan": (c_int, [c_int, c_void_p, c_int64, c_void_p, c_int64, c_int, c_void_p, c_int64,
                                   c_int64, c_int64, c_int64, c_void_p, c_void_p, c_int64, c_int]),
    "om_debug_gemm_ex": (c_int, [c_int, c_void_p, c_int64, c_void_p, c_int64, c_int, c_void_p, c_int64,
                                 c_int64, c_int64, c_int64, C.POINTER(OmDebugGemmEpilogue), c_void_p]),
    "om_debug_gemm_plan_ex": (c_int, [c_int, c_void_p, c_int64, c_void_p, c_int64, c_int, c_void_p, c_int64,
                                      c_int64, c_int64, c_int64, C.POINTER(OmDebugGemmEpilogue)]),
    "om_debug_gemm_splitk": (c_int, [c_int, c_void_p, c_int64, c_void_p, c_int64, c_void_p, c_int64, c_int64, c_int64, c_int64, c_void_p]),
    "om_debug_attention": (c_int, [c_void_p, c_void_p, c_void_p, c_int64, c_int, c_int, c_int, c_void_p]),
    "om_debug_attention_ex": (c_int, [c_int, c_void_p, c_void_p, c_void_p, c_void_p, c_int64, c_int, c_int, c_int, c_float, c_float,
                                      C.c_uint64, c_void_p, c_int, c_void_p, c_void_p, c_int]),
    "om_debug_rope": (c_int, [c_int, c_void_p, c_int64, c_int, c_int, c_float, c_void_p]),
    "om_debug_rope_rows": (c_int, [c_int, c_void_p, c_int64, c_int, c_int, c_float, c_void_p, c_void_p]),
    "om_debug_swiglu_rows": (c_int, [c_int, c_void_p, c_void_p, c_int64, c_int, c_void_p]),
    "om_debug_embed": (c_int, [c_int, c_void_p, c_void_p, c_void_p, c_void_p, c_void_p, c_void_p, c_void_p, c_void_p, c_int64, c_int, c_int,
                               c_int, c_int, c_float, c_void_p]),
    "om_debug_attention_causal": (c_int, [c_int, c_void_p, c_void_p, c_void_p, c_int64, c_int, c_int, c_int, c_float, c_void_p]),
    "om_debug_rope_gqa": (c_int, [c_int, c_void_p, c_int64, c_int, c_int, c_int, C.POINTER(c_float), c_float, c_void_p]),
    "om_debug_attention_causal_packed": (c_int, [c_int, c_void_p, c_void_p, c_void_p, c_void_p, c_int64, c_int, c_int, c_int, c_float, c_void_p]),
    "om_debug_rope_gqa_rows": (c_int, [c_int, c_void_p, c_int64, c_int, c_int, c_int, C.POINTER(c_float), c_float, c_void_p, c_void_p]),
    "om_debug_attention_causal_hd": (c_int, [c_int, c_void_p, c_void_p, c_void_p, c_int64, c_int, c_int, c_int, c_int, c_float, c_void_p]),
    "om_debug_attention_causal_hd_packed": (c_int, [c_int, c_void_p, c_void_p, c_void_p, c_void_p, c_int64, c_int, c_int, c_int, c_int, c_float,
                                                    c_void_p]),
    "om_debug_qknorm_rope": (c_int, [c_int, c_void_p, c_int64, c_int, c_int, c_int, c_int, c_void_p, c_void_p, c_float, C.POINTER(c_float),
                                     c_float, c_void_p]),
    "om_debug_qknorm_rope_rows": (c_int, [c_int, c_void_p, c_int64, c_int, c_int, c_int, c_int, c_void_p, c_void_p, c_float, C.POINTER(c_float),
                                          c_float, c_void_p, c_void_p]),
    "om_debug_attention_gqa_d256": (c_int, [c_int, c_void_p, c_void_p, c_void_p, c_int64, c_int, c_int, c_int, c_float, c_int, c_void_p]),
    "om_debug_qknorm_rope_d256": (c_int, [c_int, c_void_p, c_int64, c_int, c_int, c_int, c_void_p, c_void_p, c_float, C.POINTER(c_float), c_float,
                                          c_void_p]),
    "om_debug_attention_gqa_d256_packed": (c_int, [c_int, c_void_p, c_void_p, c_void_p, c_void_p, c_int64, c_int, c_int, c_int, c_float, c_int,
                                                   c_void_p]),
    "om_debug_qknorm_rope_d256_rows": (c_int, [c_int, c_void_p, c_int64, c_int, c_int, c_int, c_void_p, c_void_p, c_float, C.POINTER(c_float),
                                               c_float, c_void_p, c_void_p]),
    "om_debug_rmsnorm_add": (c_int, [c_int, c_void_p, c_int64, c_void_p, c_int64, c_void_p, c_int64, c_int, c_float, c_void_p]),
    "om_debug_mask_extent": (c_int, [c_void_p, c_int64, c_int, c_void_p, c_void_p]),
    "om_debug_pack_rows": (c_int, [c_void_p, c_int64, c_int, c_int64, c_void_p, c_void_p, c_void_p, c_void_p]),
    "om_debug_attention_last": (c_int, []),
    "om_debug_attention_plan": (c_int, [c_int, c_int64, c_int, c_int, c_int, c_int, c_float, c_int, c_int, c_int]),
    "om_debug_attention_bwd_last": (c_int, []),
    "om_debug_attention_bwd_plan": (c_int, [c_int, c_int64, c_int, c_int, c_int, c_int, c_int, c_int, c_int]),
    "om_debug_attention_bwd_ex": (c_int, [c_int, c_void_p, c_void_p, c_void_p, c_void_p, c_void_p, c_void_p, c_void_p, c_void_p, c_int64, c_int,
                                          c_int, c_int, c_float, c_float, C.c_uint64, c_void_p, c_int, c_void_p]),
    "om_debug_attention_bwd_stats_bytes": (c_size_t, [c_int64, c_int]),
    "om_debug_encoder_plan": (c_int, [C.POINTER(OmEncoderConfig), c_int, c_int, c_int64, c_int64, c_int64, c_int]),
    "om_debug_encoder_skip_pad": (c_int, [C.POINTER(OmEncoderConfig), c_int, c_int, c_int64, c_int64, c_int]),
    "om_debug_encoder_cls_tail": (c_int, [C.POINTER(OmEncoderConfig), c_int, c_int, c_int64, c_int64, c_int64, c_int]),
    "om_debug_encoder_lanes": (c_int, [C.POINTER(OmEncoderConfig), c_int, c_int, c_int64, c_int64, c_int64, c_int, C.POINTER(c_int64)]),
    "om_debug_encoder_lane_ranges": (c_int, [C.POINTER(OmEncoderConfig), c_int, c_int, c_int64, c_int64, c_int, C.POINTER(c_int64), c_int]),
    "om_debug_encoder_lane_forks": (c_int64, []),
    "om_debug_gather_rows": (c_int, [c_void_p, c_void_p, c_void_p, c_void_p, c_void_p, c_void_p, c_void_p, c_void_p, c_void_p, c_int64, c_int64,
                                     c_int64, c_int, c_void_p]),
    "om_debug_attn_drop_keep": (c_int, [C.c_uint64, c_int64, c_int, c_int, c_int, c_int, c_int, c_float]),
    "om_debug_wave_sum_check": (c_int, [c_void_p, c_void_p, c_void_p, c_int64, c_void_p]),
    "om_debug_row_kernel_last": (c_int, []),
    "om_debug_layernorm": (c_int, [c_int, c_void_p, c_int64, c_void_p, c_int64, c_void_p, c_void_p, c_int64, c_int, c_float, c_int, c_void_p,
                                   c_int, c_void_p]),
    "om_debug_layernorm_f32out": (c_int, [c_int, c_void_p, c_int64, c_void_p, c_int64, c_void_p, c_void_p, c_int64, c_int, c_float, c_int,
                                          c_void_p, c_void_p, c_int, c_void_p]),
    "om_debug_layernorm_from_f32": (c_int, [c_int, c_void_p, c_int64, c_void_p, c_int64, c_void_p, c_void_p, c_int64, c_int, c_float, c_int,
                                            c_void_p]),
    "om_debug_layernorm_dual": (c_int, [c_int, c_void_p, c_int64, c_void_p, c_void_p, c_int64, c_void_p, c_void_p, c_int64, c_int, c_float,
                                        c_void_p]),
    "om_debug_norm_bwd": (c_int, [c_int, c_void_p, c_void_p, c_void_p, c_void_p, c_void_p, c_void_p, c_int64, c_int, c_float, c_int, c_void_p,
                                  c_void_p]),
    "om_debug_ln_bwd_drop": (c_int, [c_int, c_void_p, c_void_p, c_void_p, c_void_p, c_void_p, c_float, C.c_uint64, c_void_p, c_void_p, c_int64,
                                     c_int, c_float, c_void_p, c_void_p, c_void_p, C.POINTER(c_int), c_void_p, c_void_p]),
    "om_debug_ln_param_reduce": (c_int, [C.POINTER(OmLnSite), c_int, c_int, c_void_p]),
    "om_debug_embed_bwd": (c_int, [c_int, c_void_p, c_void_p, c_void_p, c_void_p, c_void_p, c_void_p, c_void_p, c_void_p, c_void_p, c_void_p,
                                   c_void_p, c_void_p, c_int64, c_int, c_int, c_int, c_int, c_float, c_void_p, c_void_p]),
    "om_debug_pool": (c_int, [c_int, c_void_p, c_void_p, c_void_p, c_int64, c_int, c_int, c_int, c_void_p, c_void_p]),
    "om_debug_pool_bwd": (c_int, [c_int, c_void_p, c_void_p, c_void_p, c_int64, c_int, c_int, c_int, c_void_p, c_void_p]),
    "om_debug_l2norm": (c_int, [c_void_p, c_void_p, c_int64, c_int, c_void_p]),
    "om_debug_l2norm_bwd": (c_int, [c_void_p, c_void_p, c_void_p, c_int64, c_int, c_void_p]),
    "om_debug_colsum": (c_int, [c_int, c_void_p, c_int64, c_int64, c_int, c_void_p, c_void_p]),
    "om_debug_dropout": (c_int, [c_int, c_void_p, c_void_p, c_int64, c_float, C.c_uint64, c_void_p, c_int, c_void_p]),
    "om_debug_ln_fold": (c_int, [c_int, c_void_p, c_void_p, c_void_p, c_void_p, c_void_p, c_void_p, c_void_p, c_int, c_int, c_void_p]),
    "om_debug_ln_stats_reduce": (c_int, [c_void_p, c_int, c_int64, c_void_p, c_void_p]),
    "om_encoder_fold_bytes": (c_size_t, [C.POINTER(OmEncoderConfig)]),
    "om_encoder_fold_weights": (c_int, [C.POINTER(OmEncoderConfig), C.POINTER(OmEncoderWeights), c_void_p, c_size_t, c_void_p]),
    "om_kernel_timing_enable": (c_int, [c_int]),
    "om_kernel_timing_read": (c_int, [c_int, C.POINTER(C.c_double), C.POINTER(c_int64), C.POINTER(C.c_double)]),
    "om_gemm_nt": (c_int, [c_int, c_void_p, c_int64, c_void_p, c_int64, c_int, c_void_p, c_int64,
                           c_int64, c_int64, c_int64, c_void_p, c_void_p, c_int64, c_int, c_void_p]),
    "om_gemm_tn_acc": (c_int, [c_int, c_void_p, c_int64, c_void_p, c_int64, c_void_p, c_int64, c_void_p,
                               c_int64, c_int64, c_int64, c_void_p]),
    "om_gemm_tn_acc_batch": (c_int, [c_int, C.POINTER(OmTnProblem), c_int, c_int64, c_void_p]),
    "om_encoder_workspace_bytes": (c_size_t, [C.POINTER(OmEncoderConfig), c_int64, c_int64]),
    "om_t5_decoder_workspace_bytes": (c_size_t, [C.POINTER(OmEncoderConfig), c_int64, c_int64]),
    "om_t5_decoder_step": (c_int, [C.POINTER(OmEncoderConfig), C.POINTER(OmT5DecoderWeights), c_void_p, c_void_p,
                                   c_int64, c_int64, c_void_p, c_void_p, c_size_t, c_void_p]),
    "om_t5_relative_bucket": (c_int, [c_int, c_int, c_int]),
    "om_encoder_forward": (c_int, [C.POINTER(OmEncoderConfig), C.POINTER(OmEncoderWeights), c_void_p,
                                   c_void_p, c_void_p, c_int64, c_int64, c_void_p, c_void_p,
                                   c_void_p, c_size_t, c_void_p]),
    "om_causal_encoder_workspace_bytes": (c_size_t, [C.POINTER(OmCausalConfig), c_int64, c_int64]),
    "om_causal_encoder_forward": (c_int, [C.POINTER(OmCausalConfig), C.POINTER(OmEncoderWeights), c_void_p, c_void_p, c_int64, c_int64,
                                          c_void_p, c_void_p, c_void_p, c_size_t, c_void_p]),
    "om_causal_encoder_packed_supported": (c_int, [C.POINTER(OmCausalConfig), c_int64, c_int64, c_int64]),
    "om_causal_encoder_workspace_bytes_packed": (c_size_t, [C.POINTER(OmCausalConfig), c_int64, c_int64, c_int64]),
    "om_causal_encoder_forward_packed": (c_int, [C.POINTER(OmCausalConfig), C.POINTER(OmEncoderWeights), c_void_p, c_void_p, c_int64, c_int64,
                                                 c_int64, c_void_p, c_void_p, c_size_t, c_void_p]),
    "om_causal2_encoder_workspace_bytes": (c_size_t, [C.POINTER(OmCausalConfig2), c_int64, c_int64]),
    "om_causal2_encoder_forward": (c_int, [C.POINTER(OmCausalConfig2), C.POINTER(OmEncoderWeights), C.POINTER(OmCausalQkNorm), c_void_p, c_void_p,
                                           c_int64, c_int64, c_void_p, c_void_p, c_void_p, c_size_t, c_void_p]),
    "om_causal2_encoder_packed_supported": (c_int, [C.POINTER(OmCausalConfig2), c_int64, c_int64, c_int64]),
    "om_causal2_encoder_workspace_bytes_packed": (c_size_t, [C.POINTER(OmCausalConfig2), c_int64, c_int64, c_int64]),
    "om_causal2_encoder_forward_packed": (c_int, [C.POINTER(OmCausalConfig2), C.POINTER(OmEncoderWeights), C.POINTER(OmCausalQkNorm), c_void_p,
                                                  c_void_p, c_int64, c_int64, c_int64, c_void_p, c_void_p, c_size_t, c_void_p]),
    "om_gemma3_encoder_workspace_bytes": (c_size_t, [C.POINTER(OmGemma3Config), c_int64, c_int64]),
    "om_gemma3_encoder_forward": (c_int, [C.POINTER(OmGemma3Config), C.POINTER(OmEncoderWeights), C.POINTER(OmGemma3Norms), c_void_p, c_void_p,
                                          c_int64, c_int64, c_void_p, c_void_p, c_void_p, c_size_t, c_void_p]),
    "om_gemma3_encoder_packed_supported": (c_int, [C.POINTER(OmGemma3Config), c_int64, c_int64, c_int64]),
    "om_gemma3_encoder_workspace_bytes_packed": (c_size_t, [C.POINTER(OmGemma3Config), c_int64, c_int64, c_int64]),
    "om_gemma3_encoder_forward_packed": (c_int, [C.POINTER(OmGemma3Config), C.POINTER(OmEncoderWeights), C.POINTER(OmGemma3Norms), c_void_p,
                                                 c_void_p, c_int64, c_int64, c_int64, c_void_p, c_void_p, c_size_t, c_void_p]),
    "om_encoder_packed_supported": (c_int, [C.POINTER(OmEncoderConfig), c_int, c_int64, c_int64, c_int64]),
    "om_encoder_workspace_bytes_packed": (c_size_t, [C.POINTER(OmEncoderConfig), c_int64, c_int64, c_int64]),
    "om_encoder_forward_packed": (c_int, [C.POINTER(OmEncoderConfig), C.POINTER(OmEncoderWeights), c_void_p,
                                          c_void_p, c_void_p, c_int64, c_int64, c_int64, c_void_p,
                                          c_void_p, c_size_t, c_void_p]),
    "om_encoder_tape_bytes": (c_size_t, [C.POINTER(OmEncoderConfig), c_int64, c_int64]),
    "om_encoder_train_workspace_bytes": (c_size_t, [C.POINTER(OmEncoderConfig), c_int64, c_int64]),
    "om_encoder_train_forward": (c_int, [C.POINTER(OmEncoderConfig), C.POINTER(OmEncoderWeights), c_void_p,
                                         c_void_p, c_void_p, c_int64, c_int64, c_float, c_float, C.c_uint64,
                                         c_void_p, c_size_t, c_void_p, c_void_p, c_size_t, c_void_p]),
    "om_encoder_train_backward": (c_int, [C.POINTER(OmEncoderConfig), C.POINTER(OmEncoderWeights), c_void_p,
                                          c_void_p, c_void_p, c_int64, c_int64, c_float, c_float, C.c_uint64,
                                          c_void_p, c_void_p, C.POINTER(OmEncoderGrads), c_void_p, c_size_t,
                                          c_void_p]),
    "om_encoder_train_packed_supported": (c_int, [C.POINTER(OmEncoderConfig), c_int64, c_int64, c_int64]),
    "om_encoder_tape_bytes_packed": (c_size_t, [C.POINTER(OmEncoderConfig), c_int64, c_int64, c_int64]),
    "om_encoder_train_workspace_bytes_packed": (c_size_t, [C.POINTER(OmEncoderConfig), c_int64, c_int64, c_int64]),
    "om_encoder_train_forward_packed": (c_int, [C.POINTER(OmEncoderConfig), C.POINTER(OmEncoderWeights), c_void_p,
                                                c_void_p, c_void_p, c_int64, c_int64, c_int64, c_float, c_float, C.c_uint64,
                                                c_void_p, c_size_t, c_void_p, c_void_p, c_size_t, c_void_p]),
    "om_encoder_train_backward_packed": (c_int, [C.POINTER(OmEncoderConfig), C.POINTER(OmEncoderWeights), c_void_p,
                                                 c_void_p, c_void_p, c_int64, c_int64, c_int64, c_float, c_float, C.c_uint64,
                                                 c_void_p, c_void_p, C.POINTER(OmEncoderGrads), c_void_p, c_size_t,
                                                 c_void_p]),
    "om_encoder_train_forward_hidden": (c_int, [C.POINTER(OmEncoderConfig), C.POINTER(OmEncoderWeights), c_void_p,
                                                c_void_p, c_void_p, c_int64, c_int64, c_float, c_float, C.c_uint64,
                                                c_void_p, c_size_t, c_void_p, c_void_p, c_size_t, c_void_p]),
    "om_encoder_train_backward_hidden": (c_int, [C.POINTER(OmEncoderConfig), C.POINTER(OmEncoderWeights), c_void_p,
                                                 c_void_p, c_void_p, c_int64, c_int64, c_float, c_float, C.c_uint64,
                                                 c_void_p, c_void_p, C.POINTER(OmEncoderGrads), c_void_p, c_size_t,
                                                 c_void_p]),
    "om_t5_decoder_tape_bytes": (c_size_t, [C.POINTER(OmEncoderConfig), c_int, c_int64, c_int64]),
    "om_t5_decoder_train_workspace_bytes": (c_size_t, [C.POINTER(OmEncoderConfig), c_int, c_int64, c_int64]),
    "om_t5_decoder_train_forward": (c_int, [C.POINTER(OmEncoderConfig), C.POINTER(OmT5DecoderWeights), c_void_p, c_void_p,
                                            c_int64, c_int64, c_float, C.c_uint64, c_void_p, c_size_t, c_void_p,
                                            c_void_p, c_size_t, c_void_p]),
    "om_t5_decoder_train_backward": (c_int, [C.POINTER(OmEncoderConfig), C.POINTER(OmT5DecoderWeights), c_void_p, c_void_p,
                                             c_int64, c_int64, c_float, C.c_uint64, c_void_p, c_void_p,
                                             C.POINTER(OmT5DecoderGrads), c_void_p, c_void_p, c_size_t, c_void_p]),
    "om_linear_f32_backward": (c_int, [c_void_p, c_void_p, c_void_p, c_void_p, c_void_p, c_int, c_int, c_int, c_void_p]),
    "om_index_to_f16": (c_int, [c_void_p, c_int64, c_int, c_void_p, c_void_p, c_void_p]),
    "om_sim_topk_workspace_bytes": (c_size_t, [c_int64, c_int, c_int]),
    "om_sim_topk": (c_int, [c_int, c_void_p, c_int64, c_void_p, c_void_p, c_void_p, c_int64, c_int,
                            c_int, c_int64, c_void_p, c_void_p, c_void_p, c_size_t, c_void_p]),
    "om_sim_topk_info": (None, [C.POINTER(c_int64)]),
    "om_debug_scan_plan": (c_int, [c_int, c_int64, c_int, C.POINTER(c_int)]),
    "om_debug_sim_stream": (c_int, [c_void_p, c_int64, C.c_uint32, c_void_p, c_int64, c_int, c_void_p, c_void_p, c_void_p, c_int, c_void_p]),
    "om_topk_merge": (c_int, [c_void_p, c_void_p, c_int, c_int64, c_int, c_int, c_void_p, c_void_p,
                              c_void_p]),
    "om_contrastive_fwd_bwd": (c_int, [c_void_p, c_void_p, c_int, c_int, c_int, c_int, c_float,
                                       c_int, c_int, c_int, c_int, c_void_p, c_void_p, c_void_p,
                                       c_void_p, c_void_p, c_void_p]),
    "om_encoder_train_set_layer_events": (c_int, [c_void_p, c_int]),
    "om_comm_unique_id": (c_int, [c_void_p]),
    "om_comm_init": (c_int, [c_void_p, c_int, c_int, C.POINTER(c_void_p)]),
    "om_comm_destroy": (c_int, [c_void_p]),
    "om_comm_count": (c_int, [c_void_p, C.POINTER(c_int)]),
    "om_allgather_rows": (c_int, [c_void_p, c_void_p, c_void_p, c_int64, c_int64, c_void_p]),
    "om_allreduce_grads": (c_int, [c_void_p, c_void_p, c_int64, c_int, c_void_p]),
    "om_exchange_topk": (c_int, [c_void_p, c_int, c_void_p, c_void_p, c_int64, c_int, c_void_p, c_void_p, c_void_p]),
    "om_grad_sqnorm": (c_int, [c_void_p, c_void_p, c_int, c_void_p, c_void_p, c_void_p]),
    "om_adamw_step": (c_int, [c_void_p, c_void_p, c_int, c_float, c_float, c_float, c_float, c_int64, c_void_p, c_float, c_float,
                              c_int, c_void_p, c_void_p]),
    "om_loss_scale_update": (c_int, [c_void_p, c_void_p, c_int, c_void_p]),
    "om_contrastive_fwd_bwd_ex": (c_int, [c_void_p, c_void_p, c_int, c_int, c_int, c_void_p, c_int, c_int, c_void_p,
                                          c_float, c_int, c_int, c_int, c_int, c_void_p, c_void_p, c_void_p,
                                          c_void_p, c_void_p, c_void_p]),
}

_lib = None


class NativeError(RuntimeError):
    pass


def lib():
    global _lib
    if _lib is None:
        if not os.path.exists(LIB_PATH):
            raise NativeError(
                f"{LIB_PATH} is missing: build the HIP library first "
                "(python -m openmatch_amd._build, or __graft_entry__.build()). "
                "openmatch_amd has no CPU / eager fallback.")
        handle = C.CDLL(LIB_PATH)
        for name, (res, args) in _SIGNATURES.items():
            try:
                fn = getattr(handle, name)
            except AttributeError as e:
                raise NativeError(f"{LIB_PATH} does not export {name}; rebuild it") from e
            fn.restype, fn.argtypes = res, args
        if handle.om_abi_version() != ABI_VERSION:
            raise NativeError("libopenmatch_hip.so ABI version mismatch; rebuild it")
        _lib = handle
    return _lib


def exported_symbols():
    return list(_SIGNATURES)


def check(rc):
    if rc != 0:
        raise NativeError(lib().om_last_error().decode("utf-8", "replace"))


def require_device(*tensors):
    for t in tensors:
        if t is None:
            continue
        if not t.is_cuda:
            raise NativeError(
                "openmatch_amd runs on MI355X only: got a CPU tensor. Move the model and the batch "
                "to the GPU (model.to('cuda')); there is no CPU / eager fallback.")
        if not t.is_contiguous():
            raise NativeError("non-contiguous tensor passed to the HIP boundary")


def ptr(t):
    return c_void_p(t.data_ptr()) if t is not None else c_void_p(0)


def stream_ptr(device=None):
    return c_void_p(torch.cuda.current_stream(device).cuda_stream)


class Workspace:
    _pool = {}

    @classmethod
    def get(cls, device, nbytes, tag="default"):
        key = (str(device), tag)
        buf = cls._pool.get(key)
        if buf is None or buf.numel() - ((-buf.data_ptr()) % 256) < nbytes:
            buf = torch.empty(int(nbytes) + 256, dtype=torch.uint8, device=device)
            cls._pool[key] = buf
        off = (-buf.data_ptr()) % 256
        return buf, buf.data_ptr() + off
```

Measured before the change: 74830 passages/s.

## Compute last-layer attention only for the [CLS] query row

In the last BERT layer, where only the [CLS] output is pooled, the QKV projection is split. K and V are computed for all rows, while Q is computed only for the gathered [CLS] rows. A new attention kernel then runs a single wave per (batch, head) using that one query. This removes the Q third of the last QKV GEMM and most of the last-layer attention work. The cost is extra plan checks, a compact buffer carved from the FFN workspace, and a fallback path whenever the GEMM families do not match.

Result: no change. 75050 passages/s (median of 6 runs) (+0.3%).

```diff
diff --git a/include/openmatch_hip.h b/include/openmatch_hip.h
--- a/include/openmatch_hip.h
+++ b/include/openmatch_hip.h
@@ -100,7 +100,8 @@
 #define OM_OPT_ENCODER_SKIP_PAD 22
 #define OM_OPT_ENCODER_CLS_TAIL 23
 #define OM_OPT_ENCODER_LANES 24
-#define OM_OPT_COUNT 25
+#define OM_OPT_ENCODER_CLS_QUERY 25
+#define OM_OPT_COUNT 26
 int om_debug_option(int opt, int value);
 int om_debug_option_value(int opt);
 int om_debug_attention(const void* qkv, void* ctx, const int64_t* mask, int64_t B, int L, int H, int heads, void* stream);
@@ -171,6 +172,11 @@
 int om_debug_encoder_skip_pad(const struct OmEncoderConfig* cfg, int gated_ffn, int has_rel_bias, int64_t B, int64_t L, int want_hidden);
 int om_debug_encoder_cls_tail(const struct OmEncoderConfig* cfg, int gated_ffn, int has_rel_bias, int64_t B, int64_t L, int64_t packed_rows,
                               int want_hidden);
+int om_debug_encoder_cls_query(const struct OmEncoderConfig* cfg, int gated_ffn, int has_rel_bias, int64_t B, int64_t L, int64_t packed_rows,
+                               int want_hidden);
+int64_t om_debug_encoder_cls_query_chains(void);
+int om_debug_attention_cls(int dtype, const void* qkv, const void* q, void* ctx, const int64_t* mask, int64_t B, int64_t Mc, int L, int H,
+                           int heads, float scale, void* stream, int reverse, const int* kmax, const int* cu);
 int om_debug_encoder_lanes(const struct OmEncoderConfig* cfg, int gated_ffn, int has_rel_bias, int64_t B, int64_t L, int64_t packed_rows,
                            int want_hidden, int64_t* B0);
 #define OM_ENCODER_LANE_RANGES 15
diff --git a/openmatch_amd/csrc/abi.cpp b/openmatch_amd/csrc/abi.cpp
--- a/openmatch_amd/csrc/abi.cpp
+++ b/openmatch_amd/csrc/abi.cpp
@@ -118,6 +118,8 @@
   g_opt[OM_OPT_ENCODER_CLS_TAIL] = e ? atoi(e) : 1;
   e = getenv("OM_ENCODER_LANES");
   g_opt[OM_OPT_ENCODER_LANES] = e ? atoi(e) : 65536;
+  e = getenv("OM_ENCODER_CLS_QUERY");
+  g_opt[OM_OPT_ENCODER_CLS_QUERY] = e ? atoi(e) : 1;
   g_opt_init.store(true);
 }
 }
diff --git a/openmatch_amd/csrc/attention.hip b/openmatch_amd/csrc/attention.hip
--- a/openmatch_amd/csrc/attention.hip
+++ b/openmatch_amd/csrc/attention.hip
@@ -140,18 +140,19 @@
   }
 }
 
-template <typename T, int KT, bool BIAS, bool DROP, int DBG, int KTV>
+template <typename T, int KT, bool BIAS, bool DROP, int DBG, int KTV, bool CLS = false>
 __device__ __forceinline__ void attention_fwd16_body(
     const T* __restrict__ qkv, T* __restrict__ ctx, const int64_t* __restrict__ mask,
     const float* __restrict__ pos_bias, int L, int H, int heads, float scale, float drop_p, uint64_t seed, int rev,
-    int64_t row0, int Lm) {
+    int64_t row0, int Lm,
+    const T* __restrict__ qc = nullptr, T* __restrict__ cc = nullptr, int64_t bcls = 0) {
   typedef typename MmaOps<T>::frag_t frag_t;
   extern __shared__ __attribute__((aligned(16))) char smem[];
   char* const sK = smem;
   char* const sV = smem + KT * 32 * 128;
   float* const sM = (float*)(smem + 2 * KT * 32 * 128);
   const int h = blockIdx.x % heads;
-  const int64_t b = rev ? (int64_t)(gridDim.x / heads) - 1 - blockIdx.x / heads : blockIdx.x / heads;
+  const int64_t b = CLS ? bcls : rev ? (int64_t)(gridDim.x / heads) - 1 - blockIdx.x / heads : blockIdx.x / heads;
   const int tid = threadIdx.x, lane = tid & 63, half = lane >> 5, l31 = lane & 31;
   const int wave = __builtin_amdgcn_readfirstlane(tid >> 6);
   const int64_t ld2 = 6 * (int64_t)H;
@@ -176,10 +177,11 @@
   const int qrow = (q0 + l31) < L ? (q0 + l31) : (L - 1);
   frag_t qf[4];
 #pragma unroll
-  for (int kk = 0; kk < 4; ++kk) qf[kk] = *(const frag_t*)(base + (int64_t)qrow * ld2 + (kk * 2 + half) * 16);
+  for (int kk = 0; kk < 4; ++kk)
+    qf[kk] = CLS ? *(const frag_t*)((const char*)(qc + h * 64) + (kk * 2 + half) * 16) : *(const frag_t*)(base + (int64_t)qrow * ld2 + (kk * 2 + half) * 16);
   asm volatile("s_waitcnt vmcnt(0)" ::: "memory");
   __syncthreads();
-  if (q0 >= L) return;
+  if (CLS ? wave != 0 : q0 >= L) return;
 
   constexpr int KTC = (DBG & 2) ? 0 : KTV;
   const int key = (l31 >> 1) & 7;
@@ -286,6 +288,10 @@
       auto r1 = __builtin_amdgcn_permlane32_swap(a1, b1, false, false);
       *(uint4*)(so + l31 * 128 + (((4 * dt + 2 * gp + half) ^ (l31 & 7)) << 4)) = make_uint4(r0[0], r1[0], r0[1], r1[1]);
     }
+  if (CLS) {
+    if (lane < 8) *(uint4*)((char*)(cc + h * 64) + lane * 16) = *(const uint4*)(so + (lane << 4));
+    return;
+  }
   char* const out = (char*)(ctx + (row0 + q0) * (int64_t)H + h * 64);
 #pragma unroll
   for (int it = 0; it < 4; ++it) {
@@ -317,6 +323,42 @@
   }
   OM_ATTN_BODY(KT);
 #undef OM_ATTN_BODY
+}
+
+template <typename T, int KT>
+__global__ __launch_bounds__(64 * KT, KT <= 4 ? 4 : 2) void attention_fwd16_cls_kernel(
+    const T* __restrict__ qkv, const T* __restrict__ q, T* __restrict__ ctx, const int64_t* __restrict__ mask, int64_t B, int L, int H,
+    int heads, float scale, int rev, const int* __restrict__ kmax, const int* __restrict__ cu) {
+#define OM_ATTN_BODY(V) \
+  attention_fwd16_body<T, KT, false, false, 0, V, true>(qkv, nullptr, mask, nullptr, Lb, H, heads, scale, 0.f, 0, rev, row0, L, q + b * H, ctx + r * H, b)
+  const int64_t r = rev ? (int64_t)(gridDim.x / heads) - 1 - blockIdx.x / heads : blockIdx.x / heads;
+  const int64_t b = r < B ? r : B - 1;
+  int64_t row0 = b * L;
+  int Lb = L;
+  if (cu) {
+    const int c0 = __builtin_amdgcn_readfirstlane(cu[b]), c1 = __builtin_amdgcn_readfirstlane(cu[b + 1]);
+    row0 = c0; Lb = c1 - c0;
+    if (Lb <= 0) return;
+  }
+  if (KT == 4 && (kmax || cu)) {
+    const int kt = ((cu ? Lb : __builtin_amdgcn_readfirstlane(kmax[b])) + 31) >> 5;
+    if (kt <= 1) { OM_ATTN_BODY(1); return; }
+    if (kt == 2) { OM_ATTN_BODY(2); return; }
+    if (kt == 3) { OM_ATTN_BODY(3); return; }
+  }
+  OM_ATTN_BODY(KT);
+#undef OM_ATTN_BODY
+}
+
+template <typename T, int KT>
+static int launch_attn16_cls(const void* qkv, const void* q, void* ctx, const int64_t* mask, int64_t B, int64_t Mc, int L, int H, int heads,
+                             float scale, hipStream_t s, int rev, const int* kmax, const int* cu) {
+  const int lds = 2 * KT * 32 * 128 + KT * 32 * 4;
+  if (attn_lds_once<attention_fwd16_cls_kernel<T, KT>>(lds)) return 1;
+  hipLaunchKernelGGL((attention_fwd16_cls_kernel<T, KT>), dim3((unsigned)(heads * Mc)), dim3(64 * KT), lds, s, (const T*)qkv, (const T*)q,
+                     (T*)ctx, mask, B, L, H, heads, scale, rev, kmax, cu);
+  OM_LAUNCH_CHECK();
+  return 0;
 }
 
 template <typename T, int KT, bool BIAS, bool DROP>
@@ -512,6 +554,29 @@
   }
 }
 
+int omk_attention_cls(int dtype, const void* qkv, const void* q, void* ctx, const int64_t* mask, int64_t B, int64_t Mc, int L, int H, int heads,
+                      float scale, hipStream_t s, int reverse, const int* kmax, const int* cu) {
+  g_attn_last = 0;
+  if (B <= 0) return 0;
+  const AttnPlan p = attn_plan_fwd(dtype, B, L, H, heads, false, 0.f, kmax != nullptr, cu != nullptr, 0, attn_switches());
+  if (p.error) OM_FAIL(p.error);
+  if (p.family != OM_ATTN_FAMILY_FWD16 && p.family != OM_ATTN_FAMILY_FWD16_KMAX4) OM_FAIL("[CLS]-query attention: the 16-bit kernel up to 256 tokens, head_dim 64");
+  if (Mc < B || Mc * heads > 0x7fffffffLL) OM_FAIL("[CLS]-query attention: B <= Mc, Mc * heads below 2^31");
+  g_attn_last = p.family | (p.kt << 8);
+  return attn_with_type16(dtype, [&](auto t) {
+    return attn_with_kt<1, 2, 4, 6, 8>(p.kt, [&](auto kt) {
+      return launch_attn16_cls<decltype(t), kt()>(qkv, q, ctx, mask, B, Mc, L, H, heads, scale, s, reverse, kmax, cu);
+    });
+  });
+}
+extern "C" int om_debug_attention_cls(int dtype, const void* qkv, const void* q, void* ctx, const int64_t* mask, int64_t B, int64_t Mc, int L, int H,
+                                      int heads, float scale, void* stream, int reverse, const int* kmax, const int* cu) {
+  g_attn_last = 0;
+  if (!qkv || !q || !ctx || !mask) OM_FAIL("null argument");
+  if (dtype != OM_BF16 && dtype != OM_F16) OM_FAIL("[CLS]-query attention: dtype must be OM_BF16 or OM_F16");
+  return omk_attention_cls(dtype, qkv, q, ctx, mask, B, Mc, L, H, heads, scale, (hipStream_t)stream, reverse, kmax, cu);
+}
+
 extern "C" int om_debug_attention_plan(int dtype, int64_t B, int L, int H, int heads, int has_bias, float drop_p, int has_kmax, int has_cu, int w) {
   const AttnPlan p = attn_plan_fwd(dtype, B, L, H, heads, has_bias != 0, drop_p, has_kmax != 0, has_cu != 0, w, attn_switches());
   if (p.error) { om_set_error(std::string(__func__) + ": " + p.error); return -1; }
diff --git a/openmatch_amd/csrc/encoder.hip b/openmatch_amd/csrc/encoder.hip
--- a/openmatch_amd/csrc/encoder.hip
+++ b/openmatch_amd/csrc/encoder.hip
@@ -191,6 +191,17 @@
   return encoder_cls_tail(in, encoder_plan(in, sw), sw) ? 1 : 0;
 }
 
+extern "C" int om_debug_encoder_cls_query(const OmEncoderConfig* c, int gated_ffn, int has_rel_bias, int64_t B, int64_t L, int64_t packed_rows,
+                                          int want_hidden) {
+  if (!c) {
+    om_set_error("om_debug_encoder_cls_query: null argument");
+    return -1;
+  }
+  const EncPlanIn in = {c, B, L, packed_rows, want_hidden != 0, gated_ffn != 0, has_rel_bias != 0, c->type_vocab > 0};
+  const EncSwitches sw = encoder_switches();
+  return encoder_cls_query(in, encoder_plan(in, sw), sw) ? 1 : 0;
+}
+
 extern "C" int om_t5_relative_bucket(int relative_position, int num_buckets, int max_distance) {
   int nb = num_buckets / 2;
   int bucket = relative_position > 0 ? nb : 0;
@@ -224,6 +235,7 @@
   int64_t cls_mc;
   std::vector<int>* families;
   int64_t whole_mg, whole_mc;
+  bool cls_query;
 };
 
 struct EncStream {
@@ -254,6 +266,9 @@
   const void* const ffa = nomic ? ws.ff2 : ws.ff
 #define NOMIC_ROPE() do { if (nomic) RUN(omk_rope(dt, ws.qkv, M, (int)L, H, c->rope_theta_global, s, k.row_map)); } while (0)
 #define NOMIC_SWIGLU(rows_) do { if (nomic) RUN(omk_swiglu_rows(dt, ws.ff, ws.ff2, rows_, F, s)); } while (0)
+
+static std::atomic<int64_t> g_cls_query_chains{0};
+extern "C" int64_t om_debug_encoder_cls_query_chains(void) { return g_cls_query_chains.load(); }
 
 static int bert_fused(const EncCall& k, EncStream* out) {
   ENC_LOCALS;
@@ -276,16 +291,20 @@
 #define LAUNCH(expr) do { if (!probe) RUN(expr); } while (0)
   const int64_t Mc = k.cls_mc;
   const size_t cplane = (size_t)Mc * H * 2;
-  char* const cbase = ws.qkv;
-  float* const cst2p = (float*)(cbase + 7 * cplane);
-  float* const cst1 = cst2p + 2 * Mc;
-  if (Mc > 0 && ((char*)(cst1 + 2 * Mc) > ws.qkv + (size_t)Mg * 3 * H * 2 || Mc > Mg || c->n_layers < 2 || lo8))
-    OM_FAIL("[CLS] tail: the compact buffers do not fit the qkv area");
+  char* cbase = ws.qkv;
+  float *cst2p = nullptr, *cst1 = nullptr;
+  auto compact_in = [&](bool ff) {
+    cbase = ff ? ws.ff + (size_t)Mc * F1 * 2 : ws.qkv;
+    cst2p = (float*)(cbase + (ff ? 8 : 7) * cplane);
+    cst1 = cst2p + 2 * Mc;
+    return (char*)(cst1 + 2 * Mc) <= (ff ? ws.ff + (size_t)Mg * F1 * 2 : ws.qkv + (size_t)Mg * 3 * H * 2);
+  };
+  if (Mc > 0 && (!compact_in(false) || Mc > Mg || c->n_layers < 2 || lo8)) OM_FAIL("[CLS] tail: the compact buffers do not fit the qkv area");
 #define OM_WALK() (pingpong ? (walk ^= 1, walk ^ 1) : 0)
   for (int l = 0; l < c->n_layers; ++l) {
     const OmLayerWeights& lw = Ls[l];
     const bool last = l == c->n_layers - 1, tail = last && Mc > 0;
-    float* st1 = tail ? cst1 : ws.stats1 + (size_t)l * Mg * 2;
+    bool cq = false;
     float* st2 = ws.stats2 + (size_t)l * Mg * 2;
     const float* st2p = l ? ws.stats2 + (size_t)(l - 1) * Mg * 2 : nullptr;
     const int64_t Mr = tail ? Mc : Mg;
@@ -301,14 +320,41 @@
       const void* wf; const float *cs, *bfp;
       RUN(folded_weights(c, k.w, l, false, lw.qkv_w, pw.ln2_g, pw.ln2_b, lw.qkv_b, 3 * H, H, ws.wfold, ws.colsum, ws.bfold, s, &wf, &cs, &bfp));
       e.bias = bfp; e.ln_stats = st2p; e.ln_colsum = cs; e.ln_inv_h = inv_h; e.ln_eps = c->ln_eps; e.reverse = OM_WALK(); e.rows_dev = k.rows_dev;
-      RUN(gemm(ws.x1, H, wf, H, ws.qkv, 3 * H, Mg, 3 * H, H, e));
+      GemmEpilogue ekv = e, eq = e;
+      ekv.bias = bfp + H; ekv.ln_colsum = cs + H;
+      eq.rows_dev = nullptr;
+      const char* const wkv = (const char*)wf + (size_t)H * H * 2;
+      char* const ckv = ws.qkv + (size_t)H * 2;
+      if (tail && k.cls_query && compact_in(true)) {
+        eq.ln_stats = cst2p;
+        const int fam = omk_gemm_family(dt, ws.x1, H, wf, H, dt, ws.qkv, 3 * H, Mg, 3 * H, H, e, k.whole_mg);
+        cq = fam > 0 && omk_gemm_family(dt, ws.x1, H, wkv, H, dt, ckv, 3 * H, Mg, 2 * H, H, ekv, k.whole_mg) == fam &&
+             omk_gemm_family(dt, cbase + cplane, H, wf, H, dt, cbase + 7 * cplane, H, Mc, H, H, eq, k.whole_mc) == fam;
+      }
+      if (cq && !probe) g_cls_query_chains.fetch_add(1);
+      if (cq) {
+        const GatherPlane planes[3] = {{nullptr, nullptr}, {ws.x1, cbase + cplane}, {two ? ws.x1_lo : nullptr, cbase + 2 * cplane}};
+        LAUNCH(omk_gather_rows(planes, st2p, cst2p, k.cu ? ws.cls_rows : nullptr, B, L, Mc, H, s));
+        RUN(gemm(ws.x1, H, wkv, H, ckv, 3 * H, Mg, 2 * H, H, ekv));
+        RUN(gemm(cbase + cplane, H, wf, H, cbase + 7 * cplane, H, Mc, H, H, eq));
+      } else {
+        if (tail) compact_in(false);
+        RUN(gemm(ws.x1, H, wf, H, ws.qkv, 3 * H, Mg, 3 * H, H, e));
+      }
     }
     if (!probe) NOMIC_ROPE();
     const int attn_walk = OM_WALK();
-    LAUNCH(omk_attention(dt, ws.qkv, ws.ctx, k.mask, k.posbias, B, (int)L, H, nh, scale, 0.f, 0, s, attn_walk, ws.kmax, k.cu));
+    if (cq) {
+      LAUNCH(omk_attention_cls(dt, ws.qkv, cbase + 7 * cplane, cbase, k.mask, B, Mc, (int)L, H, nh, scale, s, attn_walk, ws.kmax, k.cu));
+    } else {
+      LAUNCH(omk_attention(dt, ws.qkv, ws.ctx, k.mask, k.posbias, B, (int)L, H, nh, scale, 0.f, 0, s, attn_walk, ws.kmax, k.cu));
+      if (tail) {
+        const GatherPlane planes[3] = {{ws.ctx, cbase}, {ws.x1, cbase + cplane}, {two ? ws.x1_lo : nullptr, cbase + 2 * cplane}};
+        LAUNCH(omk_gather_rows(planes, st2p, cst2p, k.cu ? ws.cls_rows : nullptr, B, L, Mc, H, s));
+      }
+    }
+    float* st1 = tail ? cst1 : ws.stats1 + (size_t)l * Mg * 2;
     if (tail) {
-      const GatherPlane planes[3] = {{ws.ctx, cbase}, {ws.x1, cbase + cplane}, {two ? ws.x1_lo : nullptr, cbase + 2 * cplane}};
-      LAUNCH(omk_gather_rows(planes, st2p, cst2p, k.cu ? ws.cls_rows : nullptr, B, L, Mc, H, s));
       ctx = cbase; xin = cbase + cplane; xin_lo = cbase + 2 * cplane; st2p = cst2p;
       y = cbase + 3 * cplane; y_lo = cbase + 4 * cplane; xout = cbase + 5 * cplane; xout_lo = cbase + 6 * cplane;
     }
@@ -810,11 +856,12 @@
   const bool packed = pack_bound > 0;
   int64_t cls_mc = 0;
   if (!encoder_cls_tail(plan_in, plan, sw, &cls_mc)) cls_mc = 0;
+  const bool cls_query = cls_mc > 0 && !om_timing_on() && encoder_cls_query(plan_in, plan, sw);
   const int* const row_map = packed ? ws.row_map : nullptr;
   if (families) {
     if (plan.path != OM_ENC_PATH_BERT_FUSED) OM_FAIL("encoder lanes: the fused BERT path only");
     const EncCall k = {c, w, attention_mask, B, L, plan, ws, nullptr, packed ? ws.cu : nullptr, row_map, out_hidden, s, skip ? ws.cu + B : nullptr,
-                       cls_mc, families, q.whole_mg, q.whole_mc};
+                       cls_mc, families, q.whole_mg, q.whole_mc, cls_query};
     EncStream unused = {};
     RUN(bert_fused(k, &unused));
     if (c->head_in > 0 && w->head_w)
@@ -840,7 +887,7 @@
     RUN(omk_embed(dt, input_ids, nullptr, w->word_emb, nullptr, nullptr, nullptr, nullptr, ws.x, M, (int)L, H, c->vocab, 1, c->ln_eps, 0, s, row_map));
 
   const EncCall k = {c, w, attention_mask, B, L, plan, ws, plan.rel_bias ? ws.posbias : nullptr, packed ? ws.cu : nullptr, row_map, out_hidden, s,
-                     skip ? ws.cu + B : nullptr, cls_mc, nullptr, q.whole_mg, q.whole_mc};
+                     skip ? ws.cu + B : nullptr, cls_mc, nullptr, q.whole_mg, q.whole_mc, cls_query};
   EncStream stream_out = {};
   switch (plan.path) {
     case OM_ENC_PATH_BERT_FUSED: RUN(bert_fused(k, &stream_out)); break;
diff --git a/openmatch_amd/csrc/encoder_plan.h b/openmatch_amd/csrc/encoder_plan.h
--- a/openmatch_amd/csrc/encoder_plan.h
+++ b/openmatch_amd/csrc/encoder_plan.h
@@ -1,6 +1,7 @@
 #pragma once
 #include <algorithm>
 
+#include "attn_plan.h"
 #include "kernels.h"
 
 bool omk_gemm_skinny_ok(int in_dtype, int out_dtype, int64_t M, int64_t N, int64_t K, const GemmEpilogue& ep, int max_m);
@@ -15,12 +16,14 @@
   int skip_pad;
   int cls_tail;
   int lanes;
+  int cls_query;
 };
 
 static EncSwitches encoder_switches() {
   return EncSwitches{om_option(OM_OPT_ENCODER_FUSED_LN), om_option(OM_OPT_ENCODER_TWO_PLANE), om_option(OM_OPT_ENCODER_PINGPONG),
                      om_option(OM_OPT_GEMM_SKINNY_M), om_option(OM_OPT_FEW_ROWS_LN_FUSE), om_option(OM_OPT_ATTENTION_FAST),
-                     om_option(OM_OPT_ENCODER_SKIP_PAD), om_option(OM_OPT_ENCODER_CLS_TAIL), om_option(OM_OPT_ENCODER_LANES)};
+                     om_option(OM_OPT_ENCODER_SKIP_PAD), om_option(OM_OPT_ENCODER_CLS_TAIL), om_option(OM_OPT_ENCODER_LANES),
+                     om_option(OM_OPT_ENCODER_CLS_QUERY)};
 }
 
 struct EncPlanIn {
@@ -184,6 +187,17 @@
   return true;
 }
 
+static bool encoder_cls_query(const EncPlanIn& in, const EncPlan& p, const EncSwitches sw) {
+  int64_t mc = 0;
+  if (!sw.cls_query || !encoder_cls_tail(in, p, sw, &mc)) return false;
+  const OmEncoderConfig* c = in.c;
+  if (c->arch != OM_ARCH_BERT || c->head_dim != 64 || p.rel_bias || in.has_rel_bias) return false;
+  const AttnPlan a = attn_plan_fwd(c->dtype, in.B, (int)in.L, c->hidden, c->n_heads, false, 0.f, true, in.packed_rows > 0, 0, AttnSwitches{sw.attention_fast});
+  if (a.error || (a.family != OM_ATTN_FAMILY_FWD16 && a.family != OM_ATTN_FAMILY_FWD16_KMAX4)) return false;
+  const int64_t H = c->hidden, F1 = enc_ffn1_cols(c);
+  return (F1 + 8 * H) * mc * 2 + 4 * mc * 4 <= F1 * p.Mp * 2;
+}
+
 static const int64_t ENC_LANE_ROWS_END = 131072;
 static bool encoder_lanes(const EncPlanIn& in, const EncPlan& p, const EncSwitches sw, int64_t* B0 = nullptr) {
   if (sw.lanes <= 0 || in.packed_rows != 0 || in.want_hidden || in.has_rel_bias || in.c->pooling == OM_POOL_NONE) return false;
@@ -193,13 +207,13 @@
   const int64_t b0 = in.B / 2 / step * step;
   if (b0 <= 0 || b0 * in.L < (int64_t)sw.lanes || (in.B - b0) * in.L < (int64_t)sw.lanes) return false;
   if ((in.B - b0) * in.L >= ENC_LANE_ROWS_END) return false;
-  const bool skip = encoder_skip_pad(in, p, sw), tail = encoder_cls_tail(in, p, sw);
+  const bool skip = encoder_skip_pad(in, p, sw), tail = encoder_cls_tail(in, p, sw), query = encoder_cls_query(in, p, sw);
   for (const int64_t bh : {b0, in.B - b0}) {
     EncPlanIn li = in;
     li.B = bh;
     const EncPlan lp = encoder_plan_checked(li, sw);
     if (lp.error || lp.path != p.path || lp.two != p.two || lp.lo8 != p.lo8 || lp.pingpong != p.pingpong) return false;
-    if (encoder_skip_pad(li, lp, sw) != skip || encoder_cls_tail(li, lp, sw) != tail) return false;
+    if (encoder_skip_pad(li, lp, sw) != skip || encoder_cls_tail(li, lp, sw) != tail || encoder_cls_query(li, lp, sw) != query) return false;
   }
   if (B0) *B0 = b0;
   return true;
diff --git a/openmatch_amd/csrc/kernels.h b/openmatch_amd/csrc/kernels.h
--- a/openmatch_amd/csrc/kernels.h
+++ b/openmatch_amd/csrc/kernels.h
@@ -33,6 +33,8 @@
                   const int* kmax = nullptr ,
                   const int* cu = nullptr ,
                   int w = 0 );
+int omk_attention_cls(int dtype, const void* qkv, const void* q, void* ctx, const int64_t* mask, int64_t B, int64_t Mc, int L, int H, int heads,
+                      float scale, hipStream_t s, int reverse, const int* kmax, const int* cu);
 struct AttnPlan;
 int omk_attention_d32(const AttnPlan& p, int dtype, const void* qkv, void* ctx, const int64_t* mask, const float* pos_bias, int64_t B, int L,
                       int H, int heads, float scale, float drop_p, uint64_t seed, hipStream_t s, int reverse, const int* kmax, const int* cu);
diff --git a/openmatch_amd/native.py b/openmatch_amd/native.py
--- a/openmatch_amd/native.py
+++ b/openmatch_amd/native.py
@@ -190,6 +190,10 @@
     "om_debug_encoder_plan": (c_int, [C.POINTER(OmEncoderConfig), c_int, c_int, c_int64, c_int64, c_int64, c_int]),
     "om_debug_encoder_skip_pad": (c_int, [C.POINTER(OmEncoderConfig), c_int, c_int, c_int64, c_int64, c_int]),
     "om_debug_encoder_cls_tail": (c_int, [C.POINTER(OmEncoderConfig), c_int, c_int, c_int64, c_int64, c_int64, c_int]),
+    "om_debug_encoder_cls_query": (c_int, [C.POINTER(OmEncoderConfig), c_int, c_int, c_int64, c_int64, c_int64, c_int]),
+    "om_debug_encoder_cls_query_chains": (c_int64, []),
+    "om_debug_attention_cls": (c_int, [c_int, c_void_p, c_void_p, c_void_p, c_void_p, c_int64, c_int64, c_int, c_int, c_int, c_float, c_void_p,
+                                       c_int, c_void_p, c_void_p]),
     "om_debug_encoder_lanes": (c_int, [C.POINTER(OmEncoderConfig), c_int, c_int, c_int64, c_int64, c_int64, c_int, C.POINTER(c_int64)]),
     "om_debug_encoder_lane_ranges": (c_int, [C.POINTER(OmEncoderConfig), c_int, c_int, c_int64, c_int64, c_int, C.POINTER(c_int64), c_int]),
     "om_debug_encoder_lane_forks": (c_int64, []),
```
